# duanyiqun/DiffusionDepth

Measured on AMD Instinct MI355X. Metric: depth-maps/sec (20-step DDIM, KITTI 352x1216 f16r, B=4 maps per GPU per step; depth RMSE vs the reference's CPU path <= 1e-3 on this workload AND at KITTI's depth range 0-80 m: see cpu_baseline.rmse_gate), higher is better.
Workload: dtype f16 (f16 MFMA operands, fp32 accumulation; refined mode: f16-pair weights in conv1 / conv4 / conv3(cond), block-scaled int16 hand-over of y3 and conv3(cond)); 1 GPU; kitti 352x1216 image -> latent 16x176x608, cond 256x176x608, Res head denoiser (mmbev_res50 config), T=20, encoder+loop+decoder, inputs resident in HBM; global_batch=4, parallelism=dp1 (independent images, no collective), ranks_seen=1, streams=2, graph=True, variant=res

## Files before the change

### diffusiondepth_amd/backend.py

```python
from __future__ import annotations

import ctypes
import os
from typing import Dict, Optional

import numpy as np

_HERE = os.path.dirname(os.path.abspath(__file__))
_LIB_NAME = "libddepth_hip.so"
_lib = None

PRECISIONS = {"naive_fp32": 0, "fp32": 1, "bf16": 2, "f16": 3, "fp16": 3, "f16x3": 4, "split_f16": 4, "f16r": 5, "refined_f16": 5}
VARIANTS = {"res": 0, "swin": 1}

ABI_SYMBOLS = [
    "dd_create", "dd_destroy", "dd_last_error", "dd_version", "dd_set_weight", "dd_set_weight_device", "dd_commit_weights",
    "dd_set_schedule", "dd_condition", "dd_neck_condition", "dd_denoise", "dd_denoise_trace", "dd_denoise_once", "dd_denoise_once_backward", "dd_denoise_backward", "dd_zero_grad", "dd_get_grad", "dd_add_noise", "dd_encode", "dd_decode",
    "dd_set_option", "dd_last_loop_ms", "dd_get_counter", "dd_get_layer_ms", "dd_debug_fetch", "dd_debug_weights_digest",
]


def precision_id(p) -> int:
    if isinstance(p, int):
        return p
# ... 272 lines not shown
        cond_in = cond
        cond = _check_tensor(cond, "cond", dtype=torch.float32)
        if cond is not cond_in:
            self._cond_token = None
        B, C, h, w = x_T.shape
        if C != 16 or cond.dim() != 4 or cond.shape[0] != B or cond.shape[1] != 256:
            raise ValueError(f"x_T must be (B,16,h,w) and cond (B,256,ch,cw); got {tuple(x_T.shape)}, {tuple(cond.shape)}")
        T = int(num_inference_steps)
        states = torch.empty((max(T, 1), B, 16, h, w), device=self.device, dtype=torch.float32)
        with torch.cuda.device(self.device):
            self._ck(self._lib.dd_denoise_trace(self._h, x_T.data_ptr(), self._cond_arg(cond, precision), states.data_ptr(), B, h, w,
                                                cond.shape[2], cond.shape[3], T, precision_id(precision), _stream_ptr(self.device)),
                     "dd_denoise_trace")
        return states

    def denoise_once(self, x_t, t, cond, precision="fp32", keep_trajectory=False):
        torch = _torch()
        x_t = _check_tensor(x_t, "x_t", dtype=torch.float32)
        cond = _check_tensor(cond, "cond", dtype=torch.float32)
        B, C, h, w = x_t.shape
        t = torch.as_tensor(t, device=self.device).to(torch.int64).reshape(-1)
        if t.numel() == 1 and B > 1:
            t = t.expand(B)
        t = _check_tensor(t, "t", (B,), torch.int64)
        out = torch.empty_like(x_t)
        self.last_trajectory_ticket = 0
        if keep_trajectory:
            self.set_option("keep_trajectory", 1)
        try:
            with torch.cuda.device(self.device):
                self._ck(self._lib.dd_denoise_once(self._h, x_t.data_ptr(), t.data_ptr(), self._cond_arg(cond, precision), out.data_ptr(),
                                                   B, h, w, cond.shape[2], cond.shape[3], precision_id(precision),
                                                   _stream_ptr(self.device)), "dd_denoise_once")
            if keep_trajectory and precision != "naive_fp32":
                self.last_trajectory_ticket = self.counter("trajectory_ticket")
        finally:
            if keep_trajectory:
                self.set_option("keep_trajectory", 0)
        return out

    PARAM_SHAPES = {
        "model.noise_embedding.0.weight": (64, 16, 3, 3), "model.noise_embedding.0.bias": (64,),
        "model.noise_embedding.1.weight": (64,), "model.noise_embedding.1.bias": (64,),
        "model.noise_embedding.3.weight": (256, 64, 3, 3), "model.noise_embedding.3.bias": (256,),
        "model.noise_embedding.4.weight": (256,), "model.noise_embedding.4.bias": (256,),
        "model.time_embedding.weight": (1280, 256),
        "model.pred.0.weight": (64, 256, 3, 3), "model.pred.0.bias": (64,),
        "model.pred.1.weight": (64,), "model.pred.1.bias": (64,),
        "model.pred.3.weight": (16, 64, 3, 3), "model.pred.3.bias": (16,),
        "model.pred.4.weight": (16,), "model.pred.4.bias": (16,),
    }

    SWIN_PARAM_SHAPES = {
        "model.upsample_fuse.convA.conv.weight": (256, 256, 3, 3), "model.upsample_fuse.convA.conv.bias": (256,),
        "model.upsample_fuse.convB.conv.weight": (256, 256, 3, 3), "model.upsample_fuse.convB.conv.bias": (256,),
    }

    def param_shapes(self):
        d = dict(self.PARAM_SHAPES)
        if self.variant == "swin":
            d.update(self.SWIN_PARAM_SHAPES)
        return d

    def denoise_once_backward(self, x_t, t, cond, grad_eps, precision="naive_fp32", need_grad_x=True, need_grad_cond=True,
                              trajectory_ticket=0):
        torch = _torch()
        x_t = _check_tensor(x_t, "x_t", dtype=torch.float32)
        cond = _check_tensor(cond, "cond", dtype=torch.float32)
        grad_eps = _check_tensor(grad_eps, "grad_eps", x_t.shape, torch.float32)
        B, C, h, w = x_t.shape
        t = torch.as_tensor(t, device=self.device).to(torch.int64).reshape(-1)
        if t.numel() == 1 and B > 1:
            t = t.expand(B)
        t = _check_tensor(t, "t", (B,), torch.int64)
        gx = torch.empty_like(x_t) if need_grad_x else None
        gc = torch.empty_like(cond) if need_grad_cond else None
        if trajectory_ticket:
            self.set_option("use_trajectory", int(trajectory_ticket))
        with torch.cuda.device(self.device):
            self._ck(self._lib.dd_denoise_once_backward(
                self._h, x_t.data_ptr(), t.data_ptr(), cond.data_ptr(), grad_eps.data_ptr(),
                gx.data_ptr() if gx is not None else None, gc.data_ptr() if gc is not None else None,
                B, h, w, cond.shape[2], cond.shape[3], precision_id(precision), _stream_ptr(self.device)), "dd_denoise_once_backward")
        self._cond_token = None
        return gx, gc

    def denoise_backward(self, x_T, cond, grad_x0, num_inference_steps: int, precision="naive_fp32", need_grad_xT=False, need_grad_cond=True,
                         trajectory_ticket=0):
        torch = _torch()
        x_T = _check_tensor(x_T, "x_T", dtype=torch.float32)
        cond = _check_tensor(cond, "cond", dtype=torch.float32)
        grad_x0 = _check_tensor(grad_x0, "grad_x0", x_T.shape, torch.float32)
        B, C, h, w = x_T.shape
        gx = torch.empty_like(x_T) if need_grad_xT else None
        gc = torch.empty_like(cond) if need_grad_cond else None
        if trajectory_ticket:
            self.set_option("use_trajectory", int(trajectory_ticket))
        with torch.cuda.device(self.device):
            self._ck(self._lib.dd_denoise_backward(
                self._h, x_T.data_ptr(), cond.data_ptr(), grad_x0.data_ptr(), gx.data_ptr() if gx is not None else None,
                gc.data_ptr() if gc is not None else None, B, h, w, cond.shape[2], cond.shape[3], int(num_inference_steps),
                precision_id(precision), _stream_ptr(self.device)), "dd_denoise_backward")
        self._cond_token = None
        return gx, gc

    def zero_grad(self):
        self._ck(self._lib.dd_zero_grad(self._h, _stream_ptr(self.device)), "dd_zero_grad")

    def grad(self, name: str):
        torch = _torch()
        out = torch.empty(self.param_shapes()[name], device=self.device, dtype=torch.float32)
        with torch.cuda.device(self.device):
            self._ck(self._lib.dd_get_grad(self._h, name.encode(), out.data_ptr(), out.numel(), _stream_ptr(self.device)), f"dd_get_grad({name})")
        return out

    def grads(self):
        return {k: self.grad(k) for k in self.param_shapes()}

    def add_noise(self, x0, noise, t):
        torch = _torch()
        x0 = _check_tensor(x0, "x0", dtype=torch.float32)
        noise = _check_tensor(noise, "noise", x0.shape, torch.float32)
        B = x0.shape[0]
        t = _check_tensor(torch.as_tensor(t, device=self.device).to(torch.int64).reshape(-1), "t", (B,), torch.int64)
        out = torch.empty_like(x0)
        C, h, w = (x0.shape[1], x0.shape[2], x0.shape[3]) if x0.dim() == 4 else (1, 1, x0[0].numel())
        with torch.cuda.device(self.device):
            self._ck(self._lib.dd_add_noise(self._h, x0.data_ptr(), noise.data_ptr(), t.data_ptr(), out.data_ptr(),
                                            B, C, h, w, _stream_ptr(self.device)), "dd_add_noise")
        return out

    def encode(self, depth):
        torch = _torch()
        depth = _check_tensor(depth, "depth", dtype=torch.float32)
        B, C, H, W = depth.shape
        if C != 1:
            raise ValueError("depth must be (B,1,H,W)")
        out = torch.empty((B, 16, (H - 1) // 2 + 1, (W - 1) // 2 + 1), device=depth.device, dtype=torch.float32)
        with torch.cuda.device(self.device):
            self._ck(self._lib.dd_encode(self._h, depth.data_ptr(), out.data_ptr(), B, H, W, _stream_ptr(self.device)), "dd_encode")
        return out

    def decode(self, latent):
        torch = _torch()
        latent = _check_tensor(latent, "latent", dtype=torch.float32)
        B, C, h, w = latent.shape
        if C != 16:
            raise ValueError("latent must be (B,16,h,w)")
        out = torch.empty((B, 1, 2 * h, 2 * w), device=latent.device, dtype=torch.float32)
        with torch.cuda.device(self.device):
            self._ck(self._lib.dd_decode(self._h, latent.data_ptr(), out.data_ptr(), B, h, w, _stream_ptr(self.device)), "dd_decode")
        return out

    def debug_fetch(self, name: str, B: int, h: int, w: int):
        torch = _torch()
        C = {"y1": 64, "y2": 256, "y3": 64, "y4": 16}[name]
        out = torch.empty((B, C, h, w), device=self.device, dtype=torch.float32)
        self._ck(self._lib.dd_debug_fetch(self._h, name.encode(), out.data_ptr(), out.numel(), _stream_ptr(self.device)),
                 "dd_debug_fetch")
        return out
```

### diffusiondepth_amd/csrc/dd_api.cpp

```cpp
#include "dd_api_internal.h"
#include <cstdlib>

namespace ddapi {
thread_local std::string g_create_error;
}


extern "C" {

const char* dd_version(void) { return "ddepth 0.1 gfx950 (hip, mfma bf16/f16/f32 implicit-GEMM conv3x3+GN+ReLU, hipGraph DDIM loop)"; }

const char* dd_last_error(dd_handle_t h) { return h ? h->err.c_str() : g_create_error.c_str(); }

int dd_create(dd_handle_t* out, int device, int variant) {
  if (!out) { g_create_error = "dd_create: out is NULL"; return DD_ERR_INVALID_ARG; }
  *out = nullptr;
  if (variant != DD_VARIANT_RES && variant != DD_VARIANT_SWIN) { g_create_error = "dd_create: unknown variant"; return DD_ERR_INVALID_ARG; }
  int n = 0;
  hipError_t e = hipGetDeviceCount(&n);
  if (e != hipSuccess || n <= 0) {
    g_create_error = std::string("dd_create: no HIP device available (") + (e != hipSuccess ? hipGetErrorString(e) : "count = 0") +
                     "); this library has no CPU fallback";
    return DD_ERR_HIP;
  }
  if (device < 0 || device >= n) { g_create_error = "dd_create: device index out of range"; return DD_ERR_INVALID_ARG; }
  e = hipSetDevice(device);
  if (e != hipSuccess) { g_create_error = std::string("hipSetDevice: ") + hipGetErrorString(e); return DD_ERR_HIP; }
  dd_handle_t h = new dd_handle_s();
  h->device = device;
  h->variant = variant;
  {
    hipDeviceProp_t prop;
    if (hipGetDeviceProperties(&prop, device) == hipSuccess && prop.multiProcessorCount > 0) {
      h->resident_slots = 2 * prop.multiProcessorCount;
      h->thin_slots = h->resident_slots > 4096 ? 4096 : h->resident_slots;
    }
  }
  {
    const char* pc = getenv("DEBUG_CLR_GRAPH_PACKET_CAPTURE");
    h->use_graph = pc && pc[0] == '0' && pc[1] == 0;
    h->graph_off_by_env = !h->use_graph;
  }
  *out = h;
  return DD_OK;
}

int dd_destroy(dd_handle_t h) {
  if (!h) return DD_OK;
  (void)hipSetDevice(h->device);
  (void)hipDeviceSynchronize();
  drain_layer_events(h);
  h->plans.clear();
  if (h->ev0) (void)hipEventDestroy(h->ev0);
  if (h->ev1) (void)hipEventDestroy(h->ev1);
  if (h->cap_stream) (void)hipStreamDestroy(h->cap_stream);
  for (int l = 0; l < dd_handle_s::MAX_LANES; ++l) {
    if (h->lane_stream[l]) (void)hipStreamDestroy(h->lane_stream[l]);
    if (h->lane_done[l]) (void)hipEventDestroy(h->lane_done[l]);
  }
  if (h->lane_fork) (void)hipEventDestroy(h->lane_fork);
  for (hipStream_t b : h->burnt_streams) (void)hipStreamDestroy(b);
  for (hipEvent_t e : h->probe_events) (void)hipEventDestroy(e);
  delete h;
  return DD_OK;
}

int dd_set_schedule(dd_handle_t h, const float* alphas_cumprod, int num_train_timesteps) {
  if (!h) return DD_ERR_INVALID_ARG;
  if (!alphas_cumprod || num_train_timesteps <= 0) return h->fail(DD_ERR_INVALID_ARG, "dd_set_schedule: null table or non-positive length");
  if (num_train_timesteps > EMB_ROWS)
    return h->fail(DD_ERR_INVALID_ARG, "dd_set_schedule: num_train_timesteps exceeds the time embedding's " + std::to_string(EMB_ROWS) +
                                       " rows (reference ...res.py:313 nn.Embedding(1280, 256))");
  for (int i = 0; i < num_train_timesteps; ++i)
    if (!(alphas_cumprod[i] > 0.f && alphas_cumprod[i] <= 1.f))
      return h->fail(DD_ERR_INVALID_ARG, "dd_set_schedule: alphas_cumprod must lie in (0, 1]");
  DD_HIP(hipSetDevice(h->device));
  DD_HIP(hipDeviceSynchronize());
  h->plans.clear();
  h->last_once_plan = nullptr;
  h->acp.assign(alphas_cumprod, alphas_cumprod + num_train_timesteps);
  h->n_train = num_train_timesteps;
  DD_HIP(h->d_acp.alloc((size_t)num_train_timesteps * 4));
  DD_HIP(hipMemcpy(h->d_acp.p, h->acp.data(), (size_t)num_train_timesteps * 4, hipMemcpyHostToDevice));
  return DD_OK;
}

int dd_set_option(dd_handle_t h, const char* key, int64_t value) {
  if (!h || !key) return DD_ERR_INVALID_ARG;
  const std::string k(key);
  if (k == "graph") h->use_graph = value != 0;
  else if (k == "timing") h->timing = value != 0;
  else if (k == "debug_sync") h->debug_sync = value != 0;
  else if (k == "check_finite") h->check_finite = (int)value;
  else if (k == "train_graphs") h->train_graphs = value != 0;
  else if (k == "graph_fence") h->graph_fence = (int)value;
  else if (k == "ablate") {
    if (h->ablate != (int)value) {
      DD_HIP(hipDeviceSynchronize());
      h->plans.clear();
      h->last_once_plan = nullptr;
    }
    h->ablate = (int)value;
  }
  else if (k == "swin_w5") {
    if (value < 0 || value > 1) return h->fail(DD_ERR_INVALID_ARG, "dd_set_option: swin_w5 must be 0 or 1");
    if (h->swin_w5 != (int)value) { DD_HIP(hipDeviceSynchronize()); h->plans.clear(); h->last_once_plan = nullptr; }
    h->swin_w5 = (int)value;
  }
  else if (k == "hoist_cond") {
    if (value < -1 || value > 1) return h->fail(DD_ERR_INVALID_ARG, "dd_set_option: hoist_cond must be -1 (automatic), 0 or 1");
    h->hoist_cond = (int)value;
  }
  else if (k == "bf16_storage") {
    if (h->bf16_pure != (value != 0)) {
      DD_HIP(hipDeviceSynchronize());
      h->plans.clear(); h->last_once_plan = nullptr;
      h->cond_bufs.clear(); h->fpn_cond.reset(); h->fpn_cond_key[3] = -1; h->fpn_out.reset(); h->fpn_work.reset();
    }
    h->bf16_pure = value != 0;
  }
  else if (k == "naive_wgrad") h->naive_wgrad = value != 0;
  else if (k == "lane_probe") h->lane_probe = value != 0;
  else if (k == "x3_grad_fp32") h->x3_grad_fp32 = value != 0;
  else if (k == "keep_trajectory") h->keep_traj = value != 0;
  else if (k == "use_trajectory") h->use_traj = value;
  else if (k == "adjoint_tiled") h->adjoint_tiled = value != 0;
  else if (k == "streams") h->n_streams = value < 1 ? 1 : (int)value;
  else if (k == "keep_activations_mb") h->keep_act_mb = value < 0 ? 0 : value;
  else if (k == "big_tiles") {
    if (value < -1 || value > 1) return h->fail(DD_ERR_INVALID_ARG, "dd_set_option: big_tiles must be -1 (automatic), 0 or 1");
    if (h->big_tiles != (int)value) { DD_HIP(hipDeviceSynchronize()); h->plans.clear(); h->last_once_plan = nullptr; }
    h->big_tiles = (int)value;
  }
  else if (k == "thin_slots") {
    if (value < 1 || value > 4096) return h->fail(DD_ERR_INVALID_ARG, "dd_set_option: thin_slots must be in [1, 4096]");
    if (h->thin_slots != (int)value) { DD_HIP(hipDeviceSynchronize()); h->plans.clear(); h->last_once_plan = nullptr; }
    h->thin_slots = (int)value;
  }
  else if (k == "one_buffer") {
    if (value < 0 || value > 2) return h->fail(DD_ERR_INVALID_ARG, "dd_set_option: one_buffer must be 0, 1 or 2");
    if (h->one_buffer != (int)value) { DD_HIP(hipDeviceSynchronize()); h->plans.clear(); h->last_once_plan = nullptr; }
    h->one_buffer = (int)value;
  }
  else if (k == "cond_direct") {
    if (value < 0 || value > 1) return h->fail(DD_ERR_INVALID_ARG, "dd_set_option: cond_direct must be 0 or 1");
    h->cond_direct = (int)value;
  }
  else if (k == "cond_split") {
    if (value < 0 || value > 1) return h->fail(DD_ERR_INVALID_ARG, "dd_set_option: cond_split must be 0 or 1");
    h->cond_split = (int)value;
  }
  else if (k == "thin_stream") {
    if (value < 0 || value > 1) return h->fail(DD_ERR_INVALID_ARG, "dd_set_option: thin_stream must be 0 or 1");
    if (h->thin_stream != (int)value) {
      DD_HIP(hipDeviceSynchronize());
      h->plans.clear(); h->last_once_plan = nullptr;
    }
    h->thin_stream = (int)value;
  }
  else if (k == "f16r_wide" || k == "f16r_p4" || k == "f16r_c1") {
    if (value < 0 || value > 1) return h->fail(DD_ERR_INVALID_ARG, "dd_set_option: " + k + " must be 0 or 1");
    int& opt = k == "f16r_wide" ? h->f16r_wide : k == "f16r_c1" ? h->f16r_c1 : h->f16r_p4;
    if (opt != (int)value) { DD_HIP(hipDeviceSynchronize()); h->plans.clear(); h->last_once_plan = nullptr; }
    opt = (int)value;
  }
  else if (k == "phase_prof_buffer") h->prof_buf = reinterpret_cast<unsigned long long*>((uintptr_t)value);
  else if (k == "phase_prof_layer") h->prof_layer = (int)value;
  else if (k == "layer_timing") {
    drain_layer_events(h);
    h->layer_timing = value != 0;
    for (int i = 0; i < dd_handle_s::N_LAYER_SLOTS; ++i) { h->layer_ms[i] = 0; h->layer_cnt[i] = 0; }
  } else return h->fail(DD_ERR_INVALID_ARG, "dd_set_option: unknown key '" + k + "'");
  return DD_OK;
}

int dd_get_counter(dd_handle_t h, const char* key, int64_t* value) {
  if (!h || !key || !value) return DD_ERR_INVALID_ARG;
  const std::string k(key);
  if (k == "graph_launches") *value = h->n_graph_launches;
  else if (k == "graph_default") *value = h->graph_off_by_env ? 0 : 1;
  else if (k == "eager_loops") *value = h->n_eager_loops;
  else if (k == "graph_capture_failures") *value = h->n_capture_failures;
  else if (k == "plans") *value = (int64_t)h->plans.size();
  else if (k == "neck_launches") *value = h->n_neck_launches;
  else if (k == "trajectory_ticket") *value = h->traj_serial;
  else if (k == "lane_calls") *value = h->n_lane_calls;
  else if (k == "lane_probe_retries") *value = h->n_lane_probe_retries;
  else if (k == "lane_overlap") *value = h->lane_overlap_seen;
  else if (k == "cond_split_ok") *value = (h->fpn_committed && h->fpn_split_ok ? 1 : 0) | (h->neck_committed && h->neck_split_ok ? 2 : 0);
  else if (k == "resident_slots") *value = h->resident_slots;
  else if (k == "trajectory_reuses") *value = h->n_traj_reuse;
  else if (k == "thin_stream_launches") *value = h->thin_stream_launches;
  else if (k.compare(0, 13, "kid_launches:") == 0) {
    int id = 0;
    const size_t n = k.size() - 13;
    bool ok = n >= 1 && n <= 3 && !(n > 1 && k[13] == '0');
    for (size_t i = 13; ok && i < k.size(); ++i) { ok = k[i] >= '0' && k[i] <= '9'; id = id * 10 + (k[i] - '0'); }
    if (!ok || !kid_listed(id)) return h->fail(DD_ERR_INVALID_ARG, "dd_get_counter: '" + k + "' does not name a kernel id (dd_kernel_ids.h)");
    *value = h->kid_launches[id];
  }
  else return h->fail(DD_ERR_INVALID_ARG, "dd_get_counter: unknown key '" + k + "'");
  return DD_OK;
}

int dd_get_layer_ms(dd_handle_t h, int layer, double* total_ms, int64_t* launches) {
  if (!h || layer < 1 || layer > dd_handle_s::N_LAYER_SLOTS || !total_ms || !launches) return DD_ERR_INVALID_ARG;
  drain_layer_events(h);
  *total_ms = h->layer_ms[layer - 1];
  *launches = h->layer_cnt[layer - 1];
  return DD_OK;
}

int dd_last_loop_ms(dd_handle_t h, float* ms) {
  if (!h || !ms) return DD_ERR_INVALID_ARG;
  *ms = 0.f;
  if (!h->ev_valid) return DD_OK;
  DD_HIP(hipEventSynchronize(h->ev1));
  DD_HIP(hipEventElapsedTime(ms, h->ev0, h->ev1));
  return DD_OK;
}

static int condition_impl(dd_handle_t h, const float* const* feats, const int* feat_h, const int* feat_w, int n_levels, int B,
                          float* cond_out, int precision, void* stream, bool with_neck);

int dd_condition(dd_handle_t h, const float* const* feats, const int* feat_h, const int* feat_w, int n_levels, int B,
                 float* cond_out, int precision, void* stream) {
  return condition_impl(h, feats, feat_h, feat_w, n_levels, B, cond_out, precision, stream, false);
}

int dd_neck_condition(dd_handle_t h, const float* const* feats, const int* feat_h, const int* feat_w, int n_levels, int B,
                      float* cond_out, int precision, void* stream) {
  if (!h) return DD_ERR_INVALID_ARG;
  if (!h->neck_committed) return h->fail(DD_ERR_STATE, "hahineck.* weights not committed (dd_set_weight for the lateral / projection / fusion convolutions, "
                                                       "dd_commit_weights; DD_VARIANT_SWIN)");
  return condition_impl(h, feats, feat_h, feat_w, n_levels, B, cond_out, precision, stream, true);
}

static int condition_impl(dd_handle_t h, const float* const* feats, const int* feat_h, const int* feat_w, int n_levels, int B,
                          float* cond_out, int precision, void* stream, bool with_neck) {
  if (!h) return DD_ERR_INVALID_ARG;
  if (!h->fpn_committed) return h->fail(DD_ERR_STATE, "conv_lateral.* / conv_up.* weights not committed (dd_set_weight, dd_commit_weights)");
  if (with_neck && h->variant != DD_VARIANT_SWIN)
    return h->fail(DD_ERR_UNSUPPORTED, "dd_neck_condition: the HAHI neck kernels are built for the Swin-L (192/384/768/1536) and MPViT-small (128/216/288/288) pyramids of DD_VARIANT_SWIN");
  if (n_levels != FPN_LEVELS || !feats || !feat_h || !feat_w) return h->fail(DD_ERR_INVALID_ARG, "dd_condition: expects 4 pyramid levels");
  if (precision < DD_PREC_FP32 || precision > DD_PREC_LAST) return h->fail(DD_ERR_INVALID_ARG, "dd_condition: precision must be fp32, bf16, f16, f16x3 or f16r");
  if (B <= 0) return h->fail(DD_ERR_INVALID_ARG, "dd_condition: B must be positive");
  for (int i = 0; i < FPN_LEVELS; ++i) {
    if (!feats[i] || feat_h[i] <= 0 || feat_w[i] <= 0) return h->fail(DD_ERR_INVALID_ARG, "dd_condition: null feature pointer or non-positive size");
    if ((long long)B * feat_h[i] * feat_w[i] * fpn_cin_pad(h->variant, h->fpn_pyramid)[i] >= (1LL << 31) * 4) return h->fail(DD_ERR_INVALID_ARG, "tensor too large");
  }
  hipStream_t s = reinterpret_cast<hipStream_t>(stream);
  DD_HIP(hipSetDevice(h->device));
  int ek = ek_of_precision(precision, h->bf16_pure);
  bool split_pyr = false;
  if (ek == EK_F16S || ek == EK_F16R) {
    split_pyr = h->cond_split && h->fpn_split_ok && (!with_neck || h->neck_split_ok);
    ek = EK_F32;
  }
  const int kk = split_pyr ? (int)EK_F16S : ek;
  const int wk = split_pyr ? WIMG_SPLIT : opnd_kind(ek);
  const int ok = opnd_kind(ek), sk = store_kind(ek);
  const size_t es = ek_size(ek);
  FpnWork* fw = h->fpn_work.get();
  bool same = fw && fw->B == B && fw->ek == ek && fw->pyr == h->fpn_pyramid && (fw->neck || !with_neck);
  for (int i = 0; same && i < FPN_LEVELS; ++i) same = fw->hs[i] == feat_h[i] && fw->ws[i] == feat_w[i];
  if (!same) {
    DD_HIP(hipDeviceSynchronize());
    h->fpn_work.reset(new FpnWork());
    fw = h->fpn_work.get();
    fw->B = B; fw->ek = ek; fw->pyr = h->fpn_pyramid;
    for (int i = 0; i < FPN_LEVELS; ++i) {
      fw->hs[i] = feat_h[i]; fw->ws[i] = feat_w[i];
      const size_t px = (size_t)B * feat_h[i] * feat_w[i];
      DD_HIP(fw->fin[i].alloc(px * fpn_cin_pad(h->variant, h->fpn_pyramid)[i] * es));
      if (with_neck) {
        DD_HIP(fw->nk_cat[i].alloc(px * (neck_ck(h->fpn_pyramid, i) + 512) * es));
        DD_HIP(fw->nk_out[i].alloc(px * neck_ck(h->fpn_pyramid, i) * es));
        fw->neck = true;
      }
      if (i > 0) {
        DD_HIP(fw->lat[i].alloc(px * COND_C * es));
        DD_HIP(fw->up[i - 1].alloc(px * 4 * COND_C * es));
        if (2 * feat_h[i] != feat_h[i - 1] || 2 * feat_w[i] != feat_w[i - 1])
          DD_HIP(fw->pooled[i - 1].alloc((size_t)B * feat_h[i - 1] * feat_w[i - 1] * COND_C * es));
      }
    }
  }
  std::shared_ptr<DevBuf> cbuf;
  int rc = DD_OK;
  const bool swin = h->variant == DD_VARIANT_SWIN;
  if (swin) {
    const size_t need = (size_t)B * feat_h[0] * feat_w[0] * COND_C * es;
    if (!h->fpn_out || h->fpn_out->bytes < need) { h->fpn_out = std::make_shared<DevBuf>(); DD_HIP(h->fpn_out->alloc(need)); }
    cbuf = h->fpn_out;
  } else {
    rc = get_cond_buf(h, B, feat_h[0], feat_w[0], precision, &cbuf);
    if (rc) return rc;
  }

  const int P = pyramid_of(h->variant, h->fpn_pyramid);
  for (int i = FPN_LEVELS - 1; i >= 0; --i) {
    const int hh = feat_h[i], ww = feat_w[i];
    DD_HIP(launch_nchw_to_nhwc_padded(feats[i], fw->fin[i].p, ok, B, fpn_cin(h->variant, h->fpn_pyramid)[i],
                                      fpn_cin_pad(h->variant, h->fpn_pyramid)[i], hh, ww, 1, s));
    const int lat_layer = kid_fpn_lateral(P, i);
    const void* lat_in = fw->fin[i].p;
    if (with_neck) {
      const int C = neck_ck(h->fpn_pyramid, i), CT = C + 512, l_off = (i == 0) ? 512 : 0, e_off = (i == 0) ? 0 : C;
      ConvParams q{};
      q.B = B; q.h = hh; q.w = ww;
      q.in = fw->fin[i].p; q.in_cstride = C; q.in_coff = 0;
      q.out = fw->nk_cat[i].p; q.out_cstride = CT; q.out_coff = l_off;
      q.wpack = h->neck_w[i][wk].p; q.bias = h->neck_b[i].as<float>();
      DD_TRY(launch_conv(h, kid_neck(P, NECK_LATERAL, i), kk, q, s, kid_neck(P, NECK_LATERAL, i)));
      q.in = fw->nk_cat[i].p; q.in_cstride = CT; q.in_coff = l_off;
      q.out = fw->nk_cat[i].p; q.out_cstride = CT; q.out_coff = e_off;
      q.wpack = h->neck_w[4 + i][wk].p; q.bias = h->neck_b[4 + i].as<float>();
      DD_TRY(launch_conv(h, kid_neck(P, NECK_PROJ, i), kk, q, s, kid_neck(P, NECK_PROJ, i)));
      q.in = fw->nk_cat[i].p; q.in_cstride = CT; q.in_coff = 0;
      q.out = fw->nk_out[i].p; q.out_cstride = C; q.out_coff = 0;
      q.wpack = h->neck_w[8 + i][wk].p; q.bias = h->neck_b[8 + i].as<float>();
      DD_TRY(launch_conv(h, kid_neck(P, NECK_FUSION, i), kk, q, s, kid_neck(P, NECK_FUSION, i)));
      h->n_neck_launches += 3;
      lat_in = fw->nk_out[i].p;
    }
    ConvParams p{};
    p.B = B; p.h = hh; p.w = ww;
    p.in = lat_in; p.wpack = h->fpn_lat_w[i][wk].p; p.bias = h->fpn_lat_b[i].as<float>();
    p.out = (i == 0) ? cbuf->p : fw->lat[i].p;
    p.addend = (i == FPN_LEVELS - 1) ? nullptr : (fw->pooled[i].p ? fw->pooled[i].p : fw->up[i].p);
    DD_TRY(launch_conv(h, lat_layer, kk, p, s, lat_layer));
    if (i > 0) {
      ConvParams u{};
      u.B = B; u.h = hh; u.w = ww;
      u.in = fw->lat[i].p; u.wpack = h->fpn_up_w[i - 1][wk].p; u.bias = h->fpn_up_b[i - 1].as<float>(); u.out = fw->up[i - 1].p;
      DD_TRY(launch_conv(h, KID_FPN_UP, kk, u, s, KID_FPN_UP));
      if (fw->pooled[i - 1].p)
        DD_HIP(launch_adaptive_pool_blocked(fw->up[i - 1].p, fw->pooled[i - 1].p, ok, B, COND_C, 2 * hh, 2 * ww, feat_h[i - 1], feat_w[i - 1], s));
    }
    if (h->debug_sync) DD_HIP(hipStreamSynchronize(s));
  }
  if (cond_out) DD_HIP(launch_blocked_to_nchw(cbuf->p, sk, cond_out, B, COND_C, feat_h[0], feat_w[0], 0, s));
  h->fpn_cond = cbuf;
  h->fpn_cond_key[0] = B; h->fpn_cond_key[1] = feat_h[0]; h->fpn_cond_key[2] = feat_w[0]; h->fpn_cond_key[3] = precision;
  return DD_OK;
}

}

namespace ddapi {
int denoise_lane(dd_handle_t h, const float* x_T, const float* cond, float* x_0, int B, int lat_h, int lat_w,
                 int cond_h, int cond_w, int T, int precision, hipStream_t s, int lane, int img0, int whole_B, int64_t ticket, int S) {
  int rc = DD_OK;
  const bool timed = h->timing && lane == 0 && B == whole_B;
  Plan* pl = nullptr;
  int keep = (h->keep_traj && precision != DD_PREC_NAIVE_FP32) ? 1 : 0;
  if (keep) {
    const size_t es = ek_size(store_kind(ek_of_precision(precision, h->bf16_pure)));
    const size_t per_step = (size_t)B * lat_h * lat_w * ((2 * HID_C + COND_C + (h->variant == DD_VARIANT_SWIN ? 2 * COND_C : 0)) * es + LATENT_C * 4);
    const size_t need = per_step * (size_t)T;
    if (need <= ((size_t)h->keep_act_mb << 20) &&
        (h->plans.count(PlanKey{B, lat_h, lat_w, cond_h, cond_w, T, precision, want_hoist(h, precision, T, 2), 2, lane, S}) || keep2_fits(h, need))) keep = 2;
  }
  rc = get_plan(h, PlanKey{B, lat_h, lat_w, cond_h, cond_w, T, precision, want_hoist(h, precision, T, keep), keep, lane, S}, &pl);
  if (rc && keep == 2) {
    (void)hipGetLastError();
    h->plans.erase(PlanKey{B, lat_h, lat_w, cond_h, cond_w, T, precision, want_hoist(h, precision, T, 2), 2, lane, S});
    keep = 1;
    rc = get_plan(h, PlanKey{B, lat_h, lat_w, cond_h, cond_w, T, precision, want_hoist(h, precision, T, keep), keep, lane, S}, &pl);
  }
  if (rc) return rc;
  const size_t n16 = (size_t)B * lat_h * lat_w * LATENT_C;
  float* x_first = keep ? pl->xstash.as<float>() : pl->x[0].as<float>();
  const float* x_last = keep ? pl->xstash.as<float>() + (size_t)(T - 1) * n16 : pl->x[(T - 1) & 1].as<float>();
  if (keep) pl->traj_ticket = 0;

  DD_HIP(launch_nchw_to_nhwc(x_T, x_first, EK_F32, B, LATENT_C, lat_h, lat_w, 0, s));
  rc = stage_condition(h, pl, cond, B, lat_h, lat_w, cond_h, cond_w, precision, s, img0, whole_B);
  if (rc) return rc;
  if (pl->exec && !pl->key.hoist && pl->graph_cond != pl->cond_ptr()) {
    DD_HIP(hipStreamSynchronize(s));
    (void)hipGraphExecDestroy(pl->exec);
    pl->exec = nullptr;
  }

  if (timed) {
    if (!h->ev0) { DD_HIP(hipEventCreate(&h->ev0)); DD_HIP(hipEventCreate(&h->ev1)); }
    DD_HIP(hipEventRecord(h->ev0, s));
  }
  if (precision == DD_PREC_NAIVE_FP32) {
    DD_HIP(hipMemsetAsync(pl->stats.p, 0, pl->stats_bytes, s));
    for (int k = 0; k < T; ++k) {
      float* xc = pl->x[k & 1].as<float>();
      float* xn = pl->x[(k + 1) & 1].as<float>();
      rc = enqueue_naive_eps(h, pl, k, xc, pl->tsteps.as<long long>(), k, 0, s);
      if (rc) return rc;
      DD_HIP(launch_naive_axpby(xc, pl->eps.as<float>(), pl->c1c2.as<float>(), k, xn, (long long)B * lat_h * lat_w * LATENT_C, s));
    }
    h->n_eager_loops++;
    if (timed) { DD_HIP(hipEventRecord(h->ev1, s)); h->ev_valid = true; }
    DD_HIP(launch_nhwc_to_nchw_f32(pl->x[T & 1].p, EK_F32, x_0, B, LATENT_C, lat_h, lat_w, 0, s));
    return DD_OK;
  }

  const bool want_graph = h->use_graph && !h->layer_timing && !h->debug_sync && !pl->capture_failed && (!keep || h->train_graphs);
  bool launched = false;
  if (want_graph) {
    if (!pl->exec) {
      rc = enqueue_loop_body(h, pl, s);
      if (rc) return rc;
      DD_HIP(hipStreamSynchronize(s));
      hipGraph_t graph = nullptr;
      hipError_t e = hipSuccess;
      if (!h->cap_stream) e = hipStreamCreateWithFlags(&h->cap_stream, hipStreamNonBlocking);
      if (e == hipSuccess) e = hipStreamBeginCapture(h->cap_stream, hipStreamCaptureModeThreadLocal);
      if (e == hipSuccess) {
        int brc = enqueue_loop_body(h, pl, h->cap_stream);
        hipError_t e2 = hipStreamEndCapture(h->cap_stream, &graph);
        if (brc == DD_OK && e2 == hipSuccess && graph) {
          e = hipGraphInstantiate(&pl->exec, graph, nullptr, nullptr, 0);
          if (e != hipSuccess) pl->exec = nullptr;
          pl->graph_cond = pl->cond_ptr();
        }
        if (graph) (void)hipGraphDestroy(graph);
      }
      if (!pl->exec) {
        (void)hipGetLastError();
        pl->capture_failed = true;
        h->n_capture_failures++;
      }
      DD_HIP(launch_nchw_to_nhwc(x_T, x_first, EK_F32, B, LATENT_C, lat_h, lat_w, 0, s));
      if (timed) DD_HIP(hipEventRecord(h->ev0, s));
    }
    if (pl->exec) {
      if (h->graph_fence & 1) DD_HIP(hipStreamSynchronize(s));
      if (h->graph_fence & 4) {
        if (!h->lane_fork) DD_HIP(hipEventCreateWithFlags(&h->lane_fork, hipEventDisableTiming));
        if (!h->lane_done[0]) DD_HIP(hipEventCreateWithFlags(&h->lane_done[0], hipEventDisableTiming));
        DD_HIP(hipEventRecord(h->lane_fork, s));
        DD_HIP(hipStreamWaitEvent(h->cap_stream, h->lane_fork, 0));
        DD_HIP(hipGraphLaunch(pl->exec, h->cap_stream));
        DD_HIP(hipEventRecord(h->lane_done[0], h->cap_stream));
        DD_HIP(hipStreamWaitEvent(s, h->lane_done[0], 0));
      } else
      DD_HIP(hipGraphLaunch(pl->exec, s));
      if (h->graph_fence & 2) DD_HIP(hipStreamSynchronize(s));
      h->n_graph_launches++;
      launched = true;
    }
  }
  if (!launched) {
    rc = enqueue_loop_body(h, pl, s);
    if (rc) return rc;
    h->n_eager_loops++;
  }
  if (timed) { DD_HIP(hipEventRecord(h->ev1, s)); h->ev_valid = true; }
  DD_HIP(launch_final(x_last, static_cast<const float*>(pl->slot(pl->y4, T - 1)), pl->stat_ptr(T - 1, 3), h->L[3].gamma.as<float>(),
                      h->L[3].beta.as<float>(), pl->c1c2.as<float>(), T - 1, 0, x_0, B, lat_h, lat_w, s));
  if (keep) { pl->traj_ticket = ticket; pl->traj_weights = h->weights_serial; pl->traj_consumed = false; }
  if (h->debug_sync) DD_HIP(hipStreamSynchronize(s));
  return DD_OK;
}
}

namespace ddapi {
int acquire_lane_stream(dd_handle_t h, int lane, hipStream_t caller) {
  hipStream_t cand = nullptr;
  DD_HIP(hipStreamCreateWithFlags(&cand, hipStreamNonBlocking));
#ifndef DD_HOST_EMULATION
  hipStreamCaptureStatus cs = hipStreamCaptureStatusNone;
  const bool capturing = hipStreamIsCapturing(caller, &cs) == hipSuccess && cs != hipStreamCaptureStatusNone;
  if (h->lane_probe && !capturing) {
    hipEvent_t ea = nullptr, ed = nullptr, ec = nullptr;
    long long* stamps = nullptr;
    DD_HIP(hipEventCreateWithFlags(&ea, hipEventDisableTiming)); DD_HIP(hipEventCreateWithFlags(&ed, hipEventDisableTiming)); DD_HIP(hipEventCreateWithFlags(&ec, hipEventDisableTiming));
    h->probe_events.push_back(ea); h->probe_events.push_back(ed); h->probe_events.push_back(ec);
    DD_HIP(hipMalloc(&stamps, 4 * sizeof(long long)));
    const long long ticks = 10000;
    int rc_ = DD_OK;
    for (int attempt = 0; attempt < 4; ++attempt) {
      hipError_t e = launch_spin(1, nullptr, caller);
      if (e == hipSuccess) e = launch_spin(1, nullptr, cand);
      if (e == hipSuccess) e = hipStreamSynchronize(caller);
      if (e == hipSuccess) e = hipStreamSynchronize(cand);
      if (e == hipSuccess) e = hipEventRecord(ea, caller);
      if (e == hipSuccess) e = hipStreamWaitEvent(cand, ea, 0);
      if (e == hipSuccess) e = launch_spin(ticks, stamps, caller);
      if (e == hipSuccess) e = launch_spin(ticks, stamps + 2, cand);
      if (e == hipSuccess) e = hipEventRecord(ec, cand);
      if (e == hipSuccess) e = hipStreamWaitEvent(caller, ec, 0);
      if (e == hipSuccess) e = hipEventRecord(ed, caller);
      if (e == hipSuccess) e = hipEventSynchronize(ed);
      long long t[4] = {0, 0, 0, 0};
      if (e == hipSuccess) e = hipMemcpy(t, stamps, sizeof t, hipMemcpyDeviceToHost);
      if (e != hipSuccess) { rc_ = h->fail(DD_ERR_HIP, std::string("lane-overlap probe: ") + hipGetErrorString(e)); break; }
      const long long lo = t[0] > t[2] ? t[0] : t[2], hi = t[1] < t[3] ? t[1] : t[3];
      const bool overlap = hi - lo > ticks / 2;
      h->lane_overlap_seen = overlap ? 1 : 0;
      if (overlap || attempt == 3) break;
      h->burnt_streams.push_back(cand);
      h->n_lane_probe_retries++;
      cand = nullptr;
      e = hipStreamCreateWithFlags(&cand, hipStreamNonBlocking);
      if (e != hipSuccess) { rc_ = h->fail(DD_ERR_HIP, std::string("lane-overlap probe: ") + hipGetErrorString(e)); break; }
    }
    (void)hipFree(stamps);
    if (rc_) { if (cand) (void)hipStreamDestroy(cand); return rc_; }
  }
#else
  (void)caller;
#endif
  h->lane_stream[lane] = cand;
  return DD_OK;
}
}

extern "C" {

int dd_denoise(dd_handle_t h, const float* x_T, const float* cond, float* x_0, int B, int lat_h, int lat_w,
               int cond_h, int cond_w, int T, int precision, void* stream) {
  int rc = check_common(h, B, lat_h, lat_w, cond_h, cond_w, true);
  if (rc) return rc;
// ... 25 lines not shown
    const int n = B / S + (l < B % S ? 1 : 0);
    hipStream_t ls = l == 0 ? s : h->lane_stream[l];
    if (l > 0) DD_HIP(hipStreamWaitEvent(ls, h->lane_fork, 0));
    rc = denoise_lane(h, x_T + img0 * n_x, cond ? cond + img0 * n_c : nullptr, x_0 + img0 * n_x, n, lat_h, lat_w, cond_h, cond_w, T, precision,
                      ls, l, img0, B, ticket, S);
    if (l > 0) {
      (void)hipEventRecord(h->lane_done[l], ls);
      (void)hipStreamWaitEvent(s, h->lane_done[l], 0);
    }
    if (rc) return rc;
    img0 += n;
  }
  h->n_lane_calls++;
  if (h->timing) { DD_HIP(hipEventRecord(h->ev1, s)); h->ev_valid = true; }
  return DD_OK;
}

int dd_denoise_trace(dd_handle_t h, const float* x_T, const float* cond, float* states, int B, int lat_h, int lat_w,
                     int cond_h, int cond_w, int T, int precision, void* stream) {
  int rc = check_common(h, B, lat_h, lat_w, cond_h, cond_w, true);
  if (rc) return rc;
  if (!x_T || !states) return h->fail(DD_ERR_INVALID_ARG, "dd_denoise_trace: null tensor pointer");
  if (T <= 0 || T > h->n_train) return h->fail(DD_ERR_INVALID_ARG, "dd_denoise_trace: num_inference_steps must be in [1, num_train_timesteps]");
  if (precision < DD_PREC_NAIVE_FP32 || precision > DD_PREC_LAST) return h->fail(DD_ERR_INVALID_ARG, "dd_denoise_trace: unknown precision");
  rc = check_split(h, precision, "dd_denoise_trace"); if (rc) return rc;
  if (h->variant == DD_VARIANT_SWIN && precision == DD_PREC_NAIVE_FP32)
    return h->fail(DD_ERR_UNSUPPORTED, "DD_VARIANT_SWIN runs on the fused kernels only (no naive path)");
  hipStream_t s = reinterpret_cast<hipStream_t>(stream);
  DD_HIP(hipSetDevice(h->device));
  Plan* pl = nullptr;
  rc = get_plan(h, PlanKey{B, lat_h, lat_w, cond_h, cond_w, T, precision, want_hoist(h, precision, T, 0)}, &pl);
  if (rc) return rc;
  const bool naive = precision == DD_PREC_NAIVE_FP32;
  const size_t n16 = (size_t)B * lat_h * lat_w * LATENT_C;
  if (pl->xstash.bytes < (size_t)(T + 1) * n16 * 4) DD_HIP(pl->xstash.alloc((size_t)(T + 1) * n16 * 4));
  float* X = pl->xstash.as<float>();
  const long long* ts = pl->tsteps.as<long long>();
  DD_HIP(launch_nchw_to_nhwc(x_T, X, EK_F32, B, LATENT_C, lat_h, lat_w, 0, s));
  rc = stage_condition(h, pl, cond, B, lat_h, lat_w, cond_h, cond_w, precision, s);
  if (rc) return rc;
  DD_HIP(hipMemsetAsync(pl->stats.p, 0, pl->stats_bytes, s));
  for (int k = 0; k < T; ++k) {
    if (naive) {
      rc = enqueue_naive_eps(h, pl, k, X + (size_t)k * n16, ts, k, 0, s);
      if (rc) return rc;
      DD_HIP(launch_naive_axpby(X + (size_t)k * n16, pl->eps.as<float>(), pl->c1c2.as<float>(), k, X + (size_t)(k + 1) * n16, (long long)n16, s));
    } else {
      rc = enqueue_fused_step(h, pl, k, (k == 0) ? X : X + (size_t)(k - 1) * n16, X + (size_t)k * n16, k > 0, ts, k, 0, s);
      if (rc) return rc;
    }
  }
  h->n_eager_loops++;
  for (int j = 0; j + 1 < T; ++j)
    DD_HIP(launch_nhwc_to_nchw_f32(X + (size_t)(j + 1) * n16, EK_F32, states + (size_t)j * n16, B, LATENT_C, lat_h, lat_w, 0, s));
  if (naive) {
    DD_HIP(launch_nhwc_to_nchw_f32(X + (size_t)T * n16, EK_F32, states + (size_t)(T - 1) * n16, B, LATENT_C, lat_h, lat_w, 0, s));
  } else {
    DD_HIP(launch_final(X + (size_t)(T - 1) * n16, pl->y4.as<float>(), pl->stat_ptr(T - 1, 3), h->L[3].gamma.as<float>(),
                        h->L[3].beta.as<float>(), pl->c1c2.as<float>(), T - 1, 0, states + (size_t)(T - 1) * n16, B, lat_h, lat_w, s));
  }
  if (h->debug_sync) DD_HIP(hipStreamSynchronize(s));
  return DD_OK;
}

int dd_denoise_once(dd_handle_t h, const float* x_t, const int64_t* t, const float* cond, float* eps, int B, int lat_h,
                    int lat_w, int cond_h, int cond_w, int precision, void* stream) {
  int rc = check_common(h, B, lat_h, lat_w, cond_h, cond_w, false);
  if (rc) return rc;
  if (!x_t || !t || !eps) return h->fail(DD_ERR_INVALID_ARG, "dd_denoise_once: null pointer");
  if (precision < DD_PREC_NAIVE_FP32 || precision > DD_PREC_LAST) return h->fail(DD_ERR_INVALID_ARG, "dd_denoise_once: unknown precision");
  rc = check_split(h, precision, "dd_denoise_once"); if (rc) return rc;
  if (h->variant == DD_VARIANT_SWIN && precision == DD_PREC_NAIVE_FP32)
    return h->fail(DD_ERR_UNSUPPORTED, "DD_VARIANT_SWIN runs on the fused kernels only (no naive path)");
  hipStream_t s = reinterpret_cast<hipStream_t>(stream);
  DD_HIP(hipSetDevice(h->device));
  Plan* pl = nullptr;
  rc = get_plan(h, PlanKey{B, lat_h, lat_w, cond_h, cond_w, 0, precision, want_hoist(h, precision, 0, 0)}, &pl);
  if (rc) return rc;
  const long long* tv = reinterpret_cast<const long long*>(t);
  DD_HIP(launch_nchw_to_nhwc(x_t, pl->x[0].p, EK_F32, B, LATENT_C, lat_h, lat_w, 0, s));
  rc = stage_condition(h, pl, cond, B, lat_h, lat_w, cond_h, cond_w, precision, s);
  if (rc) return rc;
  if (h->variant == DD_VARIANT_SWIN && pl->key.hoist) {
    if (!h->LA.w_oihw.p || !h->LB.w_oihw.p || !h->L[2].w_oihw.p) return h->fail(DD_ERR_STATE, "hoisted Swin form: the fp32 weights of the fuse convolutions are not on the device");
    DD_HIP(launch_swin_ttab(h->LA.w_oihw.as<float>(), h->LB.w_oihw.as<float>(), h->L[2].w_oihw.as<float>(), h->emb.as<float>(), tv, B, lat_h, lat_w,
                            pl->tt_scratch.as<float>(), pl->ttab.as<float>(), s));
  }
  DD_HIP(hipMemsetAsync(pl->stats.p, 0, pl->stats_bytes, s));
  if (precision == DD_PREC_NAIVE_FP32) {
    rc = enqueue_naive_eps(h, pl, 0, pl->x[0].as<float>(), tv, 0, 1, s);
    if (rc) return rc;
    DD_HIP(launch_nhwc_to_nchw_f32(pl->eps.p, EK_F32, eps, B, LATENT_C, lat_h, lat_w, 0, s));
  } else {
    rc = enqueue_fused_step(h, pl, 0, pl->x[0].as<float>(), pl->x[1].as<float>(), false, tv, 0, 1, s);
    if (rc) return rc;
    DD_HIP(launch_final(pl->x[0].as<float>(), pl->y4.as<float>(), pl->stat_ptr(0, 3), h->L[3].gamma.as<float>(),
                        h->L[3].beta.as<float>(), pl->c1c2.as<float>(), 0, 1, eps, B, lat_h, lat_w, s));
  }
  h->last_once_plan = pl;
  pl->traj_ticket = (h->keep_traj && precision != DD_PREC_NAIVE_FP32) ? ++h->traj_serial : 0;
  pl->traj_weights = h->weights_serial;
  if (h->debug_sync) DD_HIP(hipStreamSynchronize(s));
  return DD_OK;
}

int dd_add_noise(dd_handle_t h, const float* x0, const float* noise, const int64_t* t, float* out, int B, int C,
                 int lat_h, int lat_w, void* stream) {
  if (!h) return DD_ERR_INVALID_ARG;
  if (h->n_train <= 0) return h->fail(DD_ERR_STATE, "schedule not set (dd_set_schedule)");
  if (!x0 || !noise || !t || !out || B <= 0 || C <= 0 || lat_h <= 0 || lat_w <= 0)
    return h->fail(DD_ERR_INVALID_ARG, "dd_add_noise: null pointer or non-positive size");
  DD_HIP(hipSetDevice(h->device));
  DD_HIP(launch_add_noise(x0, noise, reinterpret_cast<const long long*>(t), h->d_acp.as<float>(), h->n_train, out, B,
                          (long long)C * lat_h * lat_w, reinterpret_cast<hipStream_t>(stream)));
  return DD_OK;
}

static int ensure_codec_tmp(dd_handle_t h, size_t bytes) {
  if (h->codec_tmp.bytes >= bytes) return DD_OK;
  DD_HIP(hipDeviceSynchronize());
  DD_HIP(h->codec_tmp.alloc(bytes));
  return DD_OK;
}

int dd_encode(dd_handle_t h, const float* depth, float* latent, int B, int H, int W, void* stream) {
  if (!h) return DD_ERR_INVALID_ARG;
  if (!h->codec_committed) return h->fail(DD_ERR_STATE, "depth_transform.* weights not committed");
  if (!depth || !latent || B <= 0 || H <= 0 || W <= 0) return h->fail(DD_ERR_INVALID_ARG, "dd_encode: null pointer or non-positive size");
  DD_HIP(hipSetDevice(h->device));
  const int lh = (H - 1) / 2 + 1, lw = (W - 1) / 2 + 1;
  int rc = ensure_codec_tmp(h, (size_t)B * lh * lw * LATENT_C * 4);
  if (rc) return rc;
  DD_HIP(launch_encode(h->codec, depth, h->codec_tmp.as<float>(), latent, B, H, W, reinterpret_cast<hipStream_t>(stream)));
  return DD_OK;
}

int dd_decode(dd_handle_t h, const float* latent, float* depth, int B, int lat_h, int lat_w, void* stream) {
  if (!h) return DD_ERR_INVALID_ARG;
  if (!h->codec_committed) return h->fail(DD_ERR_STATE, "depth_transform.* weights not committed");
  if (!latent || !depth || B <= 0 || lat_h <= 0 || lat_w <= 0) return h->fail(DD_ERR_INVALID_ARG, "dd_decode: null pointer or non-positive size");
  DD_HIP(hipSetDevice(h->device));
  int rc = ensure_codec_tmp(h, (size_t)B * (2 * lat_h) * (2 * lat_w) * LATENT_C * 4);
  if (rc) return rc;
  DD_HIP(launch_decode(h->codec, latent, h->codec_tmp.as<float>(), depth, B, lat_h, lat_w, reinterpret_cast<hipStream_t>(stream)));
  return DD_OK;
}

int dd_debug_fetch(dd_handle_t h, const char* name, float* out, int64_t numel, void* stream) {
  if (!h || !name || !out) return DD_ERR_INVALID_ARG;
  Plan* pl = h->last_once_plan;
  if (!pl) return h->fail(DD_ERR_STATE, "dd_debug_fetch: no dd_denoise_once call to inspect");
  const std::string n(name);
  const void* src = nullptr; int C = 0; int ek = store_kind(pl->ek);
  if (n == "y1") { src = pl->y1.p; C = HID_C; }
  else if (n == "y2") { src = pl->y2.p; C = COND_C; }
  else if (n == "y3") {
    src = pl->y3.p; C = HID_C;
    if (pl->ek == EK_F16R && pl->wide) return h->fail(DD_ERR_UNSUPPORTED, "dd_debug_fetch: y3 travels as scaled int16 in this plan (option f16r_wide = 1)");
  }
  else if (n == "y4") { src = pl->y4.p; C = LATENT_C; ek = EK_F32; }
  else return h->fail(DD_ERR_INVALID_ARG, "dd_debug_fetch: unknown tensor '" + n + "'");
  if (numel != (int64_t)pl->key.B * C * pl->key.h * pl->key.w) return h->fail(DD_ERR_INVALID_ARG, "dd_debug_fetch: numel mismatch");
  DD_HIP(launch_nhwc_to_nchw_f32(src, ek, out, pl->key.B, C, pl->key.h, pl->key.w, pl->key.prec != DD_PREC_NAIVE_FP32,
                                 reinterpret_cast<hipStream_t>(stream)));
  return DD_OK;
}

int dd_debug_weights_digest(dd_handle_t h, uint64_t* digest) {
  if (!h || !digest) return DD_ERR_INVALID_ARG;
  if (!h->committed) return h->fail(DD_ERR_STATE, "dd_debug_weights_digest: model.* weights not committed");
  DD_HIP(hipSetDevice(h->device));
  DD_HIP(hipDeviceSynchronize());
  uint64_t d = 1469598103934665603ull;
  std::vector<uint8_t> tmp;
  auto eat = [&](const DevBuf& b) -> hipError_t {
    uint64_t n = b.bytes;
    for (int i = 0; i < 8; ++i) { d ^= (n >> (8 * i)) & 0xFF; d *= 1099511628211ull; }
    if (!b.p || !b.bytes) return hipSuccess;
    tmp.resize(b.bytes);
    hipError_t e = hipMemcpy(tmp.data(), b.p, b.bytes, hipMemcpyDeviceToHost);
    if (e != hipSuccess) return e;
    for (uint8_t c : tmp) { d ^= c; d *= 1099511628211ull; }
    return hipSuccess;
  };
  auto eat_layer = [&](const ConvLayer& L) -> hipError_t {
    for (int ek = 0; ek < NUM_EK; ++ek) {
      hipError_t e = eat(L.wpack2[ek]); if (e != hipSuccess) return e;
      e = eat(L.wpackT[ek]); if (e != hipSuccess) return e;
    }
    { hipError_t e = eat(L.wpack2[WIMG_SPLIT]); if (e != hipSuccess) return e; }
    { hipError_t e = eat(L.wpack2[WIMG_STACK]); if (e != hipSuccess) return e; }
    const DevBuf* rest[5] = {&L.bias, &L.w_oihw, &L.wT_oihw, &L.gamma, &L.beta};
    for (const DevBuf* b : rest) { hipError_t e = eat(*b); if (e != hipSuccess) return e; }
    return hipSuccess;
  };
  for (int l = 0; l < 4; ++l) DD_HIP(eat_layer(h->L[l]));
  if (h->variant == DD_VARIANT_SWIN) { DD_HIP(eat_layer(h->LA)); DD_HIP(eat_layer(h->LB)); }
  DD_HIP(eat(h->emb));
  DD_HIP(eat(h->etab));
  *digest = d;
  return DD_OK;
}

}
```

### diffusiondepth_amd/csrc/dd_api_internal.h

```cpp
#pragma once
#include "../../include/ddepth.h"
#include "dd_kernels.h"
#include "dd_kernel_ids.h"

#include <cmath>
#include <cstdio>
#include <cstring>
#include <map>
#include <memory>
#include <set>
#include <string>
#include <tuple>
#include <vector>

using namespace dd;

namespace ddapi {

extern thread_local std::string g_create_error;

struct DevBuf {
  void* p = nullptr;
  size_t bytes = 0;
  DevBuf() = default;
  DevBuf(const DevBuf&) = delete;
  DevBuf& operator=(const DevBuf&) = delete;
  ~DevBuf() { release(); }
  void release() { if (p) { (void)hipFree(p); p = nullptr; bytes = 0; } }
  hipError_t alloc(size_t n) {
    release();
    if (n == 0) n = 16;
    hipError_t e = hipMalloc(&p, n);
    if (e == hipSuccess) bytes = n;
    return e;
  }
  template <class T> T* as() const { return reinterpret_cast<T*>(p); }
};

inline uint16_t host_f32_to_bf16(float f) {
  uint32_t u;
  std::memcpy(&u, &f, 4);
  u += 0x7FFFu + ((u >> 16) & 1u);
  return (uint16_t)(u >> 16);
}
inline uint16_t host_f32_to_f16(float f) {
  _Float16 hf = (_Float16)f;
  uint16_t u;
  std::memcpy(&u, &hf, 2);
  return u;
}

constexpr int NUM_EK = 3;
constexpr int NUM_WIMG = 5;
constexpr int WIMG_SPLIT = 3;
constexpr int WIMG_STACK = 4;
inline int wimg_kind(int slot) { return slot == WIMG_SPLIT ? (int)EK_F16S : slot == WIMG_STACK ? (int)EK_F16R : slot; }
inline int wimg_slot(int kind) { return kind == EK_F16S ? WIMG_SPLIT : kind; }
inline bool wimg_has(int slot, int fwd_layer) { return slot != WIMG_STACK || fwd_layer == KID_CONV4; }
inline int ek_of_precision(int prec, bool bf16_pure) {
  switch (prec) {
    case DD_PREC_FP32: return EK_F32;
    case DD_PREC_BF16: return bf16_pure ? EK_BF16 : EK_BF16M;
    case DD_PREC_F16: return EK_F16;
    case DD_PREC_F16X3: return EK_F16S;
    case DD_PREC_F16R: return EK_F16R;
    default: return -1;
  }
}
inline size_t ek_size(int ek) { return (ek == EK_F32 || ek == EK_F16S) ? 4 : 2; }
inline int thin_kind(int ek) { return ek == EK_BF16M ? (int)EK_F16 : ek; }
constexpr int DD_PREC_LAST = DD_PREC_F16R;

constexpr int FPN_CIN_RES[FPN_LEVELS] = {64, 128, 256, 512};
constexpr int FPN_CIN_SWIN[FPN_LEVELS] = {192, 384, 768, 1536};
constexpr int FPN_CIN_MPVIT[FPN_LEVELS] = {128, 216, 288, 288};
constexpr int FPN_CIN_MPVIT_PAD[FPN_LEVELS] = {128, 224, 288, 288};
enum { PYR_DEFAULT = 0, PYR_MPVIT = 1 };
inline int pyramid_of(int variant, int pyr) { return pyr == PYR_MPVIT ? PYRAMID_MPVIT : variant == DD_VARIANT_SWIN ? PYRAMID_SWIN : PYRAMID_RES; }
inline const int* fpn_cin(int variant, int pyr) {
  return pyr == PYR_MPVIT ? FPN_CIN_MPVIT : (variant == DD_VARIANT_SWIN ? FPN_CIN_SWIN : FPN_CIN_RES);
}
inline const int* fpn_cin_pad(int variant, int pyr) { return pyr == PYR_MPVIT ? FPN_CIN_MPVIT_PAD : fpn_cin(variant, pyr); }

struct ConvLayer {
  int cin = 0, cout = 0;
  DevBuf wpack2[NUM_WIMG];
  DevBuf bias;
  DevBuf w_oihw;
  DevBuf wpackT[NUM_EK];
  DevBuf wT_oihw;
  DevBuf gamma, beta;
};

struct PlanKey {
  int B, h, w, ch, cw, T, prec, hoist;
  int keep = 0;
  int lane = 0;
  int lanes = 1;
  bool operator<(const PlanKey& o) const {
    return std::tie(B, h, w, ch, cw, T, prec, hoist, keep, lane, lanes) < std::tie(o.B, o.h, o.w, o.ch, o.cw, o.T, o.prec, o.hoist, o.keep, o.lane, o.lanes);
  }
};

struct Plan {
  PlanKey key{};
  int ek = EK_F32;
  DevBuf x[2];
  std::shared_ptr<DevBuf> cond;
  const void* cond_alias = nullptr;
  const void* graph_cond = nullptr;
  void* cond_ptr() const { return cond_alias ? const_cast<void*>(cond_alias) : (cond ? cond->p : nullptr); }
  DevBuf y1, y2, y3, y4;
  DevBuf a1, f, a3, eps;
  DevBuf sa, sf;
  DevBuf bX, bA1, bF, bA3;
  DevBuf bSa, bSf;
  DevBuf xstash;
  int64_t traj_ticket = 0;
  int64_t traj_weights = -1;
  bool traj_consumed = false;
  DevBuf gA, gY;
  DevBuf dgb;
  DevBuf bcorr;
  DevBuf ttab, tt_scratch;
  int64_t ttab_weights = -1;
  DevBuf ccond;
  DevBuf ccond_raw;
  DevBuf ccond_scale;
  DevBuf y3_scale;
  bool wide = false, c1 = false, p4 = false;
  DevBuf stats;
  DevBuf c1c2;
  DevBuf tsteps;
  std::vector<long long> tsteps_host;
  size_t stats_bytes = 0;
  hipGraphExec_t exec = nullptr;
  bool capture_failed = false;
  uint64_t last_use = 0;
  ~Plan() { if (exec) (void)hipGraphExecDestroy(exec); }
  int slots = 1;
  size_t kept_bytes = 0;
  void* slot(const DevBuf& b, int step) const { return static_cast<char*>(b.p) + (slots > 1 ? (size_t)step * (b.bytes / slots) : 0); }
  double* stat_ptr(int step, int layer) const {
    return stats.as<double>() + ((size_t)(step * 4 + layer) * key.B) * STAT_SLOTS * STAT_STRIDE;
  }
};

struct FpnWork {
  int B = 0, ek = -1, pyr = 0, hs[FPN_LEVELS] = {0}, ws[FPN_LEVELS] = {0};
  DevBuf fin[FPN_LEVELS];
  DevBuf lat[FPN_LEVELS];
  DevBuf up[FPN_LEVELS - 1];
  DevBuf pooled[FPN_LEVELS - 1];
  bool neck = false;
  DevBuf nk_cat[FPN_LEVELS];
  DevBuf nk_out[FPN_LEVELS];
};


struct NeckConv { int layer; std::string name; int cout, cin, ks, level, kind, C, Ck; };
constexpr int NECK_C_MPVIT[4] = {128, 216, 288, 288};
inline int neck_c(int pyr, int level) { return pyr == PYR_MPVIT ? NECK_C_MPVIT[level] : (192 << level); }
inline int neck_ck(int pyr, int level) { return pyr == PYR_MPVIT ? FPN_CIN_MPVIT_PAD[level] : (192 << level); }
inline std::vector<NeckConv> neck_convs(int pyr) {
  std::vector<NeckConv> v;
  const int P = pyramid_of(DD_VARIANT_SWIN, pyr);
  for (int i = 0; i < 4; ++i) {
    const int C = neck_c(pyr, i), Ck = neck_ck(pyr, i);
    const std::string si = std::to_string(i), sj = std::to_string(i - 1);
    v.push_back({kid_neck(P, NECK_LATERAL, i), "hahineck.lateral_convs." + si, C, C, 1, i, NECK_LATERAL, C, Ck});
    v.push_back({kid_neck(P, NECK_PROJ, i), i == 0 ? std::string("hahineck.conv_proj.0") : "hahineck.trans_proj." + sj, 512, C, 1, i, NECK_PROJ, C, Ck});
    v.push_back({kid_neck(P, NECK_FUSION, i), i == 0 ? std::string("hahineck.conv_fusion.0") : "hahineck.trans_fusion." + sj, C, C + 512, 3, i, NECK_FUSION, C, Ck});
  }
  return v;
}

}
using namespace ddapi;


struct dd_handle_s {
  static constexpr int MAX_LANES = 4;
  int device = 0;
  int variant = DD_VARIANT_RES;
  std::string err;
  std::map<std::string, std::vector<float>> host_w;
  std::map<std::string, std::unique_ptr<DevBuf>> dev_w;
  std::set<std::string> dev_newer;
  bool committed = false;
  bool codec_committed = false;
  ConvLayer L[4];
  ConvLayer LA, LB;
  DevBuf emb;
  DevBuf etab;
  DevBuf w5_oihw, w5pack[NUM_WIMG], pairp, kside;
  int64_t w5_weights = -1;
  int swin_w5 = 1;
  DevBuf zero_bias;
  int hoist_cond = -1;
  bool bf16_pure = false;
  DevBuf codec_buf;
  CodecWeights codec{};
  DevBuf codec_tmp;
  std::vector<float> acp;
  DevBuf d_acp;
  int n_train = 0;
  bool use_graph = true, timing = false, debug_sync = false, layer_timing = false;
  bool graph_off_by_env = false;
  int graph_fence = 0;
  bool train_graphs = false;
  int check_finite = 0;
  DevBuf chk_buf; std::vector<std::string> chk_labels;
  int ablate = 0;
  unsigned long long* prof_buf = nullptr;
  int prof_layer = 0;
  bool keep_traj = false;
  int64_t keep_act_mb = 65536;
  int n_streams = 1;
  int thin_slots = 512;
  int big_tiles = -1;
  int one_buffer = 1;
  int thin_stream = 1;
  int f16r_wide = 1;
  int f16r_c1 = 1;
  int f16r_p4 = 0;
  bool split_ok = true;
  DevBuf wmax;
  int resident_slots = 512;
  hipStream_t lane_stream[MAX_LANES] = {nullptr, nullptr, nullptr, nullptr};
  std::vector<hipEvent_t> probe_events;
  std::vector<hipStream_t> burnt_streams;
  int lane_probe = 1;
  int64_t n_lane_probe_retries = 0, lane_overlap_seen = -1;
  hipEvent_t lane_fork = nullptr, lane_done[MAX_LANES] = {nullptr, nullptr, nullptr, nullptr};
  int64_t n_lane_calls = 0;
  int active_lanes = 1;
  bool adjoint_tiled = true;
  int64_t traj_serial = 0, use_traj = 0, weights_serial = 0, n_traj_reuse = 0;
  int naive_wgrad = 0;
  int x3_grad_fp32 = 0;
  std::map<PlanKey, std::unique_ptr<Plan>> plans;
  DevBuf wgrad_ws[MAX_LANES];
  std::map<std::string, std::unique_ptr<DevBuf>> grads[MAX_LANES];
  std::map<std::tuple<int, int, int, int, int>, std::pair<std::shared_ptr<DevBuf>, uint64_t>> cond_bufs;
  bool neck_committed = false;
  DevBuf neck_w[NECK_CONVS][NUM_WIMG], neck_b[NECK_CONVS];
  int64_t n_neck_launches = 0;
  bool fpn_committed = false;
  int fpn_pyramid = PYR_DEFAULT;
  DevBuf fpn_lat_w[FPN_LEVELS][NUM_WIMG], fpn_lat_b[FPN_LEVELS];
  DevBuf fpn_up_w[FPN_LEVELS - 1][NUM_WIMG], fpn_up_b[FPN_LEVELS - 1];
  std::unique_ptr<FpnWork> fpn_work;
  std::shared_ptr<DevBuf> fpn_out;
  bool fpn_split_ok = false, neck_split_ok = false;
  int cond_direct = 1;
  int cond_split = 1;
  std::shared_ptr<DevBuf> fpn_cond;
  int fpn_cond_key[4] = {0, 0, 0, -1};
  uint64_t tick = 0;
  Plan* last_once_plan = nullptr;
  hipEvent_t ev0 = nullptr, ev1 = nullptr;
  bool ev_valid = false;
  hipStream_t cap_stream = nullptr;
  int64_t n_graph_launches = 0, n_eager_loops = 0, n_capture_failures = 0;
  static constexpr int N_LAYER_SLOTS = KID_LAST;
  double layer_ms[N_LAYER_SLOTS] = {0};
  int64_t layer_cnt[N_LAYER_SLOTS] = {0};
  std::vector<std::tuple<int, hipEvent_t, hipEvent_t>> pending_ev;
  int64_t kid_launches[KID_LAST + 1] = {0};
  int64_t thin_stream_launches = 0;

  int fail(int code, const std::string& m) { err = m; return code; }
};

#define DD_HIP(expr)                                                                              \
  do {                                                                                            \
    hipError_t _e = (expr);                                                                       \
    if (_e != hipSuccess)                                                                         \
      return h->fail(DD_ERR_HIP, std::string(#expr) + ": " + hipGetErrorString(_e));              \
  } while (0)

#define DD_TRY(expr) do { int _rc = (expr); if (_rc != DD_OK) return _rc; } while (0)

namespace ddapi {
struct WeightSpec { std::string name; int64_t numel; };

inline const char* const kConvNames[4] = {"model.noise_embedding.0", "model.noise_embedding.3", "model.pred.0", "model.pred.3"};
inline const char* const kGnNames[4] = {"model.noise_embedding.1", "model.noise_embedding.4", "model.pred.1", "model.pred.4"};
constexpr int kCins[4] = {LATENT_C, HID_C, COND_C, HID_C}, kCouts[4] = {HID_C, COND_C, HID_C, LATENT_C};

int weight_group(const std::string& name);
std::vector<WeightSpec> required_weights(int variant, int pyr = PYR_DEFAULT);
bool pack_conv_weights(const float* w_oihw, const PackGeom& g, int ek, bool swizzle, std::vector<uint8_t>& out);
int pack_geom(dd_handle_t h, int kid, int ek, PackGeom* g);
int upload(dd_handle_t h, DevBuf& dst, const void* src, size_t bytes, hipStream_t s);
int pull_device_weights_to_host(dd_handle_t h, hipStream_t s);
int ensure_bytes(dd_handle_t h, DevBuf& dst, size_t bytes);
int pack_conv_layer_device(dd_handle_t h, ConvLayer& L, const float* w, int fwd_layer, int dgrad_layer, bool with_naive, hipStream_t s);
int commit_model_from_device(dd_handle_t h, hipStream_t s);
int check_common(dd_handle_t h, int B, int lh, int lw, int ch, int cw, bool need_schedule);
int lane_count(dd_handle_t h, int B, int precision);
int check_split(dd_handle_t h, int precision, const char* who);
int acquire_lane_stream(dd_handle_t h, int lane, hipStream_t caller);
int get_cond_buf(dd_handle_t h, int B, int lh, int lw, int precision, std::shared_ptr<DevBuf>* out, int lane = 0);
int want_hoist(dd_handle_t h, int precision, int T = 1, int keep = 0);
bool keep2_fits(dd_handle_t h, size_t need);
bool plan_big_tiles(dd_handle_t h, const PlanKey& key);
int get_plan(dd_handle_t h, const PlanKey& key, Plan** out);
bool conv_tiles(ConvParams& p, int kid, int ek);
int launch_conv(dd_handle_t h, int kid, int ek, ConvParams p, hipStream_t s, int slot = 0);
template <class F> hipError_t timed(dd_handle_t h, int slot, hipStream_t s, F launch) {
  if (!h->layer_timing || slot <= 0) return launch();
  hipEvent_t a, b;
  hipError_t e = hipEventCreate(&a); if (e != hipSuccess) return e;
  e = hipEventCreate(&b); if (e != hipSuccess) return e;
  (void)hipEventRecord(a, s);
  e = launch();
  (void)hipEventRecord(b, s);
  h->pending_ev.emplace_back(slot - 1, a, b);
  return e;
}
int enqueue_fused_step(dd_handle_t h, Plan* pl, int step, const float* x_in, float* x_out, bool apply_update,
                       const long long* tvec, int t_base, int t_bstride, hipStream_t s);
int enqueue_naive_eps(dd_handle_t h, Plan* pl, int step, const float* x_in, const long long* tvec, int t_base,
                      int t_bstride, hipStream_t s);
int enqueue_cond_conv(dd_handle_t h, Plan* pl, hipStream_t s, const float* nchw = nullptr);
int ensure_swin_w5(dd_handle_t h, hipStream_t s);
int enqueue_swin_hoist(dd_handle_t h, Plan* pl, hipStream_t s);
int stage_condition(dd_handle_t h, Plan* pl, const float* cond, int B, int lat_h, int lat_w, int cond_h, int cond_w,
                    int precision, hipStream_t s, int img0 = 0, int whole_B = 0);
int enqueue_loop_body(dd_handle_t h, Plan* pl, hipStream_t s);
void drain_layer_events(dd_handle_t h);
float* grad_buf(dd_handle_t h, const std::string& name, size_t numel, hipStream_t s, hipError_t* err, int lane = 0);
int ensure_bwd_buffers(dd_handle_t h, Plan* pl);
int bwd_core(dd_handle_t h, Plan* pl, const float* x_nhwc, const long long* tv, int t_base, int t_bstride, float* grad_cond,
             int accumulate_cond, hipStream_t s, const Plan* kept = nullptr, int kstep = 0, int lane = 0);
int check_bwd(dd_handle_t h, int precision, const char* who);
int denoise_backward_lane(dd_handle_t h, const float* x_T, const float* cond, const float* grad_x0, float* grad_xT, float* grad_cond,
                          int B, int lat_h, int lat_w, int cond_h, int cond_w, int T, int precision, hipStream_t s, int lane, int img0,
                          int whole_B, int64_t ticket, bool* reused, int S);
}
```

### diffusiondepth_amd/csrc/dd_api_plans.cpp

```cpp
#include "dd_api_internal.h"

namespace ddapi {

int check_common(dd_handle_t h, int B, int lh, int lw, int ch, int cw, bool need_schedule) {
  if (!h) return DD_ERR_INVALID_ARG;
  if (!h->committed) return h->fail(DD_ERR_STATE, "model.* weights not committed (call dd_set_weight for every key, then dd_commit_weights)");
  if (need_schedule && h->n_train <= 0) return h->fail(DD_ERR_STATE, "schedule not set (dd_set_schedule)");
  if (B <= 0 || lh <= 0 || lw <= 0) return h->fail(DD_ERR_INVALID_ARG, "B, lat_h, lat_w must be positive");
  if (h->variant == DD_VARIANT_RES && (ch != lh || cw != lw))
    return h->fail(DD_ERR_INVALID_ARG, "DD_VARIANT_RES needs cond_h,cond_w == lat_h,lat_w (reference ...res.py:340 adds them elementwise)");
  if (h->variant == DD_VARIANT_SWIN && (ch <= 0 || cw <= 0)) return h->fail(DD_ERR_INVALID_ARG, "cond_h, cond_w must be positive");
  if ((long long)B * lh * lw * COND_C >= (1LL << 31) * 4) return h->fail(DD_ERR_INVALID_ARG, "tensor too large");
  return DD_OK;
}

int lane_count(dd_handle_t h, int B, int precision) {
  int S = h->n_streams;
  if (S > B) S = B;
  if (S > dd_handle_s::MAX_LANES) S = dd_handle_s::MAX_LANES;
  if (precision == DD_PREC_NAIVE_FP32 || h->layer_timing || h->debug_sync || h->prof_buf || h->check_finite) S = 1;
  return S < 1 ? 1 : S;
}

int check_split(dd_handle_t h, int precision, const char* who) {
  if (precision != DD_PREC_F16X3 && precision != DD_PREC_F16R) return DD_OK;
  if (!h->split_ok)
    return h->fail(DD_ERR_UNSUPPORTED, std::string(who) + ": a convolution weight of magnitude >= 234 does not fit the split-f16 images (weights are scaled by 256 "
                                       "into f16): DD_PREC_F16X3 / DD_PREC_F16R cannot run on these parameters; the other precisions can");
  return DD_OK;
}

int get_cond_buf(dd_handle_t h, int B, int lh, int lw, int precision, std::shared_ptr<DevBuf>* out, int lane) {
  const auto key = std::make_tuple(B, lh, lw, precision, lane);
  auto it = h->cond_bufs.find(key);
  if (it == h->cond_bufs.end()) {
    while (h->cond_bufs.size() >= 12) {
      auto victim = h->cond_bufs.begin();
      for (auto j = h->cond_bufs.begin(); j != h->cond_bufs.end(); ++j)
        if (j->second.second < victim->second.second) victim = j;
      if (h->fpn_cond == victim->second.first) { h->fpn_cond.reset(); h->fpn_cond_key[3] = -1; }
      h->cond_bufs.erase(victim);
    }
    auto buf = std::make_shared<DevBuf>();
    const size_t es = precision == DD_PREC_NAIVE_FP32 ? 4 : ek_size(cond_kind(ek_of_precision(precision, h->bf16_pure)));
    DD_HIP(buf->alloc((size_t)B * lh * lw * COND_C * es));
    it = h->cond_bufs.emplace(key, std::make_pair(buf, (uint64_t)0)).first;
  }
  it->second.second = ++h->tick;
  *out = it->second.first;
  return DD_OK;
}

int want_hoist(dd_handle_t h, int precision, int T, int keep) {
  if (precision == DD_PREC_NAIVE_FP32) return 0;
  const int ek = ek_of_precision(precision, h->bf16_pure);
  if (h->variant == DD_VARIANT_SWIN) {
    if (T <= 0 && keep == 0 && ek == EK_F16R && h->swin_w5 && h->hoist_cond != 0) return 1;
    if (T <= 0 || keep != 0 || h->hoist_cond == 0 || ((ek == EK_F16S || ek == EK_F16R) && !h->swin_w5)) return 0;
    return (h->hoist_cond == 1 || ek != EK_F32) ? 1 : 0;
  }
  if (h->variant != DD_VARIANT_RES) return 0;
  if (ek == EK_F16R) return 1;
  if (h->hoist_cond >= 0) return h->hoist_cond;
  return (ek == EK_BF16M || ek == EK_F16 || ek == EK_F16S) ? 1 : 0;
}

bool keep2_fits(dd_handle_t h, size_t need) {
  const size_t cap = (size_t)h->keep_act_mb << 20;
  if (need > cap) return false;
  for (;;) {
    size_t held = 0;
    for (auto& kv : h->plans) held += kv.second->kept_bytes;
    size_t free_b = 0, total_b = 0;
    const bool mem_ok = hipMemGetInfo(&free_b, &total_b) != hipSuccess || need + (need >> 3) <= free_b;
    if (held + need <= cap && mem_ok) return true;
    auto victim = h->plans.end();
    for (auto j = h->plans.begin(); j != h->plans.end(); ++j) {
      const Plan& q = *j->second;
      if (q.kept_bytes == 0 || (q.traj_ticket != 0 && q.traj_weights == h->weights_serial && !q.traj_consumed)) continue;
      if (victim == h->plans.end() || q.last_use < victim->second->last_use) victim = j;
    }
    if (victim == h->plans.end()) return false;
    if (h->last_once_plan == victim->second.get()) h->last_once_plan = nullptr;
    (void)hipDeviceSynchronize();
    h->plans.erase(victim);
  }
}

bool plan_big_tiles(dd_handle_t h, const PlanKey& key) {
  if (!key.hoist || key.prec == DD_PREC_NAIVE_FP32) return false;
  if (h->variant != DD_VARIANT_RES && !(h->variant == DD_VARIANT_SWIN && h->swin_w5)) return false;
  const int ek = ek_of_precision(key.prec, h->bf16_pure);
  if (ek == EK_F32 || ek == EK_F16S) return false;
  if (h->big_tiles >= 0) return h->big_tiles != 0;
  const bool many = (long long)key.B * ((key.h + 7) / 8) * ((key.w + 31) / 32) > h->resident_slots;
  return many && h->variant == DD_VARIANT_SWIN;
}
inline int conv3c_kid(dd_handle_t h, const PlanKey& key) { return plan_big_tiles(h, key) ? (int)BIG_CONV3C : KID_CONV3C; }
inline int conv3h_kid(dd_handle_t h, const PlanKey& key) {
  if (plan_big_tiles(h, key)) return (int)BIG_CONV3H;
  const bool many = (long long)key.B * ((key.h + 7) / 8) * ((key.w + 31) / 32) > h->resident_slots;
  return (h->one_buffer == 2 || (many && h->one_buffer)) ? (int)ONE_CONV3H : KID_CONV3H;
}

bool conv_tiles(ConvParams& p, int kid, int ek) {
  const int th = conv_pack_geom2(kid, ek).th;
  if (th <= 0) return false;
  p.tiles_x = (p.w + 31) / 32;
  p.tiles_y = (p.h + th - 1) / th;
  return true;
}
int launch_conv(dd_handle_t h, int kid, int ek, ConvParams p, hipStream_t s, int slot) {
  if (!conv_tiles(p, kid, ek)) return h->fail(DD_ERR_INVALID_ARG, "no fused convolution kernel for kernel id " + std::to_string(kid) + " in element kind " + std::to_string(ek));
  DD_HIP(timed(h, slot, s, [&] { return launch_conv_igemm2(kid, ek, p, s); }));
  h->kid_launches[kid_route(kid, ek).id]++;
  return DD_OK;
}

int get_plan(dd_handle_t h, const PlanKey& key, Plan** out) {
  auto it = h->plans.find(key);
  if (it != h->plans.end()) { it->second->last_use = ++h->tick; *out = it->second.get(); return DD_OK; }
  const size_t cap = 10 + 2 * (size_t)(h->n_streams > 1 ? (h->n_streams < dd_handle_s::MAX_LANES ? h->n_streams : dd_handle_s::MAX_LANES) : 0);
  while (h->plans.size() >= cap) {
    auto victim = h->plans.end();
    for (auto j = h->plans.begin(); j != h->plans.end(); ++j) {
      const Plan& q = *j->second;
      if (q.key.keep && q.traj_ticket != 0 && q.traj_weights == h->weights_serial && !q.traj_consumed) continue;
      if (victim == h->plans.end() || q.last_use < victim->second->last_use) victim = j;
    }
    if (victim == h->plans.end()) break;
    if (h->last_once_plan == victim->second.get()) h->last_once_plan = nullptr;
    DD_HIP(hipDeviceSynchronize());
    h->plans.erase(victim);
  }
  std::unique_ptr<Plan> pl(new Plan());
  pl->key = key;
  const bool naive = key.prec == DD_PREC_NAIVE_FP32;
  pl->ek = naive ? EK_F32 : ek_of_precision(key.prec, h->bf16_pure);
  if (pl->ek == EK_F16R && !key.hoist)
    return h->fail(DD_ERR_UNSUPPORTED, "DD_PREC_F16R runs the hoisted forward-only plans: for the Swin / MPViT denoiser those exist with option swin_w5 = 1 "
                                       "(dd_denoise / dd_denoise_trace / dd_denoise_once); training plans: DD_PREC_F16");
  const size_t px = (size_t)key.B * key.h * key.w;
  const size_t es = ek_size(pl->ek);
  DD_HIP(pl->x[0].alloc(px * LATENT_C * 4));
  DD_HIP(pl->x[1].alloc(px * LATENT_C * 4));
  if (key.keep) DD_HIP(pl->xstash.alloc((size_t)(key.T > 0 ? key.T : 1) * px * LATENT_C * 4));
  const bool swin = h->variant == DD_VARIANT_SWIN;
  if (!(pl->ek == EK_F16R && !swin && key.hoist)) { int rc = get_cond_buf(h, key.B, key.h, key.w, key.prec, &pl->cond, key.lane); if (rc) return rc; }
  pl->slots = (key.keep == 2 && key.T > 0) ? key.T : 1;
  const size_t ns = (size_t)pl->slots;
  if (swin) {
    const size_t es_s = pl->ek == EK_F16R ? 4 : es;
    DD_HIP(pl->sa.alloc(ns * px * COND_C * es_s)); DD_HIP(pl->sf.alloc(ns * px * COND_C * es_s));
  }
  if (key.hoist)
  {
    PackGeom g3;
    DD_TRY(pack_geom(h, conv3h_kid(h, key), pl->ek, &g3));
    const int th = g3.th;
    DD_HIP(pl->ccond.alloc((size_t)key.B * ((key.h + th - 1) / th) * ((key.w + 31) / 32) * th * 32 * HID_C * 4));
    if (pl->ek == EK_F16R) {
      pl->wide = h->f16r_wide != 0; pl->c1 = h->f16r_c1 != 0; pl->p4 = h->f16r_p4 != 0;
      DD_HIP(pl->ccond_raw.alloc((size_t)key.B * ((key.h + 7) / 8) * ((key.w + 31) / 32) * 8 * 32 * HID_C * 4));
      if (pl->wide) DD_HIP(pl->ccond_scale.alloc((size_t)key.B * ((key.h + th - 1) / th) * ((key.w + 31) / 32) * 4 * 2 * (th / 4) * 4));
    }
  }
  if (key.hoist && swin) {
    const int T1 = key.T > 0 ? key.T : key.B;
    const int RH = key.h < SWIN_TT_AX ? key.h : SWIN_TT_AX, RW = key.w < SWIN_TT_AX ? key.w : SWIN_TT_AX;
    DD_HIP(pl->ttab.alloc((size_t)T1 * SWIN_TT_ROWS * HID_C * 4));
    DD_HIP(pl->tt_scratch.alloc((size_t)T1 * RH * RW * (2 * COND_C + HID_C) * 4));
    if (h->swin_w5) {
      DD_HIP(pl->bcorr.alloc((size_t)key.B * swin_ring_stride(key.h, key.w) * HID_C * 4));
      DD_HIP(hipMemsetAsync(pl->bcorr.p, 0, pl->bcorr.bytes, nullptr));
      DD_HIP(hipStreamSynchronize(nullptr));
    }
  }
  DD_HIP(pl->y1.alloc(ns * px * HID_C * es));
  DD_HIP(pl->y2.alloc(ns * px * COND_C * es));
  DD_HIP(pl->y3.alloc(ns * px * HID_C * es));
  if (pl->ek == EK_F16R && h->f16r_wide) DD_HIP(pl->y3_scale.alloc(ns * px * 4));
  DD_HIP(pl->y4.alloc(ns * px * LATENT_C * 4));
  if (key.keep == 2) pl->kept_bytes = pl->y1.bytes + pl->y2.bytes + pl->y3.bytes + pl->y3_scale.bytes + pl->y4.bytes + pl->sa.bytes + pl->sf.bytes;
  if (naive) {
    DD_HIP(pl->a1.alloc(px * HID_C * 4));
    DD_HIP(pl->f.alloc(px * COND_C * 4));
    DD_HIP(pl->a3.alloc(px * HID_C * 4));
    DD_HIP(pl->eps.alloc(px * LATENT_C * 4));
  }
  const int T = key.T > 0 ? key.T : 1;
  pl->stats_bytes = (size_t)(T + 1) * 4 * key.B * STAT_SLOTS * STAT_STRIDE * sizeof(double);
  DD_HIP(pl->stats.alloc(pl->stats_bytes));
  std::vector<float> c1c2((size_t)T * 2, 0.f);
  std::vector<long long> ts((size_t)T, 0);
  if (key.T > 0) {
    const int ratio = h->n_train / key.T;
    for (int k = 0; k < key.T; ++k) {
      const int t = (key.T - 1 - k) * ratio;
      const int prev = t - ratio;
      const double a_t = (double)h->acp[t];
      const double a_prev = prev >= 0 ? (double)h->acp[prev] : 1.0;
      c1c2[2 * k] = (float)std::sqrt(a_prev / a_t);
      c1c2[2 * k + 1] = (float)(std::sqrt(1.0 - a_prev) - std::sqrt(a_prev * (1.0 - a_t) / a_t));
      ts[k] = t;
    }
  }
  DD_HIP(pl->c1c2.alloc(c1c2.size() * 4));
  DD_HIP(pl->tsteps.alloc(ts.size() * 8));
  pl->tsteps_host = ts;
  DD_HIP(hipMemcpy(pl->c1c2.p, c1c2.data(), c1c2.size() * 4, hipMemcpyHostToDevice));
  DD_HIP(hipMemcpy(pl->tsteps.p, ts.data(), ts.size() * 8, hipMemcpyHostToDevice));
  pl->last_use = ++h->tick;
  *out = pl.get();
  h->plans[key] = std::move(pl);
  return DD_OK;
}

int enqueue_fused_step(dd_handle_t h, Plan* pl, int step, const float* x_in, float* x_out, bool apply_update,
                       const long long* tvec, int t_base, int t_bstride, hipStream_t s) {
  const PlanKey& k = pl->key;
  ConvParams p{};
  p.B = k.B; p.h = k.h; p.w = k.w;
  p.ablate = h->ablate;
  if (tvec == pl->tsteps.as<long long>() && t_bstride == 0 && t_base >= 0 && t_base < (int)pl->tsteps_host.size())
    p.t_known = clamp_t(pl->tsteps_host[t_base]);
  const int ek = pl->ek, tk = thin_kind(ek);
  const bool rf = ek == EK_F16R;
  const int wk = ek == EK_F16S ? WIMG_SPLIT : opnd_kind(ek);
  const bool stream4 = h->thin_stream && (tk == EK_F16 || tk == EK_BF16) && !h->prof_buf && k.B <= h->thin_slots;
  auto timed_launch = [&](int layer, ConvParams q, int kid_as = 0) -> int {
    const int kid = kid_as ? kid_as : layer == KID_CONV3H ? conv3h_kid(h, k) : layer;
    q.prof = (h->prof_buf && layer == h->prof_layer) ? h->prof_buf : nullptr;
    if (layer == KID_CONV4 && (rf || stream4)) {
      if (!conv_tiles(q, KID_CONV4, tk)) return h->fail(DD_ERR_INVALID_ARG, "conv4 has no packed geometry in this element kind");
      q.persist_slots = h->thin_slots;
      if (rf) q.cadd_scale = static_cast<const float*>(pl->slot(pl->y3_scale, step));
      DD_HIP(timed(h, layer, s, [&] { return rf ? launch_conv4_stream(EK_F16, q, s, true, pl->wide, pl->p4) : launch_conv4_stream(tk, q, s); }));
      h->thin_stream_launches++;
      return DD_OK;
    }
    int lek = ek;
    if (rf && (layer == KID_CONV3H || layer == KID_SWIN_PRED) && !pl->wide) lek = EK_F16;
    if (rf && layer == KID_CONV1 && !pl->c1) lek = EK_F16;
    return launch_conv(h, kid, lek, q, s, layer);
  };
  void *y1_ = pl->slot(pl->y1, step), *y2_ = pl->slot(pl->y2, step), *y3_ = pl->slot(pl->y3, step), *y4_ = pl->slot(pl->y4, step);
  void *sa_ = pl->slot(pl->sa, step), *sf_ = pl->slot(pl->sf, step);
  const float* y4_prev = static_cast<const float*>(pl->slot(pl->y4, step > 0 ? step - 1 : 0));
  p.in = x_in; p.wpack = h->L[0].wpack2[rf ? (pl->c1 ? WIMG_SPLIT : (int)EK_F16) : wimg_slot(tk)].p; p.bias = h->L[0].bias.as<float>(); p.out = y1_;
  p.stats_out = pl->stat_ptr(step, 0);
  p.stats_in = apply_update ? pl->stat_ptr(step - 1, 3) : nullptr;
  p.gn_gamma = h->L[3].gamma.as<float>(); p.gn_beta = h->L[3].beta.as<float>();
  p.y4 = y4_prev; p.xout = x_out; p.c1c2 = pl->c1c2.as<float>(); p.step = apply_update ? step : 0;
  DD_TRY(timed_launch(KID_CONV1, p));
  p.in = y1_; p.wpack = h->L[1].wpack2[wk].p; p.bias = h->L[1].bias.as<float>(); p.out = y2_;
  p.stats_out = pl->stat_ptr(step, 1); p.stats_in = pl->stat_ptr(step, 0);
  p.gn_gamma = h->L[0].gamma.as<float>(); p.gn_beta = h->L[0].beta.as<float>();
  DD_TRY(timed_launch(KID_CONV2, p));
  if (h->variant == DD_VARIANT_SWIN && k.hoist) {
    p.in = y2_; p.wpack = h->LA.wpack2[wk].p; p.bias = h->zero_bias.as<float>(); p.out = sa_;
    p.stats_out = nullptr; p.stats_in = pl->stat_ptr(step, 1);
    p.gn_gamma = h->L[1].gamma.as<float>(); p.gn_beta = h->L[1].beta.as<float>();
    DD_TRY(timed_launch(KID_SWIN_CONVA, p, SWIN_CONVA_H));
    p.stats_in = nullptr;
    p.cadd = pl->ccond.as<float>(); p.ttab = pl->ttab.as<float>() + (size_t)step * SWIN_TT_ROWS * HID_C;
    p.ttab_bstride = k.T > 0 ? 0 : SWIN_TT_ROWS * HID_C;
    if (pl->bcorr.p) {
      DD_HIP(launch_swin_bcorr(sa_, ek == EK_F16S ? (int)EK_F32 : opnd_kind(ek), h->pairp.as<float>(), h->kside.p, pl->bcorr.as<float>(), k.B, k.h, k.w, s));
      p.in = sa_; p.wpack = h->w5pack[wk].p; p.bias = h->L[2].bias.as<float>(); p.out = y3_;
      p.stats_out = pl->stat_ptr(step, 2); p.bcorr = pl->bcorr.as<float>();
      p.cadd_scale = pl->ccond_scale.as<float>(); p.out_scale = static_cast<float*>(pl->slot(pl->y3_scale, step));
      DD_TRY(timed_launch(KID_SWIN_PRED, p, plan_big_tiles(h, k) ? SWIN_PRED5B_H : SWIN_PRED5_H));
    } else {
      p.in = sa_; p.wpack = h->LB.wpack2[wk].p; p.out = sf_;
      DD_TRY(timed_launch(KID_SWIN_CONVB, p));
      p.in = sf_; p.wpack = h->L[2].wpack2[wk].p; p.bias = h->L[2].bias.as<float>(); p.out = y3_;
      p.stats_out = pl->stat_ptr(step, 2);
      DD_TRY(timed_launch(KID_SWIN_PRED, p, SWIN_PRED_H));
    }
  } else if (h->variant == DD_VARIANT_SWIN) {
    p.in = y2_; p.wpack = h->LA.wpack2[wk].p; p.bias = h->LA.bias.as<float>(); p.out = sa_;
    p.stats_out = nullptr; p.stats_in = pl->stat_ptr(step, 1);
    p.gn_gamma = h->L[1].gamma.as<float>(); p.gn_beta = h->L[1].beta.as<float>();
    p.cond = pl->cond_ptr(); p.emb = h->emb.as<float>(); p.tvec = tvec; p.t_base = t_base; p.t_bstride = t_bstride;
    DD_TRY(timed_launch(KID_SWIN_CONVA, p));
    p.in = sa_; p.wpack = h->LB.wpack2[wk].p; p.bias = h->LB.bias.as<float>(); p.out = sf_;
    p.stats_in = nullptr;
    DD_TRY(timed_launch(KID_SWIN_CONVB, p));
    p.in = sf_; p.wpack = h->L[2].wpack2[wk].p; p.bias = h->L[2].bias.as<float>(); p.out = y3_;
    p.stats_out = pl->stat_ptr(step, 2);
    DD_TRY(timed_launch(KID_SWIN_PRED, p));
  } else {
  p.in = y2_; p.wpack = h->L[2].wpack2[wk].p; p.bias = h->L[2].bias.as<float>(); p.out = y3_;
  p.stats_out = pl->stat_ptr(step, 2); p.stats_in = pl->stat_ptr(step, 1);
  p.gn_gamma = h->L[1].gamma.as<float>(); p.gn_beta = h->L[1].beta.as<float>();
  p.cond = pl->cond_ptr(); p.emb = h->emb.as<float>(); p.tvec = tvec; p.t_base = t_base; p.t_bstride = t_bstride;
  p.cadd = pl->ccond.as<float>(); p.etab = h->etab.as<float>();
  p.cadd_scale = pl->ccond_scale.as<float>(); p.out_scale = static_cast<float*>(pl->slot(pl->y3_scale, step));
  DD_TRY(timed_launch(k.hoist ? KID_CONV3H : KID_CONV3, p));
  p.cadd_scale = nullptr; p.out_scale = nullptr;
  }
  p.in = y3_; p.wpack = h->L[3].wpack2[rf ? WIMG_STACK : wimg_slot(tk)].p; p.bias = h->L[3].bias.as<float>(); p.out = y4_;
  p.stats_out = pl->stat_ptr(step, 3); p.stats_in = pl->stat_ptr(step, 2);
  p.gn_gamma = h->L[2].gamma.as<float>(); p.gn_beta = h->L[2].beta.as<float>();
  DD_TRY(timed_launch(KID_CONV4, p));
  if (h->debug_sync) DD_HIP(hipStreamSynchronize(s));
  return DD_OK;
}

int enqueue_naive_eps(dd_handle_t h, Plan* pl, int step, const float* x_in, const long long* tvec, int t_base,
                      int t_bstride, hipStream_t s) {
  const PlanKey& k = pl->key;
  const int B = k.B, hh = k.h, ww = k.w;
  auto L = h->L;
  DD_HIP(launch_naive_conv3x3(x_in, L[0].w_oihw.as<float>(), L[0].bias.as<float>(), pl->y1.as<float>(), B, hh, ww, LATENT_C, HID_C, s));
  DD_HIP(launch_naive_gn_stats(pl->y1.as<float>(), pl->stat_ptr(step, 0), B, hh, ww, HID_C, s));
  DD_HIP(launch_naive_gn_apply(pl->y1.as<float>(), pl->stat_ptr(step, 0), L[0].gamma.as<float>(), L[0].beta.as<float>(),
                               nullptr, nullptr, nullptr, 0, 0, pl->a1.as<float>(), B, hh, ww, HID_C, s));
  DD_HIP(launch_naive_conv3x3(pl->a1.as<float>(), L[1].w_oihw.as<float>(), L[1].bias.as<float>(), pl->y2.as<float>(), B, hh, ww, HID_C, COND_C, s));
  DD_HIP(launch_naive_gn_stats(pl->y2.as<float>(), pl->stat_ptr(step, 1), B, hh, ww, COND_C, s));
  DD_HIP(launch_naive_gn_apply(pl->y2.as<float>(), pl->stat_ptr(step, 1), L[1].gamma.as<float>(), L[1].beta.as<float>(),
                               static_cast<const float*>(pl->cond_ptr()), h->emb.as<float>(), tvec, t_base, t_bstride, pl->f.as<float>(), B, hh, ww, COND_C, s));
  DD_HIP(launch_naive_conv3x3(pl->f.as<float>(), L[2].w_oihw.as<float>(), L[2].bias.as<float>(), pl->y3.as<float>(), B, hh, ww, COND_C, HID_C, s));
  DD_HIP(launch_naive_gn_stats(pl->y3.as<float>(), pl->stat_ptr(step, 2), B, hh, ww, HID_C, s));
  DD_HIP(launch_naive_gn_apply(pl->y3.as<float>(), pl->stat_ptr(step, 2), L[2].gamma.as<float>(), L[2].beta.as<float>(),
                               nullptr, nullptr, nullptr, 0, 0, pl->a3.as<float>(), B, hh, ww, HID_C, s));
  DD_HIP(launch_naive_conv3x3(pl->a3.as<float>(), L[3].w_oihw.as<float>(), L[3].bias.as<float>(), pl->y4.as<float>(), B, hh, ww, HID_C, LATENT_C, s));
  DD_HIP(launch_naive_gn_stats(pl->y4.as<float>(), pl->stat_ptr(step, 3), B, hh, ww, LATENT_C, s));
  DD_HIP(launch_naive_gn_apply(pl->y4.as<float>(), pl->stat_ptr(step, 3), L[3].gamma.as<float>(), L[3].beta.as<float>(),
                               nullptr, nullptr, nullptr, 0, 0, pl->eps.as<float>(), B, hh, ww, LATENT_C, s));
  if (h->debug_sync) DD_HIP(hipStreamSynchronize(s));
  return DD_OK;
}

int enqueue_cond_conv(dd_handle_t h, Plan* pl, hipStream_t s, const float* nchw) {
  const PlanKey& k = pl->key;
  ConvParams p{};
  p.B = k.B; p.h = k.h; p.w = k.w;
  if (pl->ek == EK_F16R) {
    p.in = nchw ? static_cast<const void*>(nchw) : pl->cond_ptr(); p.wpack = h->L[2].wpack2[WIMG_SPLIT].p; p.bias = h->zero_bias.as<float>();
    p.out = pl->ccond_raw.p;
    DD_TRY(launch_conv(h, nchw ? CONV3C_NCHW : KID_CONV3C, EK_F16S, p, s));
    DD_HIP(launch_cadd_reformat(pl->ccond_raw.as<float>(), pl->ccond.p, pl->ccond_scale.as<float>(), k.B, k.h, k.w, plan_big_tiles(h, k) ? 1 : 0, pl->wide ? 2 : 1, s));
    return DD_OK;
  }
  p.in = pl->cond_ptr(); p.wpack = h->L[2].wpack2[wimg_slot(thin_kind(pl->ek))].p; p.bias = h->zero_bias.as<float>(); p.out = pl->ccond.p;
  return launch_conv(h, conv3c_kid(h, k), pl->ek, p, s);
}


int ensure_swin_w5(dd_handle_t h, hipStream_t s) {
  if (h->w5_weights == h->weights_serial) return DD_OK;
  if (!h->LB.w_oihw.p || !h->L[2].w_oihw.p) return h->fail(DD_ERR_STATE, "hoisted Swin form: the fp32 weights of convB / pred.0 are not on the device");
  if (!h->w5_oihw.p) {
    DD_HIP(h->w5_oihw.alloc((size_t)HID_C * COND_C * 25 * 4)); DD_HIP(h->pairp.alloc((size_t)81 * COND_C * HID_C * 4)); DD_HIP(h->kside.alloc(SWIN_KSIDE_BYTES));
  }
  DD_HIP(launch_swin_compose(h->LB.w_oihw.as<float>(), h->L[2].w_oihw.as<float>(), h->w5_oihw.as<float>(), h->pairp.as<float>(), h->kside.p, s));
  for (int wi = 0; wi < NUM_WIMG; ++wi) {
    if (wi == WIMG_STACK) continue;
    const int ekk = wimg_kind(wi);
    PackGeom g5;
    int rc = pack_geom(h, SWIN_PRED5_H, ekk, &g5); if (rc) return rc;
    rc = ensure_bytes(h, h->w5pack[wi], pack_weights_bytes(g5, ekk)); if (rc) return rc;
    DD_HIP(launch_pack_weights(h->w5_oihw.as<float>(), h->w5pack[wi].p, g5, ekk, true, false, s));
  }
  h->w5_weights = h->weights_serial;
  return DD_OK;
}

int enqueue_swin_hoist(dd_handle_t h, Plan* pl, hipStream_t s) {
  const PlanKey& k = pl->key;
  if (k.T > 0 && pl->ttab_weights != h->weights_serial) {
    if (!h->LA.w_oihw.p || !h->LB.w_oihw.p || !h->L[2].w_oihw.p) return h->fail(DD_ERR_STATE, "hoisted Swin form: the fp32 weights of the fuse convolutions are not on the device");
    DD_HIP(launch_swin_ttab(h->LA.w_oihw.as<float>(), h->LB.w_oihw.as<float>(), h->L[2].w_oihw.as<float>(), h->emb.as<float>(),
                            pl->tsteps.as<long long>(), k.T, k.h, k.w, pl->tt_scratch.as<float>(), pl->ttab.as<float>(), s));
    pl->ttab_weights = h->weights_serial;
  }
  if (pl->bcorr.p) { int rc = ensure_swin_w5(h, s); if (rc) return rc; }
  ConvParams p{};
  p.B = k.B; p.h = k.h; p.w = k.w;
  if (pl->ek == EK_F16R) {
    p.in = pl->cond_ptr(); p.wpack = h->LA.wpack2[WIMG_SPLIT].p; p.bias = h->LA.bias.as<float>(); p.out = pl->sa.p;
    DD_TRY(launch_conv(h, KID_SWIN_CONVB, EK_F16S, p, s));
    p.in = pl->sa.p; p.wpack = h->LB.wpack2[WIMG_SPLIT].p; p.bias = h->LB.bias.as<float>(); p.out = pl->sf.p;
    DD_TRY(launch_conv(h, KID_SWIN_CONVB, EK_F16S, p, s));
    p.in = pl->sf.p; p.wpack = h->L[2].wpack2[WIMG_SPLIT].p; p.bias = h->zero_bias.as<float>(); p.out = pl->ccond_raw.p;
    DD_TRY(launch_conv(h, KID_CONV3C, EK_F16S, p, s));
    DD_HIP(launch_cadd_reformat(pl->ccond_raw.as<float>(), pl->ccond.p, pl->ccond_scale.as<float>(), k.B, k.h, k.w, plan_big_tiles(h, k) ? 1 : 0, pl->wide ? 2 : 1, s));
    return DD_OK;
  }
  const int tk = thin_kind(pl->ek);
  p.in = pl->cond_ptr(); p.wpack = h->LA.wpack2[wimg_slot(tk)].p; p.bias = h->LA.bias.as<float>(); p.out = pl->sa.p;
  DD_TRY(launch_conv(h, KID_SWIN_CONVB, tk, p, s));
  p.in = pl->sa.p; p.wpack = h->LB.wpack2[wimg_slot(tk)].p; p.bias = h->LB.bias.as<float>(); p.out = pl->sf.p;
  DD_TRY(launch_conv(h, KID_SWIN_CONVB, tk, p, s));
  p.in = pl->sf.p; p.wpack = h->L[2].wpack2[wimg_slot(tk)].p; p.bias = h->zero_bias.as<float>(); p.out = pl->ccond.p;
  return launch_conv(h, conv3c_kid(h, k), pl->ek, p, s);
}

int stage_condition(dd_handle_t h, Plan* pl, const float* cond, int B, int lat_h, int lat_w, int cond_h, int cond_w,
                    int precision, hipStream_t s, int img0, int whole_B) {
  if (whole_B <= 0) whole_B = B;
  pl->cond_alias = nullptr;
  const bool direct = cond && h->cond_direct && h->variant != DD_VARIANT_SWIN && pl->ek == EK_F16R && pl->key.hoist;
  if (direct) return enqueue_cond_conv(h, pl, s, cond);
  if (!pl->cond) { int rc = get_cond_buf(h, pl->key.B, pl->key.h, pl->key.w, pl->key.prec, &pl->cond, pl->key.lane); if (rc) return rc; }
  if (cond) {
    if (h->variant == DD_VARIANT_SWIN) DD_HIP(launch_upsample_to_blocked(cond, pl->cond->p, cond_kind(pl->ek), B, COND_C, cond_h, cond_w, lat_h, lat_w, s));
    else DD_HIP(launch_nchw_to_nhwc(cond, pl->cond->p, cond_kind(pl->ek), B, COND_C, cond_h, cond_w, precision != DD_PREC_NAIVE_FP32, s));
    if (h->fpn_cond == pl->cond) { h->fpn_cond.reset(); h->fpn_cond_key[3] = -1; }
  } else if (h->variant == DD_VARIANT_SWIN) {
    const int* k = h->fpn_cond_key;
    if (!h->fpn_cond || h->fpn_cond != h->fpn_out || k[0] != whole_B || k[1] != cond_h || k[2] != cond_w || k[3] != precision)
      return h->fail(DD_ERR_STATE, "cond == NULL needs a preceding dd_condition with the same batch, condition size and precision");
    const char* src = static_cast<const char*>(h->fpn_out->p) + (size_t)img0 * COND_C * cond_h * cond_w * ek_size(cond_kind(pl->ek));
    DD_HIP(launch_upsample_blocked(src, pl->cond->p, cond_kind(pl->ek), B, COND_C, cond_h, cond_w, lat_h, lat_w, s));
  } else {
    const int* k = h->fpn_cond_key;
    const bool whole = img0 == 0 && B == whole_B;
    if (!h->fpn_cond || (whole && h->fpn_cond != pl->cond) || k[0] != whole_B || k[1] != lat_h || k[2] != lat_w || k[3] != precision)
      return h->fail(DD_ERR_STATE, "cond == NULL needs a preceding dd_condition with the same batch, latent size and precision");
    if (!whole)
      pl->cond_alias = static_cast<const char*>(h->fpn_cond->p) + (size_t)img0 * lat_h * lat_w * COND_C * ek_size(cond_kind(pl->ek));
  }
  if (pl->key.hoist) { int rc = h->variant == DD_VARIANT_SWIN ? enqueue_swin_hoist(h, pl, s) : enqueue_cond_conv(h, pl, s); if (rc) return rc; }
  return DD_OK;
}

int enqueue_loop_body(dd_handle_t h, Plan* pl, hipStream_t s) {
  const int T = pl->key.T;
  DD_HIP(hipMemsetAsync(pl->stats.p, 0, pl->stats_bytes, s));
  for (int k = 0; k < T; ++k) {
    const float* xin = (k == 0) ? pl->x[0].as<float>() : pl->x[(k - 1) & 1].as<float>();
    float* xout = pl->x[k & 1].as<float>();
    if (pl->key.keep) {
      const size_t n16 = (size_t)pl->key.B * pl->key.h * pl->key.w * LATENT_C;
      float* X = pl->xstash.as<float>();
      xin = (k == 0) ? X : X + (size_t)(k - 1) * n16;
      xout = X + (size_t)k * n16;
    }
    int rc = enqueue_fused_step(h, pl, k, xin, xout, k > 0, pl->tsteps.as<long long>(), k, 0, s);
    if (rc != DD_OK) return rc;
  }
  return DD_OK;
}

void drain_layer_events(dd_handle_t h) {
  for (auto& t : h->pending_ev) {
    float ms = 0.f;
    if (hipEventSynchronize(std::get<2>(t)) == hipSuccess && hipEventElapsedTime(&ms, std::get<1>(t), std::get<2>(t)) == hipSuccess) {
      const int slot = std::get<0>(t);
      if (slot >= 0 && slot < dd_handle_s::N_LAYER_SLOTS) {
        h->layer_ms[slot] += ms;
        h->layer_cnt[slot] += 1;
      }
    }
    (void)hipEventDestroy(std::get<1>(t));
    (void)hipEventDestroy(std::get<2>(t));
  }
  h->pending_ev.clear();
}

}
```

### diffusiondepth_amd/csrc/dd_api_train.cpp

```cpp
#include "dd_api_internal.h"

namespace ddapi {

float* grad_buf(dd_handle_t h, const std::string& name, size_t numel, hipStream_t s, hipError_t* err, int lane) {
  auto& set = h->grads[lane];
  auto it = set.find(name);
  if (it == set.end()) {
    std::unique_ptr<DevBuf> b(new DevBuf());
    *err = b->alloc(numel * 4);
    if (*err != hipSuccess) return nullptr;
    *err = hipMemsetAsync(b->p, 0, numel * 4, s);
    it = set.emplace(name, std::move(b)).first;
  }
  return it->second->as<float>();
}

}

extern "C" {
int dd_zero_grad(dd_handle_t h, void* stream) {
  if (!h) return DD_ERR_INVALID_ARG;
  DD_HIP(hipSetDevice(h->device));
  for (int l = 0; l < dd_handle_s::MAX_LANES; ++l)
    for (auto& kv : h->grads[l]) DD_HIP(hipMemsetAsync(kv.second->p, 0, kv.second->bytes, reinterpret_cast<hipStream_t>(stream)));
// ... 115 lines not shown
    if (vec) {
      DD_HIP(hipMemsetAsync(pl->dgb.p, 0, (size_t)B * C * 4 * sizeof(double), s));
      DD_HIP(launch_gn_bwd_reduce_blocked(pl->gA.p, ybuf[l], ek, yk, st(l), gamma, beta, pl->dgb.as<double>(), B, C, HW, s));
      DD_HIP(launch_gn_bwd_apply_blocked(pl->gA.p, ybuf[l], ek, yk, st(l), gamma, beta, pl->dgb.as<double>(), pl->gY.p, nullptr,
                                         nullptr, nullptr, nullptr, 0, 0, B, C, HW, s));
      float* demb = nullptr;
      if (l == 1) { demb = grad_buf(h, "model.time_embedding.weight", (size_t)EMB_ROWS * COND_C, s, &e, lane); DD_HIP(e); }
      DD_HIP(launch_gn_param_grad4(pl->dgb.as<double>(), st(l), gamma, dgam, dbet, dbias, demb, tv, t_base, t_bstride, B, C, HW, s));
    } else {
      DD_HIP(hipMemsetAsync(pl->dgb.p, 0, (size_t)B * C * 2 * sizeof(double), s));
      DD_HIP(launch_gn_bwd_reduce(gav, yv, st(l), gamma, beta, pl->dgb.as<double>(), B, s));
      DD_HIP(launch_gn_bwd_apply(gav, yv, st(l), gamma, beta, pl->dgb.as<double>(), gyv, nothing, nothing, nullptr, nullptr, 0, 0, B, s));
      DD_HIP(launch_gn_param_grad(pl->dgb.as<double>(), dgam, dbet, B, C, s));
      DD_HIP(launch_channel_sum(gyv, dbias, nullptr, 0, 0, B, s));
    }
    rc = chk("GroupNorm-backward sums (dgb)", l, pl->dgb.p, (long long)B * C * (vec ? 4 : 2), 3); if (rc) return rc;
    rc = chk("dLoss/dy (gY)", l, pl->gY.p, (long long)B * C * HW, naive ? 0 : kk); if (rc) return rc;
    rc = chk("the conv's input activation", l, inbuf[l], (long long)B * CI * HW, naive ? 0 : kk); if (rc) return rc;
    float* dw = grad_buf(h, std::string(kConvNames[l]) + ".weight", (size_t)C * CI * 9, s, &e, lane); DD_HIP(e);
    const ActView inv{inbuf[l], ek_g, lay, CI, HW};
    if (!naive && ek != EK_F32 && !h->naive_wgrad) {
      const size_t need = wgrad_workspace_bytes(C, CI, B, lat_h, lat_w);
      if (h->wgrad_ws[lane].bytes < need) { DD_HIP(hipStreamSynchronize(s)); DD_HIP(h->wgrad_ws[lane].alloc(need)); }
      DD_HIP(launch_wgrad_mfma(pl->gY.p, inbuf[l], dw, h->wgrad_ws[lane].as<float>(), ek, C, CI, B, lat_h, lat_w, s, h->active_lanes));
    } else {
      DD_HIP(launch_naive_wgrad(gyv, inv, dw, B, lat_h, lat_w, s));
    }
    if (naive) {
      DD_HIP(launch_naive_conv3x3(pl->gY.as<float>(), h->L[l].wT_oihw.as<float>(), nullptr, pl->gA.as<float>(), B, lat_h, lat_w, C, CI, s));
    } else {
      ConvParams q{};
      q.B = B; q.h = lat_h; q.w = lat_w;
      q.in = pl->gY.p; q.wpack = h->L[l].wpackT[ek].p; q.bias = h->zero_bias.as<float>(); q.out = pl->gA.p;
      DD_TRY(launch_conv(h, kid_dgrad(l), ek, q, s));
    }
    rc = chk("weight gradient (dw, accumulated)", l, dw, (long long)C * CI * 9, 0); if (rc) return rc;
    rc = chk("dLoss/d(input) out of the data-gradient convolution (gA)", l, pl->gA.p, (long long)B * CI * HW, (naive || l == 0) ? 0 : kk); if (rc) return rc;
    if (l == 2 && swin) {
      const char* fuse[2] = {"model.upsample_fuse.convB.conv", "model.upsample_fuse.convA.conv"};
      ConvLayer* FL[2] = {&h->LB, &h->LA};
      const void* fin[2] = {sa_buf, pl->bF.p};
      void* gbuf[3] = {pl->gA.p, pl->gY.p, pl->gA.p};
      for (int i = 0; i < 2; ++i) {
        const ActView gout{gbuf[i], ek, 1, COND_C, HW}, fv{fin[i], ek, 1, COND_C, HW};
        float* db = grad_buf(h, std::string(fuse[i]) + ".bias", COND_C, s, &e, lane); DD_HIP(e);
        float* dwf = grad_buf(h, std::string(fuse[i]) + ".weight", (size_t)COND_C * COND_C * 9, s, &e, lane); DD_HIP(e);
        if (ek != EK_F32) DD_HIP(launch_channel_sum_blocked(gbuf[i], ek, db, B, COND_C, HW, s));
        else DD_HIP(launch_channel_sum(gout, db, nullptr, 0, 0, B, s));
        if (ek != EK_F32 && !h->naive_wgrad) {
          const size_t need = wgrad_workspace_bytes(COND_C, COND_C, B, lat_h, lat_w);
          if (h->wgrad_ws[lane].bytes < need) { DD_HIP(hipStreamSynchronize(s)); DD_HIP(h->wgrad_ws[lane].alloc(need)); }
          DD_HIP(launch_wgrad_mfma(gbuf[i], fin[i], dwf, h->wgrad_ws[lane].as<float>(), ek, COND_C, COND_C, B, lat_h, lat_w, s, h->active_lanes));
        } else {
          DD_HIP(launch_naive_wgrad(gout, fv, dwf, B, lat_h, lat_w, s));
        }
        ConvParams q{};
        q.B = B; q.h = lat_h; q.w = lat_w;
        q.in = gbuf[i]; q.wpack = FL[i]->wpackT[ek].p; q.bias = h->zero_bias.as<float>(); q.out = gbuf[i + 1];
        DD_TRY(launch_conv(h, KID_SWIN_CONVB, ek, q, s));
      }
    }
    if (l == 2) {
      const ActView gf{pl->gA.p, ek_g, lay, COND_C, HW};
      if (grad_cond && swin) {
        DD_HIP(launch_upsample_adjoint(pl->gA.p, ek, grad_cond, B, COND_C, pl->key.ch, pl->key.cw, lat_h, lat_w, accumulate_cond, s, h->adjoint_tiled));
      } else if (grad_cond) {
        if (!naive && ek != EK_F32) DD_HIP(launch_blocked_to_nchw(pl->gA.p, ek, grad_cond, B, COND_C, lat_h, lat_w, accumulate_cond, s));
        else DD_HIP(launch_view_to_nchw(gf, grad_cond, B, accumulate_cond, s));
      }
      if (naive || ek == EK_F32) {
        float* demb = grad_buf(h, "model.time_embedding.weight", (size_t)EMB_ROWS * COND_C, s, &e, lane); DD_HIP(e);
        DD_HIP(launch_channel_sum(gf, demb, tv, t_base, t_bstride, B, s));
      }
    }
    if (h->debug_sync) DD_HIP(hipStreamSynchronize(s));
  }
  return DD_OK;
}

int check_finite_begin(dd_handle_t h, hipStream_t s) {
  if (h->check_finite != 2) return DD_OK;
  if (!h->chk_buf.p) DD_HIP(h->chk_buf.alloc(16384 * sizeof(unsigned)));
  DD_HIP(hipMemsetAsync(h->chk_buf.p, 0, 16384 * sizeof(unsigned), s));
  h->chk_labels.clear();
  return DD_OK;
}
int check_finite_report(dd_handle_t h, hipStream_t s) {
  if (h->check_finite != 2 || h->chk_labels.empty()) return DD_OK;
  std::vector<unsigned> c(h->chk_labels.size());
  DD_HIP(hipMemcpyAsync(c.data(), h->chk_buf.p, c.size() * sizeof(unsigned), hipMemcpyDeviceToHost, s));
  DD_HIP(hipStreamSynchronize(s));
  for (size_t i = 0; i < c.size(); ++i)
    if (c[i]) return h->fail(DD_ERR_HIP, "check_finite: first non-finite tensor of this backward (stage " + std::to_string(i) + " of " + std::to_string(c.size()) + "): " +
                                          h->chk_labels[i] + ": " + std::to_string(c[i]) + " values");
  return DD_OK;
}

int check_bwd(dd_handle_t h, int precision, const char* who) {
  if (h->variant == DD_VARIANT_SWIN && precision == DD_PREC_NAIVE_FP32)
    return h->fail(DD_ERR_UNSUPPORTED, std::string(who) + ": DD_VARIANT_SWIN has no unfused path (use fp32 / bf16 / f16)");
  if (precision < DD_PREC_NAIVE_FP32 || precision > DD_PREC_LAST) return h->fail(DD_ERR_INVALID_ARG, std::string(who) + ": unknown precision");
  if (precision == DD_PREC_F16R)
    return h->fail(DD_ERR_UNSUPPORTED, std::string(who) + ": DD_PREC_F16R (refined f16) is a forward-only mode; train in fp32 / f16x3 (the forward's abs-1e-3 modes) or bf16 / f16");
  return check_split(h, precision, who);
}

}

extern "C" {
int dd_denoise_once_backward(dd_handle_t h, const float* x_t, const int64_t* t, const float* cond, const float* grad_eps,
                             float* grad_x, float* grad_cond, int B, int lat_h, int lat_w, int cond_h, int cond_w,
                             int precision, void* stream) {
  int rc = check_common(h, B, lat_h, lat_w, cond_h, cond_w, false);
  if (rc) return rc;
  if (!x_t || !t || !grad_eps) return h->fail(DD_ERR_INVALID_ARG, "dd_denoise_once_backward: null pointer");
  rc = check_bwd(h, precision, "dd_denoise_once_backward");
  if (rc) return rc;
  hipStream_t s = reinterpret_cast<hipStream_t>(stream);
  DD_HIP(hipSetDevice(h->device));
  Plan* pl = nullptr;
  rc = get_plan(h, PlanKey{B, lat_h, lat_w, cond_h, cond_w, 0, precision, want_hoist(h, precision, 0, 0)}, &pl);
  if (rc) return rc;
  rc = ensure_bwd_buffers(h, pl);
  if (rc) return rc;
  DD_HIP(launch_nchw_to_nhwc(x_t, pl->x[0].p, EK_F32, B, LATENT_C, lat_h, lat_w, 0, s));
  rc = stage_condition(h, pl, cond, B, lat_h, lat_w, cond_h, cond_w, precision, s);
  if (rc) return rc;
  DD_HIP(launch_nchw_to_nhwc(grad_eps, pl->gA.p, EK_F32, B, LATENT_C, lat_h, lat_w, 0, s));
  const int64_t ticket = h->use_traj;
  h->use_traj = 0;
  const Plan* kept = nullptr;
  if (ticket != 0 && precision != DD_PREC_NAIVE_FP32) {
    auto it = h->plans.find(PlanKey{B, lat_h, lat_w, cond_h, cond_w, 0, precision, want_hoist(h, precision, 0, 0)});
    if (it != h->plans.end() && it->second->traj_ticket == ticket && it->second->traj_weights == h->weights_serial && it->second->ek == pl->ek)
      kept = it->second.get();
  }
  if (kept) h->n_traj_reuse++;
  rc = check_finite_begin(h, s); if (rc) return rc;
  rc = bwd_core(h, pl, pl->x[0].as<float>(), reinterpret_cast<const long long*>(t), 0, 1, grad_cond, 0, s, kept, 0);
  if (rc) return rc;
  if (grad_x) DD_HIP(launch_nhwc_to_nchw_f32(pl->gA.p, EK_F32, grad_x, B, LATENT_C, lat_h, lat_w, 0, s));
  h->last_once_plan = pl;
  return check_finite_report(h, s);
}

}

namespace ddapi {
int denoise_backward_lane(dd_handle_t h, const float* x_T, const float* cond, const float* grad_x0, float* grad_xT, float* grad_cond,
                          int B, int lat_h, int lat_w, int cond_h, int cond_w, int T, int precision, hipStream_t s, int lane, int img0,
                          int whole_B, int64_t ticket, bool* reused, int S) {
  int rc = DD_OK;
  Plan* pl = nullptr;
  rc = get_plan(h, PlanKey{B, lat_h, lat_w, cond_h, cond_w, T, precision, want_hoist(h, precision, T, 1), 0, lane, S}, &pl);
  if (rc) return rc;
  rc = ensure_bwd_buffers(h, pl);
  if (rc) return rc;
  const bool naive = precision == DD_PREC_NAIVE_FP32;
  const size_t n16 = (size_t)B * lat_h * lat_w * LATENT_C;
  const Plan* kept = nullptr;
  for (int lvl = 2; lvl >= 1 && !kept && ticket != 0 && !naive; --lvl) {
    auto it = h->plans.find(PlanKey{B, lat_h, lat_w, cond_h, cond_w, T, precision, want_hoist(h, precision, T, lvl), lvl, lane, S});
    if (it != h->plans.end() && it->second->traj_ticket == ticket && it->second->traj_weights == h->weights_serial) kept = it->second.get();
  }
  const Plan* kept_act = (kept && kept->key.keep == 2 && kept->ek == pl->ek) ? kept : nullptr;
  *reused = kept != nullptr;
  if (kept) const_cast<Plan*>(kept)->traj_consumed = true;
  const size_t need = (size_t)(kept ? 1 : T + 1) * n16 * 4;
  if (pl->xstash.bytes < need) DD_HIP(pl->xstash.alloc(need));
  float* Xown = pl->xstash.as<float>();
  const float* X = kept ? kept->xstash.as<float>() : Xown;
  float* G = kept ? Xown : Xown + (size_t)T * n16;
  const long long* ts = pl->tsteps.as<long long>();
  rc = stage_condition(h, pl, cond, B, lat_h, lat_w, cond_h, cond_w, precision, s, img0, whole_B);
  if (rc) return rc;
  if (!kept) DD_HIP(launch_nchw_to_nhwc(x_T, Xown, EK_F32, B, LATENT_C, lat_h, lat_w, 0, s));
  if (!kept) DD_HIP(hipMemsetAsync(pl->stats.p, 0, pl->stats_bytes, s));
  for (int k = 0; !kept && k + 1 < T; ++k) {
    if (naive) {
      rc = enqueue_naive_eps(h, pl, k, Xown + (size_t)k * n16, ts, k, 0, s);
      if (rc) return rc;
      DD_HIP(launch_naive_axpby(Xown + (size_t)k * n16, pl->eps.as<float>(), pl->c1c2.as<float>(), k, Xown + (size_t)(k + 1) * n16, (long long)n16, s));
    } else {
      rc = enqueue_fused_step(h, pl, k, (k == 0) ? Xown : Xown + (size_t)(k - 1) * n16, Xown + (size_t)k * n16, k > 0, ts, k, 0, s);
      if (rc) return rc;
    }
  }
  if (!kept && !naive && T > 1) {
    rc = enqueue_fused_step(h, pl, T - 1, Xown + (size_t)(T - 2) * n16, Xown + (size_t)(T - 1) * n16, true, ts, T - 1, 0, s);
    if (rc) return rc;
  }
  DD_HIP(launch_nchw_to_nhwc(grad_x0, G, EK_F32, B, LATENT_C, lat_h, lat_w, 0, s));
  for (int k = T - 1; k >= 0; --k) {
    DD_HIP(launch_bwd_chain(G, pl->gA.as<float>(), pl->c1c2.as<float>(), k, 0, (long long)n16, s));
    rc = bwd_core(h, pl, X + (size_t)k * n16, ts, k, 0, grad_cond, k < T - 1 ? 1 : 0, s, kept_act, k, lane);
    if (rc) return rc;
    DD_HIP(launch_bwd_chain(G, pl->gA.as<float>(), pl->c1c2.as<float>(), k, 1, (long long)n16, s));
  }
  if (grad_xT) DD_HIP(launch_nhwc_to_nchw_f32(G, EK_F32, grad_xT, B, LATENT_C, lat_h, lat_w, 0, s));
  return DD_OK;
}
}

extern "C" {

int dd_denoise_backward(dd_handle_t h, const float* x_T, const float* cond, const float* grad_x0, float* grad_xT, float* grad_cond,
                        int B, int lat_h, int lat_w, int cond_h, int cond_w, int T, int precision, void* stream) {
  int rc = check_common(h, B, lat_h, lat_w, cond_h, cond_w, true);
  if (rc) return rc;
  if (!x_T || !grad_x0) return h->fail(DD_ERR_INVALID_ARG, "dd_denoise_backward: null pointer");
  if (T <= 0 || T > h->n_train) return h->fail(DD_ERR_INVALID_ARG, "dd_denoise_backward: num_inference_steps must be in [1, num_train_timesteps]");
  rc = check_bwd(h, precision, "dd_denoise_backward");
  if (rc) return rc;
  hipStream_t s = reinterpret_cast<hipStream_t>(stream);
  DD_HIP(hipSetDevice(h->device));
  const int64_t ticket = h->use_traj;
  h->use_traj = 0;
  const int S = lane_count(h, B, precision);
  bool reused = false;
  if (S <= 1) {
    rc = check_finite_begin(h, s); if (rc) return rc;
    rc = denoise_backward_lane(h, x_T, cond, grad_x0, grad_xT, grad_cond, B, lat_h, lat_w, cond_h, cond_w, T, precision, s, 0, 0, B, ticket, &reused, 1);
    if (rc == DD_OK && reused) h->n_traj_reuse++;
    return rc ? rc : check_finite_report(h, s);
  }
  for (int l = 1; l < S; ++l) {
    if (!h->lane_stream[l]) { rc = acquire_lane_stream(h, l, s); if (rc) return rc; }
    if (!h->lane_done[l]) DD_HIP(hipEventCreateWithFlags(&h->lane_done[l], hipEventDisableTiming));
  }
  if (!h->lane_fork) DD_HIP(hipEventCreateWithFlags(&h->lane_fork, hipEventDisableTiming));
  DD_HIP(hipEventRecord(h->lane_fork, s));
  const size_t n_x = (size_t)LATENT_C * lat_h * lat_w, n_c = (size_t)COND_C * cond_h * cond_w;
  int img0 = 0;
  bool all_reused = true;
  h->active_lanes = S;
  for (int l = 0; l < S; ++l) {
    const int n = B / S + (l < B % S ? 1 : 0);
    hipStream_t ls = l == 0 ? s : h->lane_stream[l];
    if (l > 0) DD_HIP(hipStreamWaitEvent(ls, h->lane_fork, 0));
    rc = denoise_backward_lane(h, x_T + img0 * n_x, cond ? cond + img0 * n_c : nullptr, grad_x0 + img0 * n_x, grad_xT ? grad_xT + img0 * n_x : nullptr,
                               grad_cond ? grad_cond + img0 * n_c : nullptr, n, lat_h, lat_w, cond_h, cond_w, T, precision, ls, l, img0, B, ticket, &reused, S);
    all_reused = all_reused && reused;
    if (l > 0) {
      (void)hipEventRecord(h->lane_done[l], ls);
      (void)hipStreamWaitEvent(s, h->lane_done[l], 0);
    }
    if (rc) {
      h->active_lanes = 1;
      for (int q = 1; q < dd_handle_s::MAX_LANES; ++q)
        for (auto& kv : h->grads[q]) (void)hipMemsetAsync(kv.second->p, 0, kv.second->bytes, s);
      return rc;
    }
    img0 += n;
  }
  h->active_lanes = 1;
  for (int l = 1; l < S; ++l)
    for (auto& kv : h->grads[l]) {
      hipError_t e = hipSuccess;
      float* dst = grad_buf(h, kv.first, kv.second->bytes / 4, s, &e, 0); DD_HIP(e);
      DD_HIP(launch_add_inplace(dst, kv.second->as<float>(), (long long)(kv.second->bytes / 4), s));
      DD_HIP(hipMemsetAsync(kv.second->p, 0, kv.second->bytes, s));
    }
  if (all_reused) h->n_traj_reuse++;
  h->n_lane_calls++;
  return DD_OK;
}

}
```

### diffusiondepth_amd/csrc/dd_igemm2.hip

```cpp
#include "dd_igemm2_cfg.h"
#include "dd_gcn.h"

namespace dd {

#if DD_PHASE_PROF && !defined(DD_HOST_EMULATION)
#define DD_PROF_MARK(i) do { if (p.prof != nullptr && threadIdx.x == 0) p.prof[(size_t)blockIdx.x * 8 + (i)] = (unsigned long long)wall_clock64(); } while (0)
#define DD_PROF_HWID() do { if (p.prof != nullptr && threadIdx.x == 0) {                                                     \
    unsigned hw_, xcc_; asm volatile("s_getreg_b32 %0, hwreg(HW_REG_HW_ID)" : "=s"(hw_)); asm volatile("s_getreg_b32 %0, hwreg(HW_REG_XCC_ID)" : "=s"(xcc_));   \
    p.prof[(size_t)blockIdx.x * 8 + 6] = hw_; p.prof[(size_t)blockIdx.x * 8 + 7] = xcc_; } } while (0)
#define DD_PROF_CLK() ((unsigned long long)__builtin_amdgcn_s_memtime())
#define DD_PROF_LOOP_DECL unsigned long long pl_acc_[4] = {0, 0, 0, 0}, pl_t_ = 0
#define DD_PROF_LOOP_START() do { if (p.prof != nullptr) pl_t_ = DD_PROF_CLK(); } while (0)
#define DD_PROF_LOOP_ADD(k) do { if (p.prof != nullptr) { const unsigned long long n_ = DD_PROF_CLK(); pl_acc_[k] += n_ - pl_t_; pl_t_ = n_; } } while (0)
#define DD_PROF_LOOP_STORE() do { if (p.prof != nullptr && lane == 0) { for (int k_ = 0; k_ < 4; ++k_)                          \
    p.prof[(size_t)gridDim.x * 8 + ((size_t)blockIdx.x * C::WAVES + wave) * 4 + k_] = pl_acc_[k_]; } } while (0)
#else
#define DD_PROF_MARK(i) ((void)0)
#define DD_PROF_HWID() ((void)0)
#define DD_PROF_LOOP_DECL
#define DD_PROF_LOOP_START() ((void)0)
#define DD_PROF_LOOP_ADD(k) ((void)0)
#define DD_PROF_LOOP_STORE() ((void)0)
#endif

// ... 510 lines not shown
          for (int tg = 0; tg < C::NTG; ++tg) stage(chunk + par, tg, par);
        } else {
#pragma unroll 1
          for (int tg = 0; tg < C::NTG; ++tg) stage(chunk + par, tg, par);
        }
      }
    }
  } else if constexpr (C::TG == 1) {
#pragma unroll 1
    for (int chunk = 0; chunk < C::NCHUNK; ++chunk) {
#pragma unroll
      for (int tg = 0; tg < C::NTG; ++tg) stage(chunk, tg, 0);
    }
  } else {
#pragma unroll 1
    for (int chunk = 0; chunk < C::NCHUNK; ++chunk) {
#pragma unroll 1
      for (int tg = 0; tg < C::NTG; ++tg) stage(chunk, tg, 0);
    }
  }

  DD_PROF_MARK(3);
  DD_PROF_LOOP_STORE();
#ifndef DD_HOST_EMULATION
  if constexpr (C::SPW > 1) asm volatile("" : "+s"(n0));
#endif
  constexpr int NG_LOCAL = (C::COUT == COND_C) ? C::NT / (COND_C / GN_GROUPS) : 4;
  float ls[4] = {0.f, 0.f, 0.f, 0.f}, lq[4] = {0.f, 0.f, 0.f, 0.f};
  char* out_b = reinterpret_cast<char*>(p.out) + (size_t)e_b * h * w * C::COUT * C::OUT_ESZ;
  if constexpr (C::IS_NECK) {
    const int cs = p.out_cstride ? p.out_cstride : C::COUT;
    out_b = reinterpret_cast<char*>(p.out) + ((size_t)e_b * cs + p.out_coff) * h * w * C::OUT_ESZ;
  }
#pragma unroll
  for (int m = 0; m < C::WM; ++m) {
    const int gy = e_y0 + wave * C::WM + m, gx = e_x0 + li;
    const bool pvalid = gy < h && gx < w && !(abl & 16);
    int trow = -1;
    if constexpr (C::ADD_T) {
      const int rc = swin_tt_class(gy, h), cc = swin_tt_class(gx, w);
      if (pvalid && (rc != swin_tt_ref(h) || cc != swin_tt_ref(w))) trow = 1 + rc * SWIN_TT_AX + cc;
    }
    unsigned tapmask = 0x1FFu;
    if constexpr (C::ADD_C) {
      const unsigned ry = (gy >= 1 ? 1u : 0u) | 2u | (gy + 1 < h ? 4u : 0u);
      const unsigned rx = (gx >= 1 ? 1u : 0u) | 2u | (gx + 1 < w ? 4u : 0u);
      tapmask = ((ry & 1u) ? rx : 0u) | ((ry & 2u) ? (rx << 3) : 0u) | ((ry & 4u) ? (rx << 6) : 0u);
    }
    auto value_of = [&](int n, int q, float (&v)[4]) {
      const int co = n0 + n * 32 + 8 * q + 4 * g;
      (void)co;
        float4 bv = *reinterpret_cast<const float4*>(tab_bias + (sp ^ flip) * C::NT + n * 32 + 8 * q + 4 * g);
        if constexpr (C::ADD_C) {
          if (tapmask != 0x1FFu) {
            const int cl = n * 32 + 8 * q + 4 * g;
#pragma unroll
            for (int tap = 0; tap < 9; ++tap) {
              if (!((tapmask >> tap) & 1u)) {
                const float4 ev = *reinterpret_cast<const float4*>(tab_et + tap * HID_C + cl);
                bv.x -= ev.x; bv.y -= ev.y; bv.z -= ev.z; bv.w -= ev.w;
              }
            }
          }
        }
        if constexpr (C::ADD_T) {
          if (trow >= 0) {
            const float4 dv = *reinterpret_cast<const float4*>(p.ttab + (size_t)e_b * p.ttab_bstride + trow * HID_C + n * 32 + 8 * q + 4 * g);
            bv.x += dv.x; bv.y += dv.y; bv.z += dv.z; bv.w += dv.w;
          }
          if constexpr (C::PRED5) {
            if (pvalid && (gy == 0 || gy == h - 1 || gx == 0 || gx == w - 1)) {
              const float* ring = p.bcorr + (size_t)e_b * swin_ring_stride(h, w) * HID_C + n * 32 + 8 * q + 4 * g;
              const float4 cv = *reinterpret_cast<const float4*>(ring + (size_t)swin_ring_index(gy, gx, h, w) * HID_C);
              bv.x -= cv.x; bv.y -= cv.y; bv.z -= cv.z; bv.w -= cv.w;
              if ((gy == 0 || gy == h - 1) && (gx == 0 || gx == w - 1)) {
                const float4 cc = *reinterpret_cast<const float4*>(ring + (size_t)(swin_ring_size(h, w) + (gy ? 2 : 0) + (gx ? 1 : 0)) * HID_C);
                bv.x -= cc.x; bv.y -= cc.y; bv.z -= cc.z; bv.w -= cc.w;
              }
            }
          }
        }
        if constexpr (C::SPLIT) {
          constexpr float OS = split_oscale(C::PRO);
          v[0] = fmaf(acc[n][m][q * 4 + 0], OS, bv.x); v[1] = fmaf(acc[n][m][q * 4 + 1], OS, bv.y);
          v[2] = fmaf(acc[n][m][q * 4 + 2], OS, bv.z); v[3] = fmaf(acc[n][m][q * 4 + 3], OS, bv.w);
        } else {
          v[0] = acc[n][m][q * 4 + 0] + bv.x; v[1] = acc[n][m][q * 4 + 1] + bv.y;
          v[2] = acc[n][m][q * 4 + 2] + bv.z; v[3] = acc[n][m][q * 4 + 3] + bv.w;
        }
        if constexpr (C::RELU_OUT) {
#pragma unroll
          for (int i = 0; i < 4; ++i) v[i] = (v[i] < 0.f) ? 0.f : v[i];
          if constexpr (C::IS_LAT) {
            if (p.addend != nullptr && pvalid) {
              constexpr int AESZ = C::SPLIT ? 4 : C::ESZ;
              const char* ab = reinterpret_cast<const char*>(p.addend) + ((size_t)e_b * h * w * C::COUT + act_offset(C::COUT, h, w, 0, co, gy, gx)) * AESZ;
              float a4[4];
              if constexpr (AESZ == 4) {
                const float4 t4 = *reinterpret_cast<const float4*>(ab);
                a4[0] = t4.x; a4[1] = t4.y; a4[2] = t4.z; a4[3] = t4.w;
              } else {
                const uint2 t2 = *reinterpret_cast<const uint2*>(ab);
                if constexpr (EK == EK_BF16) {
                  a4[0] = bf16_to_f32(t2.x & 0xFFFFu); a4[1] = bf16_to_f32(t2.x >> 16); a4[2] = bf16_to_f32(t2.y & 0xFFFFu); a4[3] = bf16_to_f32(t2.y >> 16);
                } else {
                  a4[0] = f16_to_f32(t2.x & 0xFFFFu); a4[1] = f16_to_f32(t2.x >> 16); a4[2] = f16_to_f32(t2.y & 0xFFFFu); a4[3] = f16_to_f32(t2.y >> 16);
                }
              }
#pragma unroll
              for (int i = 0; i < 4; ++i) v[i] += a4[i];
            }
          }
        }
    };
    if constexpr (C::Q15) {
      float pmax = 0.f;
#pragma unroll
      for (int n = 0; n < C::WN; ++n)
#pragma unroll
        for (int q = 0; q < 4; ++q) {
          float v[4];
          value_of(n, q, v);
          if (pvalid) {
            const float s = (v[0] + v[1]) + (v[2] + v[3]);
            const float sq = fmaf(v[0], v[0], fmaf(v[1], v[1], fmaf(v[2], v[2], v[3] * v[3])));
            const int lg = 2 * n + (q >> 1);
            ls[lg] += s; lq[lg] += sq;
          }
          pmax = fmaxf(pmax, fmaxf(fmaxf(fabsf(v[0]), fabsf(v[1])), fmaxf(fabsf(v[2]), fabsf(v[3]))));
#pragma unroll
          for (int i = 0; i < 4; ++i) acc[n][m][q * 4 + i] = v[i];
        }
      pmax = fmaxf(pmax, __shfl_xor(pmax, 32, 64));
      const float inv = pmax > 0.f ? 1.f / pmax : 0.f;
      if (pvalid && g == 0) p.out_scale[(size_t)e_b * h * w + (size_t)gy * w + gx] = pmax * (1.f / Q15_ONE);
#pragma unroll
      for (int n = 0; n < C::WN; ++n) {
        uint2 pk[4];
#pragma unroll
        for (int q = 0; q < 4; ++q) {
          pk[q].x = DD_CVT_PKNORM_I16(acc[n][m][q * 4 + 0] * inv, acc[n][m][q * 4 + 1] * inv);
          pk[q].y = DD_CVT_PKNORM_I16(acc[n][m][q * 4 + 2] * inv, acc[n][m][q * 4 + 3] * inv);
        }
#pragma unroll
        for (int k = 0; k < 2; ++k) {
          const auto rx = __builtin_amdgcn_permlane32_swap(pk[2 * k].x, pk[2 * k + 1].x, false, false);
          const auto ry = __builtin_amdgcn_permlane32_swap(pk[2 * k].y, pk[2 * k + 1].y, false, false);
          const int co = n0 + n * 32 + 16 * k + 8 * g;
          if (pvalid) *reinterpret_cast<uint4*>(out_b + act_offset(C::COUT, h, w, 0, co, gy, gx) * 2) = make_uint4(rx[0], ry[0], rx[1], ry[1]);
        }
      }
      continue;
    }
#pragma unroll
    for (int n = 0; n < C::WN; ++n) {
      uint2 pk[4];
#pragma unroll
      for (int q = 0; q < 4; ++q) {
        if (C::COUT < 32 && q >= 2) continue;
        const int co = n0 + n * 32 + 8 * q + 4 * g;
        float v[4];
        value_of(n, q, v);
        if (C::STATS && pvalid) {
          const float s = (v[0] + v[1]) + (v[2] + v[3]);
          const float sq = fmaf(v[0], v[0], fmaf(v[1], v[1], fmaf(v[2], v[2], v[3] * v[3])));
          const int lg = (C::COUT == COND_C) ? (n >> 1) : (C::COUT == HID_C) ? (2 * n + (q >> 1)) : q;
          ls[lg] += s; lq[lg] += sq;
        }
        if constexpr (C::LAYER == KID_CONV3C) {
          const size_t fi = ((((size_t)e_tile * C::WAVES + wave) * C::WN + n) * C::WM + m) * 256 + q * 64 + lane;
          if constexpr (C::CADD16) reinterpret_cast<uint2*>(p.out)[fi] = make_uint2(pack2<EK_F16>(v[0], v[1]), pack2<EK_F16>(v[2], v[3]));
          else reinterpret_cast<float4*>(p.out)[fi] = make_float4(v[0], v[1], v[2], v[3]);
        } else if constexpr (C::OUT_ESZ == 4) {
          if (pvalid && (C::COUT_PAD == C::COUT || co < C::COUT)) {
            if constexpr (C::SCATTER) {
              const int par = co >> 8, cc = co & (COND_C - 1);
              *reinterpret_cast<float4*>(reinterpret_cast<char*>(p.out) + ((size_t)e_b * 4 * h * w * COND_C +
                  act_offset(COND_C, 2 * h, 2 * w, 0, cc, 2 * gy + (par >> 1), 2 * gx + (par & 1))) * 4) = make_float4(v[0], v[1], v[2], v[3]);
            } else {
              *reinterpret_cast<float4*>(out_b + act_offset(C::COUT, h, w, 0, co, gy, gx) * 4) = make_float4(v[0], v[1], v[2], v[3]);
            }
          }
        } else {
          pk[q].x = pack2<C::OUT_K>(v[0], v[1]);
          pk[q].y = pack2<C::OUT_K>(v[2], v[3]);
        }
      }
      if constexpr (C::OUT_ESZ == 2) {
#pragma unroll
        for (int k = 0; k < 2; ++k) {
          const auto rx = __builtin_amdgcn_permlane32_swap(pk[2 * k].x, pk[2 * k + 1].x, false, false);
          const auto ry = __builtin_amdgcn_permlane32_swap(pk[2 * k].y, pk[2 * k + 1].y, false, false);
          const int co = n0 + n * 32 + 16 * k + 8 * g;
          if (pvalid && (C::COUT_PAD == C::COUT || co < C::COUT)) {
            if constexpr (C::SCATTER) {
              const int par = co >> 8, cc = co & (COND_C - 1);
              *reinterpret_cast<uint4*>(reinterpret_cast<char*>(p.out) + ((size_t)e_b * 4 * h * w * COND_C +
                  act_offset(COND_C, 2 * h, 2 * w, 0, cc, 2 * gy + (par >> 1), 2 * gx + (par & 1))) * 2) = make_uint4(rx[0], ry[0], rx[1], ry[1]);
            } else {
              *reinterpret_cast<uint4*>(out_b + act_offset(C::COUT, h, w, 0, co, gy, gx) * 2) = make_uint4(rx[0], ry[0], rx[1], ry[1]);
            }
          }
        }
      }
    }
  }
  DD_PROF_MARK(4);
  if constexpr (!C::STATS) { DD_PROF_MARK(5); return; }
  constexpr int TOP = (C::COUT < 32) ? 16 : 32;
#pragma unroll
  for (int off = TOP; off >= 1; off >>= 1) {
#pragma unroll
    for (int k = 0; k < 4; ++k) { ls[k] += __shfl_xor(ls[k], off, 64); lq[k] += __shfl_xor(lq[k], off, 64); }
  }
  double ds[4], dq[4];
#pragma unroll
  for (int k = 0; k < 4; ++k) { ds[k] = (double)ls[k]; dq[k] = (double)lq[k]; }
  if constexpr (C::COUT < 32) {
    if (li == 0) {
      s_red[wave * 8 + (0 + g) * 2 + 0] = ds[0]; s_red[wave * 8 + (0 + g) * 2 + 1] = dq[0];
      s_red[wave * 8 + (2 + g) * 2 + 0] = ds[1]; s_red[wave * 8 + (2 + g) * 2 + 1] = dq[1];
    }
  } else {
    if (lane == 0) {
#pragma unroll
      for (int k = 0; k < 4; ++k) { s_red[wave * 8 + k * 2] = ds[k]; s_red[wave * 8 + k * 2 + 1] = dq[k]; }
    }
  }
  __syncthreads();
  if (tid < 2 * NG_LOCAL && !(abl & 32)) {
    double tot = 0.0;
#pragma unroll
    for (int wv = 0; wv < C::WAVES; ++wv) tot += s_red[wv * 8 + tid];
    const int gbase = (C::COUT == COND_C) ? (n0 / (COND_C / GN_GROUPS)) : 0;
    double* dst = p.stats_out + ((size_t)e_b * STAT_SLOTS + (wgid % STAT_SLOTS)) * STAT_STRIDE + gbase * 2 + tid;
    atomicAdd(dst, tot);
  }
  DD_PROF_MARK(5);
  if (sp + 1 >= C::SPW) break;
  n0 = (nsplit + ((sp + 1) ^ flip)) * C::NT;
  sbase += C::NSTAGE;
  init_acc();
  }
}

template <int EK, int LAYER>
static hipError_t launch_one2(const ConvParams& p, hipStream_t s) {
  using C = Cfg2<EK, LAYER>;
  static bool attr_set = false;
  if (!attr_set) {
    hipError_t e = hipFuncSetAttribute(reinterpret_cast<const void*>(&conv_igemm2_kernel<C>),
                                       hipFuncAttributeMaxDynamicSharedMemorySize, C::SMEM_BYTES);
    if (e != hipSuccess) return e;
    attr_set = true;
  }
  unsigned n_wg = (unsigned)(p.tiles_x * p.tiles_y * p.B * (C::COUT_PAD / C::NT / C::SPW));
  dim3 grid(n_wg, 1);
  hipLaunchKernelGGL(conv_igemm2_kernel<C>, grid, dim3(C::THREADS), C::SMEM_BYTES, s, p);
  return hipGetLastError();
}
template <int ID, class Op> static auto for_kind(int ek, Op op) {
  switch (ek) {
    case EK_F32: return op.template run<EK_F32, ID>();
    case EK_BF16: return op.template run<EK_BF16, ID>();
    case EK_F16: return op.template run<EK_F16, ID>();
    case EK_BF16M: return op.template run<EK_BF16M, ID>();
    case EK_F16S: return op.template run<EK_F16S, ID>();
    case EK_F16R: return op.template run<EK_F16R, ID>();
    default: return op.none();
  }
}
template <class Op> static auto for_kernel_id(int id, int ek, Op op) {
  switch (id) {
#define DD_KID_CASE(K) case K: return for_kind<K>(ek, op);
    DD_KERNEL_IDS(DD_KID_CASE)
#undef DD_KID_CASE
    default: return op.none();
  }
}
struct LaunchOp {
  const ConvParams& p; hipStream_t s;
  static hipError_t none() { return hipErrorInvalidValue; }
  template <int EK, int ID> hipError_t run() const {
    constexpr KidRoute r = kid_route(ID, EK);
    if constexpr (r.id != 0) return launch_one2<r.ek, r.id>(p, s); else return none();
  }
};
hipError_t launch_conv_igemm2(int layer, int ek, const ConvParams& p, hipStream_t s) { return for_kernel_id(layer, ek, LaunchOp{p, s}); }

struct GeomOp {
  static PackGeom none() { return PackGeom{}; }
  template <int EK, int ID> PackGeom run() const {
    constexpr KidRoute r = kid_image(ID, EK);
    if constexpr (r.id != 0) {
      using C = Cfg2<r.ek, r.id>;
      return PackGeom{C::CIN, C::COUT, C::COUT_PAD, C::CK, C::TG, C::NT, C::TH, C::KS, C::NPL, (EK == EK_F16R && ID == KID_CONV4) ? 1 : 0};
    } else {
      return none();
    }
  }
};
PackGeom conv_pack_geom2(int layer, int ek) { return for_kernel_id(layer, ek, GeomOp{}); }

}
```

### diffusiondepth_amd/csrc/dd_kernels.h

```cpp
#pragma once
#include <hip/hip_runtime.h>
#include <stdint.h>

namespace dd {

constexpr int LATENT_C = 16;
constexpr int HID_C = 64;
constexpr int COND_C = 256;
constexpr int GN_GROUPS = 4;
constexpr int EMB_ROWS = 1280;
__host__ __device__ inline long long clamp_t(long long t) { return t < 0 ? 0 : (t >= EMB_ROWS ? EMB_ROWS - 1 : t); }
constexpr float GN_EPS = 1e-5f;
constexpr float BN_EPS = 1e-5f;

constexpr int STAT_SLOTS = 32;
constexpr int STAT_STRIDE = 16;

enum ElemKind : int { EK_F32 = 0, EK_BF16 = 1, EK_F16 = 2, EK_BF16M = 3, EK_F16S = 4, EK_F16R = 5 };
constexpr float Q15_ONE = 32767.f;
__host__ __device__ constexpr int opnd_kind(int ek) { return ek == EK_BF16M ? (int)EK_BF16 : (ek == EK_F16S || ek == EK_F16R) ? (int)EK_F16 : ek; }
__host__ __device__ constexpr int store_kind(int ek) { return (ek == EK_BF16M || ek == EK_F16R) ? (int)EK_F16 : ek == EK_F16S ? (int)EK_F32 : ek; }
__host__ __device__ constexpr int cond_kind(int ek) { return ek == EK_F16R ? (int)EK_F32 : store_kind(ek); }
constexpr float STACK_LSCALE = 2048.f;
constexpr float SPLIT_WSCALE = 256.f;
constexpr float SPLIT_PSCALE = 16.f;
__host__ __device__ constexpr float split_pscale(int pro) { return (pro == 1  || pro == 2 ) ? SPLIT_PSCALE : 1.f; }
__host__ __device__ constexpr float split_oscale(int pro) { return 1.f / (SPLIT_WSCALE * split_pscale(pro)); }

enum Prologue : int {
  PRO_X = 0,
  PRO_GN = 1,
  PRO_GN_ADD = 2,
  PRO_RAW = 3
};

struct ConvParams {
  const void* in;
  const void* wpack;
  const float* bias;
  void* out;
  double* stats_out;
  const double* stats_in;
  const float* gn_gamma;
  const float* gn_beta;
  const void* cond;
  const float* emb;
  const long long* tvec;
  int t_base, t_bstride;
  long long t_known = -1;
  const float* y4;
  float* xout;
  const float* c1c2;
  int step;
  int B, h, w;
  int tiles_x, tiles_y;
  const float* cadd;
  const float* cadd_scale;
  float* out_scale;
  const float* etab;
  const float* ttab;
  int ttab_bstride;
  const float* bcorr;
  const void* addend;
  int in_cstride, in_coff, out_cstride, out_coff;
  unsigned long long* prof;
  int persist_slots;
  int ablate;
};

__host__ __device__ inline int swin_ring_size(int h, int w) { return 2 * w + 2 * (h > 2 ? h - 2 : 0); }
__host__ __device__ inline int swin_ring_stride(int h, int w) { return swin_ring_size(h, w) + 4; }
__host__ __device__ inline int swin_ring_index(int y, int x, int h, int w) {
  return y == 0 ? x : (y == h - 1 ? w + x : (x == 0 ? 2 * w + (y - 1) : 2 * w + (h - 2) + (y - 1)));
}
constexpr int SWIN_TT_AX = 7, SWIN_TT_ROWS = 1 + SWIN_TT_AX * SWIN_TT_AX;
__host__ __device__ inline int swin_tt_class(int y, int n) { const int R = n < SWIN_TT_AX ? n : SWIN_TT_AX; return y < 3 ? y : (y >= n - 3 ? R - (n - y) : 3); }
__host__ __device__ inline int swin_tt_ref(int n) { return n - 1 < 3 ? n - 1 : 3; }
inline int persist_grid(int B, int tiles_per_img, int slots) {
  int n = slots / (B > 0 ? B : 1);
  if (n < 1) n = 1;
  if (n > tiles_per_img) n = tiles_per_img;
  return B * n;
}
struct PackGeom { int cin, cout, cout_pad, ck, tg, nt, th, ks, planes, stack; };
hipError_t launch_conv_igemm2(int layer, int ek, const ConvParams& p, hipStream_t s);
hipError_t launch_conv4_stream(int ek, const ConvParams& p, hipStream_t s, bool stack = false, bool in_q15 = false, bool psplit = false);
hipError_t launch_cadd_reformat(const float* src, void* dst, float* scales, int B, int h, int w, int big, int out_kind, hipStream_t s);
PackGeom conv_pack_geom2(int layer, int ek);

size_t pack_weights_bytes(const PackGeom& g, int ek);
hipError_t launch_pack_weights(const float* src_oihw, void* dst, const PackGeom& g, int ek, bool swizzle, bool transposed, hipStream_t s);
hipError_t launch_transpose_flip(const float* w, float* wt, int cout, int cin, int kk, hipStream_t s);
hipError_t launch_max_abs(const float* w, long long n, unsigned* out_bits, hipStream_t s);
hipError_t launch_spin(long long ticks_100mhz, long long* stamp2, hipStream_t s);
hipError_t launch_count_nonfinite(const void* p, long long n, int kind, unsigned* out, hipStream_t s);

hipError_t launch_nchw_to_nhwc(const float* src, void* dst, int ek, int B, int C, int h, int w, int blocked, hipStream_t s);
hipError_t launch_nchw_to_nhwc_padded(const float* src, void* dst, int ek, int B, int C, int Cd, int h, int w, int blocked, hipStream_t s);
hipError_t launch_upsample_to_blocked(const float* src, void* dst, int ek, int B, int C, int ch, int cw, int h, int w, hipStream_t s);
hipError_t launch_blocked_to_nchw(const void* src, int ek, float* dst, int B, int C, int h, int w, int accumulate, hipStream_t s);
hipError_t launch_adaptive_pool_blocked(const void* src, void* dst, int ek, int B, int C, int ih, int iw, int oh, int ow, hipStream_t s);
hipError_t launch_upsample_blocked(const void* src, void* dst, int ek, int B, int C, int ch, int cw, int h, int w, hipStream_t s);
hipError_t launch_nhwc_to_nchw_f32(const void* src, int ek, float* dst, int B, int C, int h, int w, int blocked, hipStream_t s);
hipError_t launch_final(const float* x, const float* y4, const double* stats, const float* gamma, const float* beta,
                        const float* c1c2, int step, int mode, float* out_nchw, int B, int h, int w, hipStream_t s);
hipError_t launch_etab(const float* w3_oihw, const float* emb, float* etab, hipStream_t s);
hipError_t launch_swin_ttab(const float* wa_oihw, const float* wb_oihw, const float* w3_oihw, const float* emb, const long long* ts, int T,
                            int h, int w, float* scratch, float* ttab, hipStream_t s);
constexpr size_t SWIN_KSIDE_BYTES = (size_t)4 * 5 * COND_C * HID_C * (2 + 2 + 4);
hipError_t launch_swin_compose(const float* wb_oihw, const float* w3_oihw, float* w5_oihw, float* pairp, void* kside, hipStream_t s);
hipError_t launch_swin_bcorr(const void* sa, int ek, const float* pairp, const void* kside, float* bcorr, int B, int h, int w, hipStream_t s);
hipError_t launch_add_noise(const float* x0, const float* noise, const long long* t, const float* acp, int n_train,
                            float* out, int B, long long per_sample, hipStream_t s);
struct CodecWeights {
  const float* enc_w0;
  const float* enc_b0;
  const float* enc_w1;
  const float* enc_b1;
  const float* enc_w1t;
  const float* dec_w0;
  const float* dec_b0;
  const float* dec_w0t;
  const float* dec_w1;
  float dec_b1;
};
hipError_t launch_encode(const CodecWeights& cw, const float* depth, float* tmp_nhwc, float* latent_nchw,
                         int B, int H, int W, hipStream_t s);
hipError_t launch_decode(const CodecWeights& cw, const float* latent_nchw, float* tmp_nhwc, float* depth,
                         int B, int h, int w, hipStream_t s);

struct ActView { const void* p; int ek; int blocked; int C; long long HW; };
hipError_t launch_gn_bwd_reduce(const ActView& ga, const ActView& y, const double* stats, const float* gamma, const float* beta,
                                double* out_bc2, int B, hipStream_t s);
hipError_t launch_gn_bwd_apply(const ActView& ga, const ActView& y, const double* stats, const float* gamma, const float* beta,
                               const double* dgb, const ActView& gy, const ActView& act, const ActView& cond, const float* emb,
                               const long long* tvec, int t_base, int t_bstride, int B, hipStream_t s);
hipError_t launch_gn_bwd_reduce_blocked(const void* ga, const void* y, int ek, int yk, const double* stats, const float* gamma, const float* beta,
                                        double* out_bc4, int B, int C, long long HW, hipStream_t s);
hipError_t launch_gn_bwd_apply_blocked(const void* ga, const void* y, int ek, int yk, const double* stats, const float* gamma, const float* beta,
                                       const double* sums_bc4, void* gy, void* act, const void* cond, const float* emb,
                                       const long long* tvec, int t_base, int t_bstride, int B, int C, long long HW, hipStream_t s);
hipError_t launch_gn_param_grad4(const double* sums_bc4, const double* stats, const float* gamma, float* dgamma, float* dbeta, float* dbias,
                                 float* demb, const long long* tvec, int t_base, int t_bstride, int B, int C, long long HW, hipStream_t s);
hipError_t launch_channel_sum_blocked(const void* v, int ek, float* out, int B, int C, long long HW, hipStream_t s);
hipError_t launch_upsample_adjoint(const void* g, int ek, float* dst, int B, int C, int ch, int cw, int h, int w, int accumulate, hipStream_t s, bool tiled = true);
hipError_t launch_channel_sum(const ActView& v, float* out, const long long* rows, int t_base, int t_bstride, int B, hipStream_t s);
hipError_t launch_add_inplace(float* dst, const float* src, long long n, hipStream_t s);
hipError_t launch_gn_param_grad(const double* dgb, float* dgamma, float* dbeta, int B, int C, hipStream_t s);
hipError_t launch_naive_wgrad(const ActView& gy, const ActView& a, float* dw_oihw, int B, int h, int w, hipStream_t s);
size_t wgrad_workspace_bytes(int CO, int CI, int B, int h, int w);
hipError_t launch_wgrad_mfma(const void* gy, const void* a, float* dw_oihw, float* workspace, int ek, int CO, int CI, int B, int h, int w, hipStream_t s,
                             int share = 1);
hipError_t launch_bwd_chain(float* g, float* ga, const float* c1c2, int k, int mode, long long n, hipStream_t s);
hipError_t launch_view_copy(const ActView& src, const ActView& dst, int B, hipStream_t s);
hipError_t launch_view_to_nchw(const ActView& v, float* dst, int B, int accumulate, hipStream_t s);

hipError_t launch_naive_conv3x3(const float* in_nhwc, const float* w_oihw, const float* bias, float* out_nhwc,
                                int B, int h, int w, int cin, int cout, hipStream_t s);
hipError_t launch_naive_gn_stats(const float* y_nhwc, double* stats, int B, int h, int w, int C, hipStream_t s);
hipError_t launch_naive_gn_apply(const float* y, const double* stats, const float* gamma, const float* beta,
                                 const float* cond, const float* emb, const long long* tvec, int t_base, int t_bstride,
                                 float* out, int B, int h, int w, int C, hipStream_t s);
hipError_t launch_naive_axpby(const float* x, const float* eps, const float* c1c2, int step, float* out,
                              long long n, hipStream_t s);

}

#include "dd_kernel_ids.h"
```

### diffusiondepth_amd/csrc/dd_thin.hip

```cpp
#include "dd_igemm2_cfg.h"
#include "dd_gcn.h"

namespace dd {

namespace thin {
constexpr int TH = 8, TW = 32, PH = TH + 2, PW = TW + 2;
constexpr int CIN = HID_C, COUT = LATENT_C, NROW = 32;
constexpr int CK = 16, NCH = CIN / CK, ROWB = CK * 2, PPP = ROWB / 16, RPB = 256 / ROWB, EPP = 8;
constexpr int THREADS = 512, WAVES = 8;
constexpr int W_STAGE = 9 * NROW * ROWB;
constexpr int W_BYTES = NCH * W_STAGE;
constexpr int PATCH_PLANE = PH * PW * ROWB;
constexpr int ITEMS = PH * PW * PPP;
constexpr int NIT = (ITEMS + THREADS - 1) / THREADS;
constexpr int TAB_BYTES = (2 * CIN + NROW) * 4 + WAVES * 8 * 8;
constexpr int smem_bytes(bool psplit) { return W_BYTES + 2 * (psplit ? 2 : 1) * PATCH_PLANE + TAB_BYTES; }
static_assert(smem_bytes(true) <= 80 * 1024, "two workgroups per CU");
static_assert(NCH == 4 && NIT == 2 && (NCH % 2) == 0, "rolling prefetch below is written for four chunks");
static_assert(Cfg2<EK_F16, KID_CONV4>::CK == CK && Cfg2<EK_F16, KID_CONV4>::TG == 9 && Cfg2<EK_F16, KID_CONV4>::NT == NROW && Cfg2<EK_F16, KID_CONV4>::W_BYTES == W_STAGE,
              "the packed weight image of layer 4 (dd_igemm2_cfg.h, DD_C4_CK16) is read as it is");
}

template <int EK, bool STACK, bool INQ, bool PSPLIT>
__global__ void __launch_bounds__(thin::THREADS, 4) conv4_stream_kernel(ConvParams p) {
// ... 96 lines not shown
    return false;
  };
  bool has_next = next_geometry();

  uint4 raw[NCH][NIT];
  float rsc[INQ ? NCH : 1][NIT];
  const float* sc_b = INQ ? p.cadd_scale + (size_t)b * h * w : nullptr;
  auto load_chunk = [&](int c, const int* po) {
    const int cbase = c * CK + jfix * EPP;
    const size_t off0 = (size_t)(cbase >> 5) * h * w * ACT_CB + (cbase & (ACT_CB - 1));
    if (abl & 2) return;
#pragma unroll
    for (int u = 0; u < NIT; ++u) {
      raw[c][u] = *reinterpret_cast<const uint4*>(in_b + (off0 + (size_t)po[u] * ACT_CB) * 2);
      if constexpr (INQ) rsc[c][u] = sc_b[po[u]];
    }
  };
  auto transform_chunk = [&](int c, int buf, unsigned mi) {
    if (abl & 1) return;
    float ta[EPP], tb[EPP];
    const int c0 = c * CK + jfix * EPP;
#pragma unroll
    for (int q = 0; q < EPP / 4; ++q) {
      const float4 a4 = *reinterpret_cast<const float4*>(tab_a + c0 + 4 * q), b4 = *reinterpret_cast<const float4*>(tab_b + c0 + 4 * q);
      ta[4 * q] = a4.x; ta[4 * q + 1] = a4.y; ta[4 * q + 2] = a4.z; ta[4 * q + 3] = a4.w;
      tb[4 * q] = b4.x; tb[4 * q + 1] = b4.y; tb[4 * q + 2] = b4.z; tb[4 * q + 3] = b4.w;
    }
#pragma unroll
    for (int u = 0; u < NIT; ++u) {
      const bool inside = (mi >> u) & 1u;
      uint4 v, vlo = make_uint4(0u, 0u, 0u, 0u);
      if constexpr (!INQ && !PSPLIT) {
        v = affine_relu_pack<EK, EK>(raw[c][u], ta, tb);
      } else {
        float y[EPP];
        if constexpr (INQ) {
          const uint32_t qw[4] = {raw[c][u].x, raw[c][u].y, raw[c][u].z, raw[c][u].w};
          const float sc = rsc[c][u];
#pragma unroll
          for (int i = 0; i < 4; ++i) { y[2 * i] = (float)(short)(qw[i] & 0xFFFFu) * sc; y[2 * i + 1] = (float)((int)qw[i] >> 16) * sc; }
        } else {
          Piece<EK>::unpack(raw[c][u], y);
        }
#pragma unroll
        for (int i = 0; i < EPP; ++i) y[i] = fmaxf(fmaf(ta[i], y[i], tb[i]), 0.f);
        v = Piece<EK>::pack(y);
        if constexpr (PSPLIT) {
          float yh[EPP];
          Piece<EK>::unpack(v, yh);
#pragma unroll
          for (int i = 0; i < EPP; ++i) yh[i] = y[i] - yh[i];
          vlo = Piece<EK>::pack(yh);
          vlo.x = inside ? vlo.x : 0u; vlo.y = inside ? vlo.y : 0u; vlo.z = inside ? vlo.z : 0u; vlo.w = inside ? vlo.w : 0u;
        }
      }
      v.x = inside ? v.x : 0u; v.y = inside ? v.y : 0u; v.z = inside ? v.z : 0u; v.w = inside ? v.w : 0u;
      if ((m_valid >> u) & 1u) {
        *reinterpret_cast<uint4*>(smem + W_BYTES + buf * PATCH_BYTES + lds_off[u]) = v;
        if constexpr (PSPLIT) *reinterpret_cast<uint4*>(smem + W_BYTES + buf * PATCH_BYTES + PATCH_PLANE + lds_off[u]) = vlo;
      }
    }
  };

#pragma unroll
  for (int c = 0; c < NCH; ++c) load_chunk(c, po_cur);
  finish_startup();
  DD_WAIT_VM(0);
  DD_WAIT_LGKM0();
  __builtin_amdgcn_s_barrier();
  asm volatile("" ::: "memory");
  transform_chunk(0, 0, mi_cur);
  DD_WAIT_LGKM0();
  __builtin_amdgcn_s_barrier();
  asm volatile("" ::: "memory");

  int colt[3];
#pragma unroll
  for (int dx = 0; dx < 3; ++dx) colt[dx] = W_BYTES + (wave * PW + li + dx) * ROWB + ((g << 4) ^ swz16<RPB, PPP>(li + dx));
  const int wkt = li * ROWB + ((g << 4) ^ swz16<RPB, PPP>(li));

  float ls[2] = {0.f, 0.f}, lq[2] = {0.f, 0.f};
  char* out_b = reinterpret_cast<char*>(p.out) + (size_t)b * h * w * COUT * 4;
#pragma unroll 1
  for (;;) {
    f32x16_t acc = {0.f, 0.f, 0.f, 0.f, 0.f, 0.f, 0.f, 0.f, 0.f, 0.f, 0.f, 0.f, 0.f, 0.f, 0.f, 0.f};
#pragma unroll
    for (int c = 0; c < NCH; ++c) {
      if (c == 0) load_chunk(0, po_nx);
      const int pbuf = (c & 1) * PATCH_BYTES;
#pragma unroll
      for (int t = 0; t < 9; ++t) {
        if (abl & 8) break;
        const int dy = t / 3, dx = t % 3;
        const uint4 pf = *reinterpret_cast<const uint4*>(smem + colt[dx] + pbuf + dy * (PW * ROWB));
        const uint4 wf = *reinterpret_cast<const uint4*>(smem + wkt + c * W_STAGE + t * (NROW * ROWB));
        mma_step<EK>(acc, wf, pf);
        if constexpr (PSPLIT) {
          const uint4 pl = *reinterpret_cast<const uint4*>(smem + colt[dx] + pbuf + PATCH_PLANE + dy * (PW * ROWB));
          mma_step<EK>(acc, wf, pl);
        }
      }
      if (c + 1 < NCH) {
        transform_chunk(c + 1, (c + 1) & 1, mi_cur);
        load_chunk(c + 1, po_nx);
      } else {
        transform_chunk(0, 0, mi_nx);
      }
      DD_WAIT_LGKM0();
      if (!(abl & 64)) __builtin_amdgcn_s_barrier();
      asm volatile("" ::: "memory");
    }
    {
      const int ty = tl / p.tiles_x, tx = tl - ty * p.tiles_x;
      const int gy = ty * TH + wave, gx = tx * TW + li;
      if (gy < h && gx < w) {
#pragma unroll
        for (int q = 0; q < 2; ++q) {
          const float4 bv = *reinterpret_cast<const float4*>(tab_bias + 8 * q + 4 * g);
          float v0, v1, v2, v3;
          if constexpr (STACK) {
            constexpr float LS = 1.f / STACK_LSCALE, OS = 1.f / PSC;
            v0 = fmaf(fmaf(acc[(q + 2) * 4 + 0], LS, acc[q * 4 + 0]), OS, bv.x); v1 = fmaf(fmaf(acc[(q + 2) * 4 + 1], LS, acc[q * 4 + 1]), OS, bv.y);
            v2 = fmaf(fmaf(acc[(q + 2) * 4 + 2], LS, acc[q * 4 + 2]), OS, bv.z); v3 = fmaf(fmaf(acc[(q + 2) * 4 + 3], LS, acc[q * 4 + 3]), OS, bv.w);
          } else {
            v0 = acc[q * 4 + 0] + bv.x; v1 = acc[q * 4 + 1] + bv.y; v2 = acc[q * 4 + 2] + bv.z; v3 = acc[q * 4 + 3] + bv.w;
          }
          ls[q] += (v0 + v1) + (v2 + v3);
          lq[q] += fmaf(v0, v0, fmaf(v1, v1, fmaf(v2, v2, v3 * v3)));
          if (!(abl & 16)) DD_GLOBAL_STORE16_UNTRACKED(out_b + (((size_t)gy * w + gx) * COUT + 8 * q + 4 * g) * 4, make_float4(v0, v1, v2, v3));
        }
      }
    }
    if (!has_next) break;
    tl += n_per_img;
#pragma unroll
    for (int u = 0; u < NIT; ++u) po_cur[u] = po_nx[u];
    mi_cur = mi_nx;
    has_next = next_geometry();
  }
#pragma unroll
  for (int off = 16; off >= 1; off >>= 1) {
#pragma unroll
    for (int k = 0; k < 2; ++k) { ls[k] += __shfl_xor(ls[k], off, 64); lq[k] += __shfl_xor(lq[k], off, 64); }
  }
  if (li == 0) {
    s_red[wave * 8 + (0 + g) * 2 + 0] = (double)ls[0]; s_red[wave * 8 + (0 + g) * 2 + 1] = (double)lq[0];
    s_red[wave * 8 + (2 + g) * 2 + 0] = (double)ls[1]; s_red[wave * 8 + (2 + g) * 2 + 1] = (double)lq[1];
  }
  __syncthreads();
  if (tid < 8 && !(abl & 32)) {
    double tot = 0.0;
#pragma unroll
    for (int wv = 0; wv < WAVES; ++wv) tot += s_red[wv * 8 + tid];
    atomicAdd(p.stats_out + ((size_t)b * STAT_SLOTS + (wg % STAT_SLOTS)) * STAT_STRIDE + tid, tot);
  }
}

template <int EK, bool STACK, bool INQ, bool PSPLIT> static hipError_t launch_conv4_stream_k(const ConvParams& p, hipStream_t s) {
  static bool attr_set = false;
  constexpr int SMEM = thin::smem_bytes(PSPLIT);
  if (!attr_set) {
    hipError_t e = hipFuncSetAttribute(reinterpret_cast<const void*>(&conv4_stream_kernel<EK, STACK, INQ, PSPLIT>), hipFuncAttributeMaxDynamicSharedMemorySize, SMEM);
    if (e != hipSuccess) return e;
    attr_set = true;
  }
  const unsigned n_wg = (unsigned)persist_grid(p.B, p.tiles_x * p.tiles_y, p.persist_slots > 0 ? p.persist_slots : 512);
  hipLaunchKernelGGL((conv4_stream_kernel<EK, STACK, INQ, PSPLIT>), dim3(n_wg), dim3(thin::THREADS), SMEM, s, p);
  return hipGetLastError();
}

hipError_t launch_conv4_stream(int ek, const ConvParams& p, hipStream_t s, bool stack, bool in_q15, bool psplit) {
  if (ek == EK_F16 && stack) {
    if (in_q15) return psplit ? launch_conv4_stream_k<EK_F16, true, true, true>(p, s) : launch_conv4_stream_k<EK_F16, true, true, false>(p, s);
    return psplit ? launch_conv4_stream_k<EK_F16, true, false, true>(p, s) : launch_conv4_stream_k<EK_F16, true, false, false>(p, s);
  }
  if (stack || in_q15 || psplit) return hipErrorInvalidValue;
  switch (ek) {
    case EK_F16: return launch_conv4_stream_k<EK_F16, false, false, false>(p, s);
    case EK_BF16: return launch_conv4_stream_k<EK_BF16, false, false, false>(p, s);
    default: return hipErrorInvalidValue;
  }
}

}
```

Before: 560.5 maps/s.

## Fuse block-scaled int16 quantization into cond conv3 epilogue and balance thin-conv grid

The conv3(cond) kernel epilogue now quantizes its output straight into the block-scaled int16 layout with per-block scales. This skips the fp32 raw buffer and the separate reformat kernel in the wide f16r path, and the raw buffer is only allocated when still needed. The persistent conv4 grid is trimmed so every workgroup walks an equal number of tiles, and per-lane thin slots are scaled by the whole batch when streams split it. A stats-slot index is changed to match the new grid assignment. The quantization is moved into the epilogue, so rounding or NaN behaviour may differ slightly from the old reformat kernel.

After: 565.6 maps/s (median of 6 runs). Within noise of the previous version (+0.9%).

```diff
diff --git a/diffusiondepth_amd/backend.py b/diffusiondepth_amd/backend.py
--- a/diffusiondepth_amd/backend.py
+++ b/diffusiondepth_amd/backend.py
@@ -448,6 +448,15 @@
             self._ck(self._lib.dd_decode(self._h, latent.data_ptr(), out.data_ptr(), B, h, w, _stream_ptr(self.device)), "dd_decode")
         return out
 
+    def debug_fetch_cadd(self, B: int, h: int, w: int, tile_h: int = 8):
+        torch = _torch()
+        blocks = B * ((h + tile_h - 1) // tile_h) * ((w + 31) // 32) * 4 * 2 * (tile_h // 4)
+        q = torch.empty((blocks, 512), device=self.device, dtype=torch.int32)
+        sc = torch.empty((blocks,), device=self.device, dtype=torch.float32)
+        self._ck(self._lib.dd_debug_fetch(self._h, b"cadd_q15", q.data_ptr(), q.numel(), _stream_ptr(self.device)), "dd_debug_fetch")
+        self._ck(self._lib.dd_debug_fetch(self._h, b"cadd_scale", sc.data_ptr(), sc.numel(), _stream_ptr(self.device)), "dd_debug_fetch")
+        return q.view(torch.int16), sc
+
     def debug_fetch(self, name: str, B: int, h: int, w: int):
         torch = _torch()
         C = {"y1": 64, "y2": 256, "y3": 64, "y4": 16}[name]
diff --git a/diffusiondepth_amd/csrc/dd_api.cpp b/diffusiondepth_amd/csrc/dd_api.cpp
--- a/diffusiondepth_amd/csrc/dd_api.cpp
+++ b/diffusiondepth_amd/csrc/dd_api.cpp
@@ -137,6 +137,11 @@
     if (h->thin_slots != (int)value) { DD_HIP(hipDeviceSynchronize()); h->plans.clear(); h->last_once_plan = nullptr; }
     h->thin_slots = (int)value;
   }
+  else if (k == "thin_fill") {
+    if (value < 0 || value > 1) return h->fail(DD_ERR_INVALID_ARG, "dd_set_option: thin_fill must be 0 or 1");
+    if (h->thin_fill != (int)value) { DD_HIP(hipDeviceSynchronize()); h->plans.clear(); h->last_once_plan = nullptr; }
+    h->thin_fill = (int)value;
+  }
   else if (k == "one_buffer") {
     if (value < 0 || value > 2) return h->fail(DD_ERR_INVALID_ARG, "dd_set_option: one_buffer must be 0, 1 or 2");
     if (h->one_buffer != (int)value) { DD_HIP(hipDeviceSynchronize()); h->plans.clear(); h->last_once_plan = nullptr; }
@@ -145,6 +150,10 @@
   else if (k == "cond_direct") {
     if (value < 0 || value > 1) return h->fail(DD_ERR_INVALID_ARG, "dd_set_option: cond_direct must be 0 or 1");
     h->cond_direct = (int)value;
+  }
+  else if (k == "cadd_fused") {
+    if (value < 0 || value > 1) return h->fail(DD_ERR_INVALID_ARG, "dd_set_option: cadd_fused must be 0 or 1");
+    h->cadd_fused = (int)value;
   }
   else if (k == "cond_split") {
     if (value < 0 || value > 1) return h->fail(DD_ERR_INVALID_ARG, "dd_set_option: cond_split must be 0 or 1");
@@ -191,6 +200,8 @@
   else if (k == "resident_slots") *value = h->resident_slots;
   else if (k == "trajectory_reuses") *value = h->n_traj_reuse;
   else if (k == "thin_stream_launches") *value = h->thin_stream_launches;
+  else if (k == "cadd_reformat_launches") *value = h->cadd_reformat_launches;
+  else if (k == "thin_grid_last") *value = h->thin_grid_last;
   else if (k.compare(0, 13, "kid_launches:") == 0) {
     int id = 0;
     const size_t n = k.size() - 13;
@@ -360,14 +371,14 @@
     const size_t per_step = (size_t)B * lat_h * lat_w * ((2 * HID_C + COND_C + (h->variant == DD_VARIANT_SWIN ? 2 * COND_C : 0)) * es + LATENT_C * 4);
     const size_t need = per_step * (size_t)T;
     if (need <= ((size_t)h->keep_act_mb << 20) &&
-        (h->plans.count(PlanKey{B, lat_h, lat_w, cond_h, cond_w, T, precision, want_hoist(h, precision, T, 2), 2, lane, S}) || keep2_fits(h, need))) keep = 2;
-  }
-  rc = get_plan(h, PlanKey{B, lat_h, lat_w, cond_h, cond_w, T, precision, want_hoist(h, precision, T, keep), keep, lane, S}, &pl);
+        (h->plans.count(PlanKey{B, lat_h, lat_w, cond_h, cond_w, T, precision, want_hoist(h, precision, T, 2), 2, lane, S, S > 1 ? whole_B : 0}) || keep2_fits(h, need))) keep = 2;
+  }
+  rc = get_plan(h, PlanKey{B, lat_h, lat_w, cond_h, cond_w, T, precision, want_hoist(h, precision, T, keep), keep, lane, S, S > 1 ? whole_B : 0}, &pl);
   if (rc && keep == 2) {
     (void)hipGetLastError();
-    h->plans.erase(PlanKey{B, lat_h, lat_w, cond_h, cond_w, T, precision, want_hoist(h, precision, T, 2), 2, lane, S});
+    h->plans.erase(PlanKey{B, lat_h, lat_w, cond_h, cond_w, T, precision, want_hoist(h, precision, T, 2), 2, lane, S, S > 1 ? whole_B : 0});
     keep = 1;
-    rc = get_plan(h, PlanKey{B, lat_h, lat_w, cond_h, cond_w, T, precision, want_hoist(h, precision, T, keep), keep, lane, S}, &pl);
+    rc = get_plan(h, PlanKey{B, lat_h, lat_w, cond_h, cond_w, T, precision, want_hoist(h, precision, T, keep), keep, lane, S, S > 1 ? whole_B : 0}, &pl);
   }
   if (rc) return rc;
   const size_t n16 = (size_t)B * lat_h * lat_w * LATENT_C;
@@ -699,6 +710,14 @@
   if (!pl) return h->fail(DD_ERR_STATE, "dd_debug_fetch: no dd_denoise_once call to inspect");
   const std::string n(name);
   const void* src = nullptr; int C = 0; int ek = store_kind(pl->ek);
+  if (n == "cadd_q15" || n == "cadd_scale") {
+    if (pl->ek != EK_F16R || !pl->wide || !pl->ccond_scale.p) return h->fail(DD_ERR_UNSUPPORTED, "dd_debug_fetch: this plan has no block-scaled int16 hoisted term");
+    const int64_t blocks = (int64_t)(pl->ccond_scale.bytes / 4);
+    const int64_t words = n == "cadd_scale" ? blocks : blocks * 512;
+    if (numel != words) return h->fail(DD_ERR_INVALID_ARG, "dd_debug_fetch: numel mismatch");
+    DD_HIP(hipMemcpyAsync(out, n == "cadd_scale" ? pl->ccond_scale.p : pl->ccond.p, (size_t)words * 4, hipMemcpyDeviceToDevice, reinterpret_cast<hipStream_t>(stream)));
+    return DD_OK;
+  }
   if (n == "y1") { src = pl->y1.p; C = HID_C; }
   else if (n == "y2") { src = pl->y2.p; C = COND_C; }
   else if (n == "y3") {
diff --git a/diffusiondepth_amd/csrc/dd_api_internal.h b/diffusiondepth_amd/csrc/dd_api_internal.h
--- a/diffusiondepth_amd/csrc/dd_api_internal.h
+++ b/diffusiondepth_amd/csrc/dd_api_internal.h
@@ -97,8 +97,9 @@
   int keep = 0;
   int lane = 0;
   int lanes = 1;
+  int batch = 0;
   bool operator<(const PlanKey& o) const {
-    return std::tie(B, h, w, ch, cw, T, prec, hoist, keep, lane, lanes) < std::tie(o.B, o.h, o.w, o.ch, o.cw, o.T, o.prec, o.hoist, o.keep, o.lane, o.lanes);
+    return std::tie(B, h, w, ch, cw, T, prec, hoist, keep, lane, lanes, batch) < std::tie(o.B, o.h, o.w, o.ch, o.cw, o.T, o.prec, o.hoist, o.keep, o.lane, o.lanes, o.batch);
   }
 };
 
@@ -218,6 +219,7 @@
   int64_t keep_act_mb = 65536;
   int n_streams = 1;
   int thin_slots = 512;
+  int thin_fill = 0;
   int big_tiles = -1;
   int one_buffer = 1;
   int thin_stream = 1;
@@ -254,6 +256,8 @@
   std::shared_ptr<DevBuf> fpn_out;
   bool fpn_split_ok = false, neck_split_ok = false;
   int cond_direct = 1;
+  int cadd_fused = 1;
+  int64_t cadd_reformat_launches = 0;
   int cond_split = 1;
   std::shared_ptr<DevBuf> fpn_cond;
   int fpn_cond_key[4] = {0, 0, 0, -1};
@@ -269,6 +273,7 @@
   std::vector<std::tuple<int, hipEvent_t, hipEvent_t>> pending_ev;
   int64_t kid_launches[KID_LAST + 1] = {0};
   int64_t thin_stream_launches = 0;
+  int64_t thin_grid_last = 0;
 
   int fail(int code, const std::string& m) { err = m; return code; }
 };
@@ -306,6 +311,7 @@
 int want_hoist(dd_handle_t h, int precision, int T = 1, int keep = 0);
 bool keep2_fits(dd_handle_t h, size_t need);
 bool plan_big_tiles(dd_handle_t h, const PlanKey& key);
+int plan_thin_slots(dd_handle_t h, const PlanKey& key);
 int get_plan(dd_handle_t h, const PlanKey& key, Plan** out);
 bool conv_tiles(ConvParams& p, int kid, int ek);
 int launch_conv(dd_handle_t h, int kid, int ek, ConvParams p, hipStream_t s, int slot = 0);
diff --git a/diffusiondepth_amd/csrc/dd_api_plans.cpp b/diffusiondepth_amd/csrc/dd_api_plans.cpp
--- a/diffusiondepth_amd/csrc/dd_api_plans.cpp
+++ b/diffusiondepth_amd/csrc/dd_api_plans.cpp
@@ -96,6 +96,11 @@
   const bool many = (long long)key.B * ((key.h + 7) / 8) * ((key.w + 31) / 32) > h->resident_slots;
   return many && h->variant == DD_VARIANT_SWIN;
 }
+int plan_thin_slots(dd_handle_t h, const PlanKey& key) {
+  if (key.lanes <= 1 || key.batch <= key.B) return h->thin_slots;
+  const int per_img = h->thin_slots / key.batch;
+  return key.B * (per_img > 1 ? per_img : 1);
+}
 inline int conv3c_kid(dd_handle_t h, const PlanKey& key) { return plan_big_tiles(h, key) ? (int)BIG_CONV3C : KID_CONV3C; }
 inline int conv3h_kid(dd_handle_t h, const PlanKey& key) {
   if (plan_big_tiles(h, key)) return (int)BIG_CONV3H;
@@ -116,6 +121,8 @@
   h->kid_launches[kid_route(kid, ek).id]++;
   return DD_OK;
 }
+
+int ensure_ccond_raw(dd_handle_t h, Plan* pl);
 
 int get_plan(dd_handle_t h, const PlanKey& key, Plan** out) {
   auto it = h->plans.find(key);
@@ -161,7 +168,7 @@
     DD_HIP(pl->ccond.alloc((size_t)key.B * ((key.h + th - 1) / th) * ((key.w + 31) / 32) * th * 32 * HID_C * 4));
     if (pl->ek == EK_F16R) {
       pl->wide = h->f16r_wide != 0; pl->c1 = h->f16r_c1 != 0; pl->p4 = h->f16r_p4 != 0;
-      DD_HIP(pl->ccond_raw.alloc((size_t)key.B * ((key.h + 7) / 8) * ((key.w + 31) / 32) * 8 * 32 * HID_C * 4));
+      if (swin) DD_TRY(ensure_ccond_raw(h, pl.get()));
       if (pl->wide) DD_HIP(pl->ccond_scale.alloc((size_t)key.B * ((key.h + th - 1) / th) * ((key.w + 31) / 32) * 4 * 2 * (th / 4) * 4));
     }
   }
@@ -233,7 +240,8 @@
     q.prof = (h->prof_buf && layer == h->prof_layer) ? h->prof_buf : nullptr;
     if (layer == KID_CONV4 && (rf || stream4)) {
       if (!conv_tiles(q, KID_CONV4, tk)) return h->fail(DD_ERR_INVALID_ARG, "conv4 has no packed geometry in this element kind");
-      q.persist_slots = h->thin_slots;
+      q.persist_slots = plan_thin_slots(h, k); q.persist_fill = h->thin_fill;
+      h->thin_grid_last = persist_grid(q.B, q.tiles_x * q.tiles_y, q.persist_slots, q.persist_fill != 0);
       if (rf) q.cadd_scale = static_cast<const float*>(pl->slot(pl->y3_scale, step));
       DD_HIP(timed(h, layer, s, [&] { return rf ? launch_conv4_stream(EK_F16, q, s, true, pl->wide, pl->p4) : launch_conv4_stream(tk, q, s); }));
       h->thin_stream_launches++;
@@ -333,15 +341,28 @@
   return DD_OK;
 }
 
+int ensure_ccond_raw(dd_handle_t h, Plan* pl) {
+  if (pl->ccond_raw.p) return DD_OK;
+  const PlanKey& k = pl->key;
+  DD_HIP(pl->ccond_raw.alloc((size_t)k.B * ((k.h + 7) / 8) * ((k.w + 31) / 32) * 8 * 32 * HID_C * 4));
+  return DD_OK;
+}
+
 int enqueue_cond_conv(dd_handle_t h, Plan* pl, hipStream_t s, const float* nchw) {
   const PlanKey& k = pl->key;
   ConvParams p{};
   p.B = k.B; p.h = k.h; p.w = k.w;
   if (pl->ek == EK_F16R) {
     p.in = nchw ? static_cast<const void*>(nchw) : pl->cond_ptr(); p.wpack = h->L[2].wpack2[WIMG_SPLIT].p; p.bias = h->zero_bias.as<float>();
+    if (pl->wide && !plan_big_tiles(h, k) && h->cadd_fused) {
+      p.out = pl->ccond.p; p.out_scale = pl->ccond_scale.as<float>();
+      return launch_conv(h, nchw ? CONV3C_NCHW : KID_CONV3C, EK_F16S, p, s);
+    }
+    DD_TRY(ensure_ccond_raw(h, pl));
     p.out = pl->ccond_raw.p;
     DD_TRY(launch_conv(h, nchw ? CONV3C_NCHW : KID_CONV3C, EK_F16S, p, s));
     DD_HIP(launch_cadd_reformat(pl->ccond_raw.as<float>(), pl->ccond.p, pl->ccond_scale.as<float>(), k.B, k.h, k.w, plan_big_tiles(h, k) ? 1 : 0, pl->wide ? 2 : 1, s));
+    h->cadd_reformat_launches++;
     return DD_OK;
   }
   p.in = pl->cond_ptr(); p.wpack = h->L[2].wpack2[wimg_slot(thin_kind(pl->ek))].p; p.bias = h->zero_bias.as<float>(); p.out = pl->ccond.p;
@@ -386,6 +407,7 @@
     DD_TRY(launch_conv(h, KID_SWIN_CONVB, EK_F16S, p, s));
     p.in = pl->sf.p; p.wpack = h->L[2].wpack2[WIMG_SPLIT].p; p.bias = h->zero_bias.as<float>(); p.out = pl->ccond_raw.p;
     DD_TRY(launch_conv(h, KID_CONV3C, EK_F16S, p, s));
+    h->cadd_reformat_launches++;
     DD_HIP(launch_cadd_reformat(pl->ccond_raw.as<float>(), pl->ccond.p, pl->ccond_scale.as<float>(), k.B, k.h, k.w, plan_big_tiles(h, k) ? 1 : 0, pl->wide ? 2 : 1, s));
     return DD_OK;
   }
diff --git a/diffusiondepth_amd/csrc/dd_api_train.cpp b/diffusiondepth_amd/csrc/dd_api_train.cpp
--- a/diffusiondepth_amd/csrc/dd_api_train.cpp
+++ b/diffusiondepth_amd/csrc/dd_api_train.cpp
@@ -291,7 +291,7 @@
                           int whole_B, int64_t ticket, bool* reused, int S) {
   int rc = DD_OK;
   Plan* pl = nullptr;
-  rc = get_plan(h, PlanKey{B, lat_h, lat_w, cond_h, cond_w, T, precision, want_hoist(h, precision, T, 1), 0, lane, S}, &pl);
+  rc = get_plan(h, PlanKey{B, lat_h, lat_w, cond_h, cond_w, T, precision, want_hoist(h, precision, T, 1), 0, lane, S, S > 1 ? whole_B : 0}, &pl);
   if (rc) return rc;
   rc = ensure_bwd_buffers(h, pl);
   if (rc) return rc;
@@ -299,7 +299,7 @@
   const size_t n16 = (size_t)B * lat_h * lat_w * LATENT_C;
   const Plan* kept = nullptr;
   for (int lvl = 2; lvl >= 1 && !kept && ticket != 0 && !naive; --lvl) {
-    auto it = h->plans.find(PlanKey{B, lat_h, lat_w, cond_h, cond_w, T, precision, want_hoist(h, precision, T, lvl), lvl, lane, S});
+    auto it = h->plans.find(PlanKey{B, lat_h, lat_w, cond_h, cond_w, T, precision, want_hoist(h, precision, T, lvl), lvl, lane, S, S > 1 ? whole_B : 0});
     if (it != h->plans.end() && it->second->traj_ticket == ticket && it->second->traj_weights == h->weights_serial) kept = it->second.get();
   }
   const Plan* kept_act = (kept && kept->key.keep == 2 && kept->ek == pl->ek) ? kept : nullptr;
diff --git a/diffusiondepth_amd/csrc/dd_igemm2.hip b/diffusiondepth_amd/csrc/dd_igemm2.hip
--- a/diffusiondepth_amd/csrc/dd_igemm2.hip
+++ b/diffusiondepth_amd/csrc/dd_igemm2.hip
@@ -686,6 +686,32 @@
       }
       continue;
     }
+    if constexpr (C::LAYER == KID_CONV3C && C::SPLIT) {
+      static_assert(!C::STATS && C::WM == 2, "layer 8 on 8x32 tiles");
+      if (p.out_scale != nullptr) {
+        auto nmax = [](float a, float b) { return (b > a || b != b) ? b : a; };
+#pragma unroll
+        for (int n = 0; n < C::WN; ++n) {
+          float v[4][4];
+          float mx = 0.f;
+#pragma unroll
+          for (int q = 0; q < 4; ++q) {
+            value_of(n, q, v[q]);
+            mx = nmax(mx, nmax(nmax(fabsf(v[q][0]), fabsf(v[q][1])), nmax(fabsf(v[q][2]), fabsf(v[q][3]))));
+          }
+#pragma unroll
+          for (int off = 32; off >= 1; off >>= 1) mx = nmax(mx, __shfl_xor(mx, off, 64));
+          const float inv = mx > 0.f ? 1.f / mx : 0.f;
+          const size_t blk = (((size_t)e_tile * C::WAVES + wave) * C::WN + n) * C::WM + m;
+          if (lane == 0) p.out_scale[blk] = mx * (1.f / Q15_ONE);
+#pragma unroll
+          for (int q = 0; q < 4; ++q)
+            reinterpret_cast<uint2*>(p.out)[blk * 256 + q * 64 + lane] =
+                make_uint2(DD_CVT_PKNORM_I16(v[q][0] * inv, v[q][1] * inv), DD_CVT_PKNORM_I16(v[q][2] * inv, v[q][3] * inv));
+        }
+        continue;
+      }
+    }
 #pragma unroll
     for (int n = 0; n < C::WN; ++n) {
       uint2 pk[4];
diff --git a/diffusiondepth_amd/csrc/dd_kernels.h b/diffusiondepth_amd/csrc/dd_kernels.h
--- a/diffusiondepth_amd/csrc/dd_kernels.h
+++ b/diffusiondepth_amd/csrc/dd_kernels.h
@@ -65,6 +65,7 @@
   int in_cstride, in_coff, out_cstride, out_coff;
   unsigned long long* prof;
   int persist_slots;
+  int persist_fill;
   int ablate;
 };
 
@@ -76,10 +77,11 @@
 constexpr int SWIN_TT_AX = 7, SWIN_TT_ROWS = 1 + SWIN_TT_AX * SWIN_TT_AX;
 __host__ __device__ inline int swin_tt_class(int y, int n) { const int R = n < SWIN_TT_AX ? n : SWIN_TT_AX; return y < 3 ? y : (y >= n - 3 ? R - (n - y) : 3); }
 __host__ __device__ inline int swin_tt_ref(int n) { return n - 1 < 3 ? n - 1 : 3; }
-inline int persist_grid(int B, int tiles_per_img, int slots) {
+inline int persist_grid(int B, int tiles_per_img, int slots, bool fill = false) {
   int n = slots / (B > 0 ? B : 1);
   if (n < 1) n = 1;
   if (n > tiles_per_img) n = tiles_per_img;
+  if (n > 0 && !fill) { const int walk = (tiles_per_img + n - 1) / n; n = (tiles_per_img + walk - 1) / walk; }
   return B * n;
 }
 struct PackGeom { int cin, cout, cout_pad, ck, tg, nt, th, ks, planes, stack; };
diff --git a/diffusiondepth_amd/csrc/dd_thin.hip b/diffusiondepth_amd/csrc/dd_thin.hip
--- a/diffusiondepth_amd/csrc/dd_thin.hip
+++ b/diffusiondepth_amd/csrc/dd_thin.hip
@@ -272,7 +272,7 @@
     double tot = 0.0;
 #pragma unroll
     for (int wv = 0; wv < WAVES; ++wv) tot += s_red[wv * 8 + tid];
-    atomicAdd(p.stats_out + ((size_t)b * STAT_SLOTS + (wg % STAT_SLOTS)) * STAT_STRIDE + tid, tot);
+    atomicAdd(p.stats_out + ((size_t)b * STAT_SLOTS + ((wg / p.B) % STAT_SLOTS)) * STAT_STRIDE + tid, tot);
   }
 }
 
@@ -284,7 +284,7 @@
     if (e != hipSuccess) return e;
     attr_set = true;
   }
-  const unsigned n_wg = (unsigned)persist_grid(p.B, p.tiles_x * p.tiles_y, p.persist_slots > 0 ? p.persist_slots : 512);
+  const unsigned n_wg = (unsigned)persist_grid(p.B, p.tiles_x * p.tiles_y, p.persist_slots > 0 ? p.persist_slots : 512, p.persist_fill != 0);
   hipLaunchKernelGGL((conv4_stream_kernel<EK, STACK, INQ, PSPLIT>), dim3(n_wg), dim3(thin::THREADS), SMEM, s, p);
   return hipGetLastError();
 }
```
